# johncai117/Meta-Fine-Tuning

Hardware: AMD Instinct MI355X
Metric: episodes/sec at 5-way N-shot (ResNet10+GNN) per GPU and 1/2/4/8-GPU node (higher is better)
Workload: dtype f32

## Files before the change

include/mft_hip.h:

```cpp
#ifndef MFT_HIP_H
#define MFT_HIP_H

#ifdef __cplusplus
extern "C" {
#endif

#define MFT_EINVAL (-22)

enum { MFT_ACT_NONE = 0, MFT_ACT_RELU = 1, MFT_ACT_LRELU = 2 };
enum { MFT_BN_AFFINE_FMA = 0x100 };

int mft_version(void);
int mft_device_info(int* cu_count, int* gcn_arch_is_gfx950);

int mft_stream_create_cumask(const unsigned* mask_words, int n_words, void** stream_out);
int mft_stream_create_priority(int priority, void** stream_out, int* range_out);
int mft_stream_destroy(void* stream);
int mft_stream_probe(float* w, float* m, float* v, long long n, void* stream);
int mft_event_create(void** event_out);
int mft_event_record(void* event, void* stream);
int mft_event_elapsed_ms(void* start, void* stop, float* ms_out);
int mft_event_destroy(void* event);
int mft_probe_placement(unsigned* out, int n_blocks, int spin_cycles, void* stream);

int mft_augment_views(const unsigned char* src, int n_img, int Hs, int Ws, const float* params, int n_views, float* out,
                      long long view_stride, long long img_stride, int size, const float* mean3, const float* std3,
                      void* stream);

int mft_nchw_to_nhwc(const float* src, float* dst, int n_img, int C, int H, int W, void* stream);

long long mft_conv2d_wgrad_adam_dgrad_ws_floats(int n_img, int H, int W, int Cin);
int mft_conv2d_wgrad_adam_dgrad_nhwc(const float* x, int ldx, const float* dy, int ldy, float* w, float* m, float* v,
                                     float* dx_partials, int n_img, int H, int W, int Cin, int Cout, int imgs_per_group,
                                     long long group_stride, int step, float lr, float beta1, float beta2, float eps, void* stream);
int mft_conv2d_wgrad_adam_dgrad_nhwc_dev(const float* x, int ldx, const float* dy, int ldy, float* w, float* m, float* v,
                                         float* dx_partials, int n_img, int H, int W, int Cin, int Cout, int imgs_per_group,
                                         long long group_stride, const float* hyper, float beta1, float beta2, float eps,
                                         void* stream);
int mft_col2im_bn_backward_small(const float* dx_partials, const float* x_raw, const float* relu_out, float* dx, int n_img, int H,
                                 int W, int C, int imgs_per_group, const float* mean, const float* rstd, const float* gamma,
                                 long long gb_group_stride, float* dgamma, float* dbeta, void* stream);

int mft_ce_pool_bn_backward2(const float* feat, const int* labels, int imgs_per_group, int n_groups, int C, int hw,
                             const float* out, const float* xa, const float* xb, float* dxa, float* dxb, const float* mean_a,
                             const float* rstd_a, const float* gamma_a, const float* mean_b, const float* rstd_b,
                             const float* gamma_b, long long gb_group_stride, float* dgamma_a, float* dbeta_a, float* dgamma_b,
                             float* dbeta_b, float* loss, void* stream);

int mft_stem_cache_fill(const float* in, const float* w, int w_ld, int n_img, int H, int W, float* pmax, float* pmin,
                        float* mean_img, float* m2_img, void* stream);
int mft_pool_window_minmax(const float* x, float* ymax, float* ymin, long long n_img, int H, int W, int C, void* stream);
int mft_bn_relu_pooled_gather(const float* pmax, const float* pmin, const int* src_idx, float* y, int n_img, int OH, int OW, int C,
                              int imgs_per_group, const float* mean, const float* rstd, const float* gamma, const float* beta,
                              void* stream);

int mft_bn_apply_planes(const float* x, int ldx, float* y, int ldy, unsigned short* planes, long long plane_stride, int C,
                        int rows_per_group, int n_groups, const float* mean, const float* rstd, const float* gamma,
                        const float* beta, long long gb_group_stride, const float* res, int ldr, const float* res_mean,
                        const float* res_rstd, const float* res_gamma, const float* res_beta, int act, float slope,
                        void* stream);
int mft_bn_relu_maxpool_gather_planes(const float* x, const int* src_idx, float* y, unsigned short* planes,
                                      long long plane_stride, int n_img, int H, int W, int C, int imgs_per_group,
                                      const float* mean, const float* rstd, const float* gamma, const float* beta, void* stream);
int mft_conv2d_nhwc_x3p_bnstats(const unsigned short* in_planes, long long in_plane_elems, int ldi, const unsigned short* w3,
                                long long plane_elems, float* out, int ldo, int n_img, int H, int W, int Cin, int Cout, int KH,
                                int KW, int stride, int pad, int imgs_per_group, float eps, float* stats_ws, float* mean,
                                float* rstd, void* stream);

int mft_ingest_episode_views(const float* const* views, int n_views, int double_first, int n_way, int per_class, int n_support,
                             int C, int H, int W, float* support_store, float* all_store, void* stream);
int mft_pack_oihw(const float* w_oihw, float* w_pk, int Cout, int Cin, int KH, int KW, int k_pad, void* stream);
int mft_pack_oihw_multi(const void* jobs, int n_jobs, long long total_elements, void* stream);
int mft_unpack_oihw(const float* w_pk, float* w_oihw, int Cout, int Cin, int KH, int KW, int k_pad, void* stream);
int mft_pack_dgrad(const float* w_pk, float* wt_pk, int Cout, int Cin, int KH, int KW,
                   int groups, long long w_stride, long long wt_stride, void* stream);

int mft_conv2d_nhwc(const float* in, int ldi, const float* w, const float* bias, float* out, int ldo,
                    int n_img, int H, int W, int Cin, int Cout, int KH, int KW, int stride, int pad,
                    int imgs_per_group, long long w_group_stride, void* stream);

int mft_split_bf16x3(const float* w, unsigned short* planes, long long n, void* stream);
int mft_split_bf16x3_multi(const void* jobs, int n_jobs, long long total_elements, void* stream);
int mft_conv2d_nhwc_x3(const float* in, int ldi, const unsigned short* w3, long long plane_elems, float* out, int ldo,
                       int n_img, int H, int W, int Cin, int Cout, int KH, int KW, int stride, int pad, void* stream);
long long mft_conv2d_x3_stats_ws_floats(int n_img, int H, int W, int Cout, int KH, int KW, int stride, int pad);
int mft_conv2d_nhwc_x3_bnstats(const float* in, int ldi, const unsigned short* w3, long long plane_elems, float* out, int ldo,
                               int n_img, int H, int W, int Cin, int Cout, int KH, int KW, int stride, int pad,
                               int imgs_per_group, float eps, float* stats_ws, float* mean, float* rstd, void* stream);
int mft_conv2d_nhwc_x3_bnin_bnstats(const float* in, int ldi, const float* in_ws, const float* in_gamma, const float* in_beta,
                                    const unsigned short* w3, long long plane_elems, float* out, int ldo, int n_img, int H, int W,
                                    int Cin, int Cout, int imgs_per_group, float eps, float* stats_ws, float* mean, float* rstd,
                                    void* stream);
int mft_split_f16x2(const float* w, unsigned short* planes, long long n, void* stream);
int mft_conv2d_nhwc_h2(const float* in, int ldi, const unsigned short* w2, long long plane_elems, float* out, int ldo,
                       int n_img, int H, int W, int Cin, int Cout, int KH, int KW, int stride, int pad, void* stream);
int mft_conv2d_nhwc_h2_bnstats(const float* in, int ldi, const unsigned short* w2, long long plane_elems, float* out, int ldo,
                               int n_img, int H, int W, int Cin, int Cout, int KH, int KW, int stride, int pad,
                               int imgs_per_group, float eps, float* stats_ws, float* mean, float* rstd, void* stream);
int mft_conv2d_nhwc_h2_bnin_bnstats(const float* in, int ldi, const float* in_ws, const float* in_gamma, const float* in_beta,
                                    const unsigned short* w2, long long plane_elems, float* out, int ldo, int n_img, int H, int W,
                                    int Cin, int Cout, int imgs_per_group, float eps, float* stats_ws, float* mean, float* rstd,
                                    void* stream);
int mft_bn_apply_x3ws(const float* x, int ldx, float* y, int ldy, int C, int rows_per_group, int n_groups, const float* ws,
                      const float* gamma, const float* beta, const float* res, int ldr, const float* res_ws,
                      const float* res_gamma, const float* res_beta, int act, float slope, float eps, float* mean, float* rstd,
                      float* res_mean, float* res_rstd, void* stream);
int mft_bn_running_ema(const float* mean_a, const float* rstd_a, int rows_a, const float* mean_b, const float* rstd_b, int rows_b,
                       const int* order, int n_steps, int C, float eps, float momentum, float* running_mean, float* running_var,
                       void* stream);
int mft_bn_apply_x3ws_fits(int C, int rows_per_group, int with_res_bn);
int mft_bn_relu_pooled_gather_moments(const float* pmax, const float* pmin, const int* src_idx, float* y, int n_img, int OH, int OW,
                                      int C, int imgs_per_group, const float* mean_img, const float* m2_img, int rows_per_img,
                                      float eps, const float* gamma, const float* beta, float* mean, float* rstd, void* stream);

int mft_has_experiments(void);

int mft_conv2d_dgrad_nhwc(const float* dy, int ldy, const float* w, float* dx, int ldx,
                          int n_img, int H, int W, int Cin, int Cout, int KH, int KW, int stride, int pad,
                          int imgs_per_group, long long w_group_stride, void* stream);

long long mft_conv_ksplit_ws_floats(long long rows, int cols, int K);
long long mft_conv_ksplit_grouped_ws_floats(long long rows_per_group, int cols, int K, int groups);
int mft_conv2d_nhwc_ksplit_grouped(const float* in, int ldi, const float* w, float* out, int ldo, int n_img, int H, int W, int Cin,
                                   int Cout, int KH, int KW, int stride, int pad, int imgs_per_group, long long w_group_stride,
                                   float* ws, void* stream);
int mft_conv2d_dgrad_nhwc_ksplit_grouped(const float* dy, int ldy, const float* w, float* dx, int ldx, int n_img, int H, int W, int Cin,
                                         int Cout, int KH, int KW, int stride, int pad, int imgs_per_group, long long w_group_stride,
                                         float* ws, void* stream);
int mft_conv2d_nhwc_ksplit(const float* in, int ldi, const float* w, const float* bias, float* out, int ldo, int n_img, int H, int W,
                           int Cin, int Cout, int KH, int KW, int stride, int pad, float* ws, void* stream);
int mft_conv2d_dgrad_nhwc_ksplit(const float* dy, int ldy, const float* w, float* dx, int ldx, int n_img, int H, int W, int Cin,
                                 int Cout, int KH, int KW, int stride, int pad, float* ws, void* stream);
long long mft_conv2d_wgrad_ws_floats(int n_img, int H, int W, int Cin, int Cout, int KH, int KW, int stride, int pad,
                                     int imgs_per_group);
int mft_conv2d_wgrad_nhwc(const float* in, int ldi, const float* dy, int ldy, float* dw,
                          int n_img, int H, int W, int Cin, int Cout, int KH, int KW, int stride, int pad,
                          int imgs_per_group, long long dw_group_stride, float* ws, void* stream);

long long mft_conv2d_wgrad_oihw_ws_floats(int n_img, int H, int W, int Cin, int Cout, int KH, int KW, int stride, int pad);
int mft_conv2d_wgrad_oihw(const float* in, int ldi, const float* dy, int ldy, float* dw_oihw, int n_img, int H, int W, int Cin,
                          int Cout, int KH, int KW, int stride, int pad, int cin_valid, int cout_valid, float* ws, void* stream);

typedef struct MftWgradJob {
    const float* in; const float* dy; float* dw_oihw; float* ws;
    int ldi, ldy, n_img, H, W, Cin, Cout, KH, KW, stride, pad, cin_valid, cout_valid, reserved;
} MftWgradJob;
int mft_conv2d_wgrad_oihw_multi(const MftWgradJob* jobs, int n_jobs, void* stream);

int mft_conv2d_wgrad_adam_nhwc(const float* in, int ldi, const float* dy, int ldy, float* w, float* m, float* v,
                               float* dw_or_null, int n_img, int H, int W, int Cin, int Cout, int KH, int KW,
                               int stride, int pad, int imgs_per_group, long long group_stride,
                               int step, float lr, float beta1, float beta2, float eps, void* stream);

int mft_wgrad_adam_next_forward(const float* x, int ldx, const float* dy, int ldy, float* w, float* m, float* v,
                                float* dw_or_null, int n_img, int H, int W, int Cin, int Cout, int KH, int KW, int stride,
                                int pad, int imgs_per_group, long long group_stride, int step, const float* hyper, float lr,
                                float beta1, float beta2, float eps, const float* x_next, int mode, float* raw, float* act,
                                const float* gamma, const float* beta, long long gb_group_stride, float* mean, float* rstd,
                                const float* sc_raw, const float* gamma_s, const float* beta_s, float* mean_s, float* rstd_s,
                                float* pooled, float bn_eps, void* stream);


long long mft_bn_stats_ws_floats(int C, int rows_per_group, int n_groups);
int mft_bn_stats(const float* x, int ldx, int C, int rows_per_group, int n_groups, float eps,
                 float* mean, float* rstd, float* ws,
                 float* running_mean, float* running_var, float momentum, long long* num_batches_tracked, void* stream);
typedef struct MftBnStatsJob {
    const float* x; float* mean; float* rstd; float* ws; float* running_mean; float* running_var; long long* num_batches_tracked;
    int ldx, C, rows_per_group, n_groups; float eps, momentum;
} MftBnStatsJob;
int mft_bn_stats_multi(const MftBnStatsJob* jobs, int n_jobs, void* stream);
typedef struct MftBnFwdJob {
    const float* x; float* y; const float* gamma; const float* beta; float* mean; float* rstd;
    float* running_mean; float* running_var; long long* num_batches_tracked;
    const float* res; const float* res_gamma; const float* res_beta; float* res_mean; float* res_rstd;
    float* res_running_mean; float* res_running_var; long long* res_num_batches_tracked;
    int ldx, ldy, ldr, C, rows_per_group, n_groups, act; float eps, momentum, slope;
} MftBnFwdJob;
int mft_bn_forward_small(const MftBnFwdJob* job, void* stream);
int mft_bn_forward_small_max_rows(void);
typedef struct MftBnApplyJob {
    const float* x; float* y; const float* mean; const float* rstd; const float* gamma; const float* beta;
    int ldx, ldy, C, rows_per_group, n_groups, act; float slope; int reserved;
} MftBnApplyJob;
int mft_bn_apply_multi(const MftBnApplyJob* jobs, int n_jobs, void* stream);
int mft_bn_apply(const float* x, int ldx, float* y, int ldy, int C, int rows_per_group, int n_groups,
                 const float* mean, const float* rstd, const float* gamma, const float* beta,
                 long long gb_group_stride,
                 const float* res, int ldr, const float* res_mean, const float* res_rstd,
                 const float* res_gamma, const float* res_beta,
                 int act, float slope, void* stream);
int mft_var_to_rstd(const float* var, float* rstd, int n, float eps, void* stream);
int mft_bn_relu_maxpool(const float* x, float* y, int n_img, int H, int W, int C, int imgs_per_group,
                        const float* mean, const float* rstd, const float* gamma, const float* beta,
                        void* stream);

int mft_bn_image_moments(const float* x, int ldx, int C, int rows_per_img, long long n_img, float* mean_img, float* m2_img,
                         void* stream);
int mft_bn_combine_moments(const float* mean_img, const float* m2_img, const int* idx, int C, int rows_per_img,
                           int imgs_per_group, int n_groups, float eps, float* mean, float* rstd, void* stream);
int mft_bn_relu_maxpool_gather(const float* x, const int* src_idx, float* y, int n_img, int H, int W, int C,
                               int imgs_per_group, const float* mean, const float* rstd, const float* gamma,
                               const float* beta, void* stream);
int mft_global_avgpool(const float* x, float* y, int n_img, int HW, int C, void* stream);

int mft_bn_backward(const float* x, int ldx, const float* dy, int lddy, const float* relu_out, int ldro,
                    float* dx, int lddx, int C, int rows_per_group, int n_groups,
                    const float* mean, const float* rstd, const float* gamma, long long gb_group_stride,
                    float* dgamma, float* dbeta, void* stream);
int mft_bn_small_forward(const float* x1, int ld1, const float* x2, int ld2, const float* res, int ldr, float* y, int ldy, int C,
                         int rows_per_group, int n_groups, const float* gamma1, const float* beta1, const float* gamma2,
                         const float* beta2, long long gb_group_stride, float* mean1, float* rstd1, float* mean2, float* rstd2,
                         int act, float slope, float eps, float* pooled, int hw, void* stream);
int mft_bn_backward2(const float* xa, const float* xb, int ldx, const float* dy, int lddy, float* dxa, float* dxb, int lddx, int C,
                     int rows_per_group, int n_groups, const float* mean_a, const float* rstd_a, const float* gamma_a,
                     const float* mean_b, const float* rstd_b, const float* gamma_b, long long gb_group_stride, float* dgamma_a,
                     float* dbeta_a, float* dgamma_b, float* dbeta_b, void* stream);
int mft_ce_pool_backward(const float* feat, const int* labels, int rows_per_group, int n_groups, int C, int hw, const float* out,
                         float* d_out, float* loss, void* stream);

int mft_avgpool_relu_backward(const float* dfeat, const float* out, float* dout, int n_img, int HW, int C, void* stream);

int mft_cross_entropy(const float* logits, int ld, const int* labels, int C, int rows_per_group, int n_groups,
                      float* loss, float* dlogits, void* stream);
int mft_cross_entropy_mean(const float* logits, int ld, const void* labels, int labels_i64, int C, int rows, float* loss,
                           double* loss_sum, void* stream);
int mft_cross_entropy_mean_backward(const float* logits, int ld, const void* labels, int labels_i64, int C, int rows,
                                    const float* grad_loss, float* dlogits, int ldd, void* stream);
int mft_softmax_rows(const float* x, int ldx, float* y, int ldy, int C, int rows, void* stream);

int mft_proto_scores(const float* feats, int ld, int episodes, int n_way, int n_support, int n_query, int D, float* scores,
                     int softmax, void* stream);
int mft_proto_backward(const float* feats, int ld, int episodes, int n_way, int n_support, int n_query, int D,
                       const float* dscores, int ldg, float* dfeats, int ldd, void* stream);

int mft_adam_step(float* p, const float* g, float* m, float* v, long long n, int step,
                  float lr, float beta1, float beta2, float eps, float weight_decay, void* stream);
int mft_sgd_step(float* p, const float* g, float* buf, long long n, int first_step,
                 float lr, float momentum, float dampening, float weight_decay, void* stream);
int mft_block_entry_small_forward(const float* x, int ldx, const float* w_c1, long long w1_group_stride, const float* w_sc,
                                  long long wsc_group_stride, float* c1, float* r1, float* sc, int n_img, int H, int W, int Cin,
                                  int Cout, int stride, int imgs_per_group, const float* gamma1, const float* beta1,
                                  long long gb_group_stride, float* mean1, float* rstd1, float eps, void* stream);

int mft_block_exit_small_forward(const float* r1, const float* w_c2, long long w_group_stride, const float* sc, float* c2,
                                 float* out, float* pooled, int n_img, int H, int W, int C, int imgs_per_group,
                                 const float* gamma2, const float* beta2, const float* gamma_sc, const float* beta_sc,
                                 long long gb_group_stride, float* mean2, float* rstd2, float* mean_sc, float* rstd_sc, float eps,
                                 void* stream);

int mft_conv2d_dgrad_bn_backward_small(const float* dy, int ldy, const float* w, float* dx, int ldx, int n_img, int H, int W,
                                       int Cin, int Cout, int KH, int KW, int pad, int imgs_per_group, long long w_group_stride,
                                       const float* x_raw, const float* relu_out, const float* mean, const float* rstd,
                                       const float* gamma, long long gb_group_stride, float* dgamma, float* dbeta, void* stream);

int mft_linear_head_sgd_run(const float* z_support, const int* y_support, const int* idx_table, int n_groups, int n_support_rows,
                            int D, int n_way, int n_steps, int batch_size, float* W, float* b, float lr, float momentum,
                            float dampening, float weight_decay, void* stream);

int mft_linear_head_adam_run(const float* z_support, const int* y_support, const int* idx_table, int n_groups, int n_support_rows,
                             int D, int n_way, int n_steps, int batch_size, float* W, float* b, float lr, float beta1, float beta2,
                             float eps, float weight_decay, void* stream);

int mft_adam_multi(const void* chunk_table, int n_chunks, int step, float lr, float beta1, float beta2, float eps,
                   float weight_decay, float grad_scale, void* stream);

int mft_adam_hyper_advance(int* step, float* hyper, float lr, float beta1, float beta2, void* stream);
int mft_adam_step_dev(float* p, const float* g, float* m, float* v, long long n, const float* hyper, float beta1, float beta2,
                      float eps, float weight_decay, void* stream);
int mft_conv2d_wgrad_adam_nhwc_dev(const float* in, int ldi, const float* dy, int ldy, float* w, float* m, float* v,
                                   float* dw_or_null, int n_img, int H, int W, int Cin, int Cout, int KH, int KW, int stride,
                                   int pad, int imgs_per_group, long long group_stride, const float* hyper, float beta1,
                                   float beta2, float eps, void* stream);
int mft_maml_delta(float* p, const float* p2, const float* p3, long long n, void* stream);

int mft_linear_head_step(const float* feat, int ldf, const int* labels, int rows_per_group, int n_groups, int n_way, int D,
                         float* W, float* b, float* mW, float* vW, float* mb, float* vb, float* dfeat, int lddf, float* loss,
                         int step, float lr, float beta1, float beta2, float eps, float weight_decay, void* stream);
int mft_linear_head_scores(const float* feat, int ldf, int rows_per_group, int n_groups, int n_way, int D, const float* W,
                           const float* b, float* out, void* stream);

int mft_pair_absdiff(const float* x, int ldx, float* d, int ldd, int n_graphs, int N, int F, void* stream);
int mft_masked_softmax(const float* s, int lds_, float* A, int n_graphs, int N, void* stream);
int mft_gemm_rk(const float* a, int lda, const float* w, int w_rows, int K, const float* bias, float* out, int ldo, int M, int N,
                void* stream);
int mft_pair_mlp_tiles_m(int graphs_per_group, int N);
int mft_pair_mlp_tiles_m_rk(int graphs_per_group, int N);
int mft_pair_mlp_layer_rk(const float* in, int ld_in, int mode, const int* ij, const float* scale_in, const float* shift_in,
                          const float* w, int K, int Kpad, const float* bias, float* out, int Cout, int n_groups,
                          int graphs_per_group, int N, float slope, float* ws_mean, float* ws_m2, float* ws_n, void* stream);
int mft_pair_mlp_stats_finalize_rk(const float* ws_mean, const float* ws_m2, const float* ws_n, int n_groups, int tiles_m, int C,
                                   const float* gamma, const float* beta, float eps, float* scale, float* shift,
                                   float* mean_out, float* rstd_out, void* stream);
int mft_pair_mlp_layer(const float* in, int ld_in, int mode, const int* ij, const float* scale_in, const float* shift_in,
                       const float* w, int K, int Kpad, const float* bias, float* out, int Cout, int n_groups,
                       int graphs_per_group, int N, float slope, float* ws_mean, float* ws_m2, float* ws_n, int f16x2, void* stream);
int mft_pair_mlp_stats_finalize(const float* ws_mean, const float* ws_m2, const float* ws_n, int n_groups, int tiles_m, int C,
                                const float* gamma, const float* beta, float eps, float* scale, float* shift,
                                float* mean_out, float* rstd_out, void* stream);
int mft_pair_mlp_score(const float* h, int C, const float* scale, const float* shift, const float* w5, const float* b5,
                       float slope, float* s_ut, int n_groups, int graphs_per_group, int N, void* stream);
int mft_masked_softmax_ut(const float* s_ut, float* A, int n_graphs, int N, void* stream);

int mft_pair_softmax_ut_backward(const float* A, const float* dA, const int* ij, float* rowdot_ws, float* ds, int ldds,
                                 int n_graphs, int N, float* dbias_zero, void* stream);
long long mft_pair_bwd_stats_ws_floats(long long rows_per_group, int C);
int mft_pair_bn_act_backward(const float* g, int ldg, const float* z, int C, const float* scale, const float* shift,
                             const float* mean, const float* rstd, const float* gamma, const int* ij, int N, long long rows_per_group,
                             int n_groups, long long n_tot, float slope, float* ws, float* sums, float* dparams, float* dbias_zero,
                             float* dz, void* stream);
int mft_pair_absdiff_ut(const float* x, int ldx, const int* ij, float* d, int Kp, int F, int N, long long row0, long long nrows,
                        void* stream);
int mft_pair_dx_gather(const float* x, int ldx, const float* dd, int lddd, float* dX, int lddx, int n_graphs, int N, int F,
                       long long row0, long long nrows, void* stream);
int mft_graph_aggregate(const float* A, const float* x, int ldx, float* y, int ldy,
                        int n_graphs, int N, int F, void* stream);
int mft_copy_cols(const float* x, int ldx, float* y, int ldy, int col_off, int C, int rows,
                  int act, float slope, void* stream);

int mft_build_graph_nodes(const float* z, int zf, float* nodes, int ld, int n_episodes, int n_way,
                          int n_support, int n_query, int fold, void* stream);
int mft_gather_query_scores(const float* out, int ldo, float* scores, int n_episodes, int n_way,
                            int n_support, int n_query, void* stream);
int mft_gather_rows(const float* src, const int* idx, float* dst, int n_rows, long long row_floats, void* stream);

long long mft_bn_backward_ws_floats(int C, int rows_per_group, int n_groups);
int mft_bn_backward_act(const float* x, int ldx, const float* dy, int lddy, const float* y_act, int ldya,
                        float* dx, int lddx, int C, int rows_per_group, int n_groups,
                        const float* mean, const float* rstd, const float* gamma, long long gb_group_stride,
                        float* dgamma, float* dbeta, int act, float slope, float* ws, float* dgamma_sum, float* dbeta_sum,
                        float* dbias_zero, void* stream);
typedef struct MftBnBwdJob {
    const float* x; const float* dy; const float* y_act; float* dx; const float* mean; const float* rstd; const float* gamma;
    float* dgamma; float* dbeta; float* ws; float* dgamma_sum; float* dbeta_sum; float* dbias_zero;
    int ldx, lddy, ldya, lddx, C, rows_per_group, n_groups, act; float slope; int reserved;
} MftBnBwdJob;
int mft_bn_backward_act_multi(const MftBnBwdJob* jobs, int n_jobs, void* stream);
int mft_act_backward(const float* dy, int lddy, const float* y, int ldy, float* dx, int lddx, int C, long long rows,
                     int act, float slope, int accumulate, void* stream);
int mft_colsum(const float* x, int ldx, int C, long long rows, float* out, float* ws, void* stream);
int mft_bn_relu_maxpool_arg(const float* x, float* y, unsigned char* argmax, int n_img, int H, int W, int C,
                            int imgs_per_group, const float* mean, const float* rstd, const float* gamma,
                            const float* beta, void* stream);
int mft_maxpool_relu_backward(const float* dy, const unsigned char* argmax, const float* y, float* dx,
                              int n_img, int H, int W, int C, void* stream);
int mft_masked_softmax_backward(const float* A, const float* dA, float* ds, int ldds, int n_graphs, int N, void* stream);
int mft_pair_absdiff_backward(const float* x, int ldx, const float* dd, int ldd, float* dx, int lddx,
                              int n_graphs, int N, int F, void* stream);
int mft_graph_aggregate_backward(const float* A, const float* x, int ldx, const float* dy, int lddy, float* dx, int lddx,
                                 float* dA, int n_graphs, int N, int F, int accumulate, void* stream);
int mft_build_graph_nodes_backward(const float* dnodes, int ld, float* dz, int zf, int n_episodes, int n_way,
                                   int n_support, int n_query, int fold, void* stream);
int mft_gather_query_scores_backward(const float* dscores, float* dout, int ldo, int n_episodes, int n_way,
                                     int n_support, int n_query, float* dbias, void* stream);

#ifdef __cplusplus
}
#endif
#endif
```

include/mft_hip_testing.h:

```cpp
#ifndef MFT_HIP_TESTING_H
#define MFT_HIP_TESTING_H
#ifdef __cplusplus
extern "C" {
#endif

int mft_debug_set_conv_tile(int tile);
int mft_debug_set_x3_tile(int tile);
int mft_debug_reset(void);
void mft_wgrad_fwd_set_exact(int on);
void mft_wgrad_fwd_set_xcd(int on);

#ifdef __cplusplus
}
#endif
#endif
```

meta-fine-tuning_amd/_lib.py:

```python
import ctypes
import os

PKG = os.path.dirname(os.path.abspath(__file__))
LIB_PATH = os.path.join(PKG, "libmft_hip.so")

_P = ctypes.c_void_p
_I = ctypes.c_int
_L = ctypes.c_longlong
_F = ctypes.c_float

SIGNATURES = {
    "mft_version": [],
    "mft_device_info": [_P, _P],
    "mft_stream_create_cumask": [_P, _I, _P],
    "mft_stream_destroy": [_P],
    "mft_stream_probe": [_P, _P, _P, _L, _P],
    "mft_probe_placement": [_P, _I, _I, _P],
    "mft_event_create": [_P],
    "mft_event_record": [_P, _P],
    "mft_event_elapsed_ms": [_P, _P, _P],
    "mft_event_destroy": [_P],
    "mft_augment_views": [_P, _I, _I, _I, _P, _I, _P, _L, _L, _I, _P, _P, _P],
    "mft_nchw_to_nhwc": [_P, _P, _I, _I, _I, _I, _P],
    "mft_pack_oihw": [_P, _P, _I, _I, _I, _I, _I, _P],
    "mft_unpack_oihw": [_P, _P, _I, _I, _I, _I, _I, _P],
    "mft_pack_dgrad": [_P, _P, _I, _I, _I, _I, _I, _L, _L, _P],
    "mft_conv2d_nhwc": [_P, _I, _P, _P, _P, _I, _I, _I, _I, _I, _I, _I, _I, _I, _I, _I, _L, _P],
    "mft_has_experiments": [],
    "mft_split_bf16x3": [_P, _P, _L, _P],
    "mft_split_bf16x3_multi": [_P, _I, _L, _P],
    "mft_conv2d_nhwc_x3": [_P, _I, _P, _L, _P, _I, _I, _I, _I, _I, _I, _I, _I, _I, _I, _P],
    "mft_conv2d_x3_stats_ws_floats": [_I, _I, _I, _I, _I, _I, _I, _I],
    "mft_conv2d_nhwc_x3_bnstats": [_P, _I, _P, _L, _P, _I, _I, _I, _I, _I, _I, _I, _I, _I, _I, _I, _F, _P, _P, _P, _P],
    "mft_conv2d_dgrad_nhwc": [_P, _I, _P, _P, _I, _I, _I, _I, _I, _I, _I, _I, _I, _I, _I, _L, _P],
    "mft_conv_ksplit_ws_floats": [_L, _I, _I],
    "mft_conv_ksplit_grouped_ws_floats": [_L, _I, _I, _I],
    "mft_conv2d_nhwc_ksplit_grouped": [_P, _I, _P, _P, _I, _I, _I, _I, _I, _I, _I, _I, _I, _I, _I, _L, _P, _P],
    "mft_conv2d_dgrad_nhwc_ksplit_grouped": [_P, _I, _P, _P, _I, _I, _I, _I, _I, _I, _I, _I, _I, _I, _I, _L, _P, _P],
    "mft_conv2d_nhwc_ksplit": [_P, _I, _P, _P, _P, _I, _I, _I, _I, _I, _I, _I, _I, _I, _I, _P, _P],
    "mft_conv2d_dgrad_nhwc_ksplit": [_P, _I, _P, _P, _I, _I, _I, _I, _I, _I, _I, _I, _I, _I, _P, _P],
    "mft_conv2d_wgrad_oihw_ws_floats": [_I, _I, _I, _I, _I, _I, _I, _I, _I],
    "mft_conv2d_wgrad_oihw": [_P, _I, _P, _I, _P, _I, _I, _I, _I, _I, _I, _I, _I, _I, _I, _I, _P, _P],
    "mft_conv2d_wgrad_oihw_multi": [_P, _I, _P],
    "mft_conv2d_wgrad_ws_floats": [_I, _I, _I, _I, _I, _I, _I, _I, _I, _I],
    "mft_conv2d_wgrad_nhwc": [_P, _I, _P, _I, _P, _I, _I, _I, _I, _I, _I, _I, _I, _I, _I, _L, _P, _P],
    "mft_conv2d_wgrad_adam_nhwc": [_P, _I, _P, _I, _P, _P, _P, _P, _I, _I, _I, _I, _I, _I, _I, _I, _I, _I, _L, _I, _F, _F, _F,
                                   _F, _P],
    "mft_pair_softmax_ut_backward": [_P, _P, _P, _P, _P, _I, _I, _I, _P, _P],
    "mft_pair_bwd_stats_ws_floats": [_L, _I],
    "mft_pair_bn_act_backward": [_P, _I, _P, _I, _P, _P, _P, _P, _P, _P, _I, _L, _I, _L, _F, _P, _P, _P, _P, _P, _P],
    "mft_pair_absdiff_ut": [_P, _I, _P, _P, _I, _I, _I, _L, _L, _P],
    "mft_pair_dx_gather": [_P, _I, _P, _I, _P, _I, _I, _I, _I, _L, _L, _P],
    "mft_pack_oihw_multi": [_P, _I, _L, _P],
    "mft_wgrad_adam_next_forward": [_P, _I, _P, _I, _P, _P, _P, _P, _I, _I, _I, _I, _I, _I, _I, _I, _I, _I, _L, _I, _P, _F, _F, _F,
                                    _F, _P, _I, _P, _P, _P, _P, _L, _P, _P, _P, _P, _P, _P, _P, _P, _F, _P],
    "mft_bn_stats_ws_floats": [_I, _I, _I],
    "mft_bn_stats": [_P, _I, _I, _I, _I, _F, _P, _P, _P, _P, _P, _F, _P, _P],
    "mft_bn_apply": [_P, _I, _P, _I, _I, _I, _I, _P, _P, _P, _P, _L, _P, _I, _P, _P, _P, _P, _I, _F, _P],
    "mft_bn_apply_multi": [_P, _I, _P],
    "mft_bn_stats_multi": [_P, _I, _P],
    "mft_bn_relu_maxpool": [_P, _P, _I, _I, _I, _I, _I, _P, _P, _P, _P, _P],
    "mft_bn_relu_maxpool_gather": [_P, _P, _P, _I, _I, _I, _I, _I, _P, _P, _P, _P, _P],
    "mft_bn_image_moments": [_P, _I, _I, _I, _L, _P, _P, _P],
    "mft_bn_combine_moments": [_P, _P, _P, _I, _I, _I, _I, _F, _P, _P, _P],
    "mft_global_avgpool": [_P, _P, _I, _I, _I, _P],
    "mft_bn_small_forward": [_P, _I, _P, _I, _P, _I, _P, _I, _I, _I, _I, _P, _P, _P, _P, _L, _P, _P, _P, _P, _I, _F, _F, _P, _I, _P],
    "mft_bn_backward2": [_P, _P, _I, _P, _I, _P, _P, _I, _I, _I, _I, _P, _P, _P, _P, _P, _P, _L, _P, _P, _P, _P, _P],
    "mft_ce_pool_backward": [_P, _P, _I, _I, _I, _I, _P, _P, _P, _P],
    "mft_bn_backward": [_P, _I, _P, _I, _P, _I, _P, _I, _I, _I, _I, _P, _P, _P, _L, _P, _P, _P],
    "mft_avgpool_relu_backward": [_P, _P, _P, _I, _I, _I, _P],
    "mft_cross_entropy": [_P, _I, _P, _I, _I, _I, _P, _P, _P],
    "mft_softmax_rows": [_P, _I, _P, _I, _I, _I, _P],
    "mft_proto_scores": [_P, _I, _I, _I, _I, _I, _I, _P, _I, _P],
    "mft_proto_backward": [_P, _I, _I, _I, _I, _I, _I, _P, _I, _P, _I, _P],
    "mft_cross_entropy_mean": [_P, _I, _P, _I, _I, _I, _P, _P, _P],
    "mft_cross_entropy_mean_backward": [_P, _I, _P, _I, _I, _I, _P, _P, _I, _P],
    "mft_adam_step": [_P, _P, _P, _P, _L, _I, _F, _F, _F, _F, _F, _P],
    "mft_sgd_step": [_P, _P, _P, _L, _I, _F, _F, _F, _F, _P],
    "mft_maml_delta": [_P, _P, _P, _L, _P],
    "mft_conv2d_wgrad_adam_dgrad_ws_floats": [_I, _I, _I, _I],
    "mft_conv2d_wgrad_adam_dgrad_nhwc": [_P, _I, _P, _I, _P, _P, _P, _P, _I, _I, _I, _I, _I, _I, _L, _I, _F, _F, _F, _F, _P],
    "mft_conv2d_wgrad_adam_dgrad_nhwc_dev": [_P, _I, _P, _I, _P, _P, _P, _P, _I, _I, _I, _I, _I, _I, _L, _P, _F, _F, _F, _P],
    "mft_col2im_bn_backward_small": [_P, _P, _P, _P, _I, _I, _I, _I, _I, _P, _P, _P, _L, _P, _P, _P],
    "mft_stream_create_priority": [_I, _P, _P],
    "mft_ce_pool_bn_backward2": [_P, _P, _I, _I, _I, _I, _P, _P, _P, _P, _P, _P, _P, _P, _P, _P, _P, _L, _P, _P, _P, _P, _P, _P],
    "mft_pool_window_minmax": [_P, _P, _P, _L, _I, _I, _I, _P],
    "mft_stem_cache_fill": [_P, _P, _I, _I, _I, _I, _P, _P, _P, _P, _P],
    "mft_conv2d_nhwc_x3_bnin_bnstats": [_P, _I, _P, _P, _P, _P, _L, _P, _I, _I, _I, _I, _I, _I, _I, _F, _P, _P, _P, _P],
    "mft_split_f16x2": [_P, _P, _L, _P],
    "mft_conv2d_nhwc_h2": [_P, _I, _P, _L, _P, _I, _I, _I, _I, _I, _I, _I, _I, _I, _I, _P],
    "mft_conv2d_nhwc_h2_bnstats": [_P, _I, _P, _L, _P, _I, _I, _I, _I, _I, _I, _I, _I, _I, _I, _I, _F, _P, _P, _P, _P],
    "mft_conv2d_nhwc_h2_bnin_bnstats": [_P, _I, _P, _P, _P, _P, _L, _P, _I, _I, _I, _I, _I, _I, _I, _F, _P, _P, _P, _P],
    "mft_bn_apply_x3ws": [_P, _I, _P, _I, _I, _I, _I, _P, _P, _P, _P, _I, _P, _P, _P, _I, _F, _F, _P, _P, _P, _P, _P],
    "mft_bn_apply_x3ws_fits": [_I, _I, _I],
    "mft_bn_running_ema": [_P, _P, _I, _P, _P, _I, _P, _I, _I, _F, _F, _P, _P, _P],
    "mft_bn_relu_pooled_gather_moments": [_P, _P, _P, _P, _I, _I, _I, _I, _I, _P, _P, _I, _F, _P, _P, _P, _P, _P],
    "mft_bn_relu_pooled_gather": [_P, _P, _P, _P, _I, _I, _I, _I, _I, _P, _P, _P, _P, _P],
    "mft_bn_apply_planes": [_P, _I, _P, _I, _P, _L, _I, _I, _I, _P, _P, _P, _P, _L, _P, _I, _P, _P, _P, _P, _I, _F, _P],
    "mft_bn_relu_maxpool_gather_planes": [_P, _P, _P, _P, _L, _I, _I, _I, _I, _I, _P, _P, _P, _P, _P],
    "mft_conv2d_nhwc_x3p_bnstats": [_P, _L, _I, _P, _L, _P, _I, _I, _I, _I, _I, _I, _I, _I, _I, _I, _I, _F, _P, _P, _P, _P],
    "mft_ingest_episode_views": [_P, _I, _I, _I, _I, _I, _I, _I, _I, _P, _P, _P],
    "mft_block_entry_small_forward": [_P, _I, _P, _L, _P, _L, _P, _P, _P, _I, _I, _I, _I, _I, _I, _I, _P, _P, _L, _P, _P, _F, _P],
    "mft_block_exit_small_forward": [_P, _P, _L, _P, _P, _P, _P, _I, _I, _I, _I, _I, _P, _P, _P, _P, _L, _P, _P, _P, _P, _F, _P],
    "mft_conv2d_dgrad_bn_backward_small": [_P, _I, _P, _P, _I, _I, _I, _I, _I, _I, _I, _I, _I, _I, _L, _P, _P, _P, _P, _P, _L,
                                           _P, _P, _P],
    "mft_linear_head_sgd_run": [_P, _P, _P, _I, _I, _I, _I, _I, _I, _P, _P, _F, _F, _F, _F, _P],
    "mft_linear_head_adam_run": [_P, _P, _P, _I, _I, _I, _I, _I, _I, _P, _P, _F, _F, _F, _F, _F, _P],
    "mft_adam_multi": [_P, _I, _I, _F, _F, _F, _F, _F, _F, _P],
    "mft_adam_hyper_advance": [_P, _P, _F, _F, _F, _P],
    "mft_adam_step_dev": [_P, _P, _P, _P, _L, _P, _F, _F, _F, _F, _P],
    "mft_conv2d_wgrad_adam_nhwc_dev": [_P, _I, _P, _I, _P, _P, _P, _P, _I, _I, _I, _I, _I, _I, _I, _I, _I, _I, _L, _P, _F, _F,
                                       _F, _P],
    "mft_linear_head_step": [_P, _I, _P, _I, _I, _I, _I, _P, _P, _P, _P, _P, _P, _P, _I, _P, _I, _F, _F, _F, _F, _F, _P],
    "mft_linear_head_scores": [_P, _I, _I, _I, _I, _I, _P, _P, _P, _P],
    "mft_pair_absdiff": [_P, _I, _P, _I, _I, _I, _I, _P],
    "mft_masked_softmax": [_P, _I, _P, _I, _I, _P],
    "mft_pair_mlp_tiles_m": [_I, _I],
    "mft_pair_mlp_layer": [_P, _I, _I, _P, _P, _P, _P, _I, _I, _P, _P, _I, _I, _I, _I, _F, _P, _P, _P, _I, _P],
    "mft_bn_forward_small": [_P, _P],
    "mft_bn_forward_small_max_rows": [],
    "mft_gemm_rk": [_P, _I, _P, _I, _I, _P, _P, _I, _I, _I, _P],
    "mft_pair_mlp_tiles_m_rk": [_I, _I],
    "mft_pair_mlp_layer_rk": [_P, _I, _I, _P, _P, _P, _P, _I, _I, _P, _P, _I, _I, _I, _I, _F, _P, _P, _P, _P],
    "mft_pair_mlp_stats_finalize_rk": [_P, _P, _P, _I, _I, _I, _P, _P, _F, _P, _P, _P, _P, _P],
    "mft_pair_mlp_stats_finalize": [_P, _P, _P, _I, _I, _I, _P, _P, _F, _P, _P, _P, _P, _P],
    "mft_pair_mlp_score": [_P, _I, _P, _P, _P, _P, _F, _P, _I, _I, _I, _P],
    "mft_masked_softmax_ut": [_P, _P, _I, _I, _P],
    "mft_graph_aggregate": [_P, _P, _I, _P, _I, _I, _I, _I, _P],
    "mft_copy_cols": [_P, _I, _P, _I, _I, _I, _I, _I, _F, _P],
    "mft_build_graph_nodes": [_P, _I, _P, _I, _I, _I, _I, _I, _I, _P],
    "mft_gather_query_scores": [_P, _I, _P, _I, _I, _I, _I, _P],
    "mft_gather_rows": [_P, _P, _P, _I, _L, _P],
    "mft_var_to_rstd": [_P, _P, _I, _F, _P],
    "mft_bn_backward_ws_floats": [_I, _I, _I],
    "mft_bn_backward_act": [_P, _I, _P, _I, _P, _I, _P, _I, _I, _I, _I, _P, _P, _P, _L, _P, _P, _I, _F, _P, _P, _P, _P, _P],
    "mft_bn_backward_act_multi": [_P, _I, _P],
    "mft_act_backward": [_P, _I, _P, _I, _P, _I, _I, _L, _I, _F, _I, _P],
    "mft_colsum": [_P, _I, _I, _L, _P, _P, _P],
    "mft_bn_relu_maxpool_arg": [_P, _P, _P, _I, _I, _I, _I, _I, _P, _P, _P, _P, _P],
    "mft_maxpool_relu_backward": [_P, _P, _P, _P, _I, _I, _I, _I, _P],
    "mft_masked_softmax_backward": [_P, _P, _P, _I, _I, _I, _P],
    "mft_pair_absdiff_backward": [_P, _I, _P, _I, _P, _I, _I, _I, _I, _P],
    "mft_graph_aggregate_backward": [_P, _P, _I, _P, _I, _P, _I, _P, _I, _I, _I, _I, _P],
    "mft_build_graph_nodes_backward": [_P, _I, _P, _I, _I, _I, _I, _I, _I, _P],
    "mft_gather_query_scores_backward": [_P, _P, _I, _I, _I, _I, _I, _P, _P],
}
TESTING_SIGNATURES = {
    "mft_debug_set_conv_tile": [_I],
    "mft_debug_set_x3_tile": [_I],
    "mft_debug_reset": [],
    "mft_wgrad_fwd_set_exact": [_I],
    "mft_wgrad_fwd_set_xcd": [_I],
}
_RESTYPE = {"mft_conv2d_x3_stats_ws_floats": _L, "mft_bn_stats_ws_floats": _L, "mft_conv2d_wgrad_ws_floats": _L, "mft_bn_backward_ws_floats": _L,
            "mft_conv2d_wgrad_adam_dgrad_ws_floats": _L, "mft_pair_bwd_stats_ws_floats": _L, "mft_conv_ksplit_ws_floats": _L, "mft_conv2d_wgrad_oihw_ws_floats": _L, "mft_conv_ksplit_grouped_ws_floats": _L}

_lib = None


def lib():
    global _lib
    if _lib is None:
        if not os.path.exists(LIB_PATH):
            raise RuntimeError(
                "libmft_hip.so not found at %s -- build it with `python -c 'import __graft_entry__ as g; g.build()'`; "
                "this package has no CPU or PyTorch fallback" % LIB_PATH)
        import torch
        if torch.cuda.is_available():
            torch.cuda.init()
            torch.empty(1, device="cuda")
        h = ctypes.CDLL(LIB_PATH)
        for name, argtypes in list(SIGNATURES.items()) + list(TESTING_SIGNATURES.items()):
            fn = getattr(h, name)
            fn.argtypes = argtypes
            fn.restype = _RESTYPE.get(name, _I)
        _lib = h
    return _lib


MFT_EINVAL = -22


def check(rc, what):
    if rc != 0:
        raise RuntimeError("%s failed with code %d (hipError_t / MFT_EINVAL=-22)" % (what, rc))


class LaunchTimer:

    _SKIP = ("mft_event_", "mft_stream_", "mft_debug_", "mft_version", "mft_device_info", "mft_has_experiments",
             "mft_wgrad_fwd_set_", "mft_probe_placement")

    def __init__(self, only=None, keep_args=False):
        self.only = only
        self.keep_args = keep_args
        self._pairs = []
        self._free = []
        self._real = None

    def _event(self):
        if self._free:
            return self._free.pop()
        e = ctypes.c_void_p()
        check(self._real.mft_event_create(ctypes.byref(e)), "mft_event_create")
        return e

    def __getattr__(self, name):
        real = self.__dict__["_real"]
        fn = getattr(real, name)
        sig = SIGNATURES.get(name)
        if (sig is None or not sig or sig[-1] is not _P or name.endswith("_ws_floats") or name.startswith(self._SKIP)
                or (self.only is not None and not self.only(name))):
            return fn

        def timed(*args):
            stream = args[-1]
            a, b = self._event(), self._event()
            real.mft_event_record(a, stream)
            rc = fn(*args)
            if rc != 0:
                self._free += [a, b]
                return rc
            real.mft_event_record(b, stream)
            self._pairs.append((name, a, b, args if self.keep_args else None))
            return rc
        return timed

    def __enter__(self):
        global _lib
        self._real = lib()
        assert not isinstance(self._real, LaunchTimer), "LaunchTimer blocks do not nest"
        _lib = self
        return self

    def __exit__(self, *exc):
        global _lib
        _lib = self._real
        if exc and exc[0] is not None:
            for _, a, b, _ in self._pairs:
                self._free += [a, b]
            self._pairs = []
            self.close()
        return False

    def collect(self, calls=False):
        out, flat = {}, []
        ms = ctypes.c_float()
        for name, a, b, args in self._pairs:
            check(self._real.mft_event_elapsed_ms(a, b, ctypes.byref(ms)), "mft_event_elapsed_ms")
            out.setdefault(name, []).append(float(ms.value))
            flat.append((name, float(ms.value), args))
            self._free += [a, b]
        self._pairs = []
        return flat if calls else out

    def close(self):
        for e in self._free:
            self._real.mft_event_destroy(e)
        self._free = []
```

meta-fine-tuning_amd/csrc/conv_igemm.hip:

```cpp
#include "mft_common.h"
#include "mft_hip_testing.h"

int mft_stem_conv_dispatch(const float* in, const float* w, float* out, int n_img, int H, int W, int w_ld,
                           hipStream_t s);
int mft_skinny_fwd_dispatch(const float* in, int ldi, const float* w, float* out, int ldo, int n_img, int H, int W,
                            int Cin, int Cout, int KH, int KW, int stride, int pad, int imgs_per_group,
                            long long w_group_stride, hipStream_t s);
void mft_skinny_set_dgrad_slices(int n);
void mft_skinny_set_tap(int v);
void mft_skinny_set_x3(int v);
void mft_skinny_set_nw(int v);
void mft_bn_small_set_rows(int rows);
void mft_bn_fwd_small_set_rows(int rows);
void mft_skinny_set_lines(int v);
int mft_skinny_dgrad_dispatch(const float* dy, int ldy, const float* w, float* dx, int ldx, int n_img, int H, int W,
                              int Cin, int Cout, int KH, int KW, int stride, int pad, int imgs_per_group,
                              long long w_group_stride, hipStream_t s);

namespace {

struct ConvArgs {
    const float* in;
    const float* w;
    const float* bias;
// ... 915 lines not shown
            rdy[u] = v;
        }
        const long long ibase = (long long)img * p.H * p.W;
#pragma unroll
        for (int u = 0; u < NPR; ++u) {
            const int ih = 2 * oh - 3 + e_kh[u], iw = 2 * ow0 - 3 + e_q3[u];
            float v = 0.f;
            if (e_lds[u] >= 0 && ih >= 0 && ih < p.H && iw >= 0 && iw < p.W) v = p.in[(ibase + (long long)ih * p.W + iw) * p.ldi + e_ci[u]];
            rpr[u] = v;
        }
    };
    auto store_strip = [&]() {
#pragma unroll
        for (int u = 0; u < NDY; ++u) {
            const int i = tid + NT * u;
            *(f32x4*)(dy_s + (i >> 4) * 64 + (i & 15) * 4) = rdy[u];
        }
#pragma unroll
        for (int u = 0; u < NPR; ++u)
            if (e_lds[u] >= 0) prow[e_lds[u]] = rpr[u];
    };

    int kh_q[NQ];
#pragma unroll
    for (int q = 0; q < NQ; ++q) kh_q[q] = wave + NWAVE * q < 14 ? (wave + NWAVE * q) >> 1 : 0;
    int s = blockIdx.x;
    if (s < n_strips) load_strip(s);
    for (; s < n_strips; s += gridDim.x) {
        __syncthreads();
        store_strip();
        __syncthreads();
        if (s + (int)gridDim.x < n_strips) load_strip(s + gridDim.x);
        const float* ap = dy_s + h * 64 + cb * 32 + r;
        const float* bp = prow + 6 * h + r;
        const int np = S2 >> 1;
        int tp = 0;
        for (; tp + 4 <= np; tp += 4) {
            float a[4], b[4][NQ];
#pragma unroll
            for (int u = 0; u < 4; ++u) {
                a[u] = ap[(tp + u) * 128];
#pragma unroll
                for (int q = 0; q < NQ; ++q) b[u][q] = bp[kh_q[q] * PR + 12 * (tp + u)];
            }
#pragma unroll
            for (int u = 0; u < 4; ++u)
#pragma unroll
                for (int q = 0; q < NQ; ++q) acc[q] = __builtin_amdgcn_mfma_f32_32x32x2f32(a[u], b[u][q], acc[q], 0, 0, 0);
        }
        for (; tp < np; ++tp) {
            const float a = ap[tp * 128];
#pragma unroll
            for (int q = 0; q < NQ; ++q) acc[q] = __builtin_amdgcn_mfma_f32_32x32x2f32(a, bp[kh_q[q] * PR + 12 * tp], acc[q], 0, 0, 0);
        }
    }
    float* out = p.ws + (long long)blockIdx.x * p.dwgs;
#pragma unroll
    for (int q = 0; q < NQ; ++q) {
        const int c = wave + NWAVE * q;
        if (c >= 14 || r >= 21) continue;
        const int kh = c >> 1;
#pragma unroll
        for (int e = 0; e < 16; ++e) {
            const int co = cb * 32 + (e & 3) + 8 * (e >> 2) + 4 * h;
            out[(long long)co * p.Kpad + kh * 21 + r] = acc[q][e];
        }
    }
}

int g_stem_wgrad_strips = 1;

template <int BM, int BN, bool ADAM, bool STEMW = false, bool EARLYT = false, int POL = 3>
int launch_wgrad(const WgradArgs& a, int taps, int groups, hipStream_t s) {
    constexpr int lds_mm = 32 * (BM + BN) * 4;
    constexpr int lds_ad = BM * (BN + 4) * 4;
    constexpr int lds0 = ADAM ? (lds_ad > lds_mm ? lds_ad : lds_mm) : lds_mm;
    int lds = lds0;
    if (ADAM && g_wgrad_min_lds_kb * 1024 > lds) lds = g_wgrad_min_lds_kb * 1024;
    auto kern = conv_wgrad_kernel<BM, BN, ADAM, STEMW, EARLYT, POL>;
    if (lds > 64 * 1024) {
        static MftPerDeviceOnce attr_once;
        if (attr_once.need()) {
            hipError_t e = hipFuncSetAttribute((const void*)kern, hipFuncAttributeMaxDynamicSharedMemorySize, lds);
            if (e != hipSuccess) return (int)e;
            attr_once.mark();
        }
    }
    WgradArgs p = a;
    p.tiles_ci = ((STEMW ? a.Kpad : a.Cin) + BN - 1) / BN;
    p.tiles_co = (a.Cout + BM - 1) / BM;
    dim3 grid(p.tiles_ci * p.tiles_co * taps, groups, p.chunks);
    hipLaunchKernelGGL(kern, grid, dim3(256), lds, s, p);
    if (p.oihw || p.chunks > 1) {
        const long long n = (long long)a.Cout * a.Kpad;
        int blocks = (int)((n / 4 + 31) / 32);
        if (blocks > 4096) blocks = 4096;
        if (p.oihw)
            hipLaunchKernelGGL(reduce_chunks_kernel<true>, dim3(blocks, 1), dim3(256), 0, s, (const float*)p.ws, p.dw, n, p.chunks, p.dwgs,
                               a.Cin, a.KH * a.KW, a.Kpad, a.cin_out > 0 ? a.cin_out : a.Cin, a.cout_out > 0 ? a.cout_out : a.Cout);
        else
            hipLaunchKernelGGL(reduce_chunks_kernel<false>, dim3(blocks, groups), dim3(256), 0, s, (const float*)p.ws, p.dw, n, p.chunks,
                               p.dwgs, a.Cin, a.KH * a.KW, a.Kpad, a.Cin, a.Cout);
    }
    return mft_launch_status();
}

constexpr int WGRAD_CHUNK_ROWS = 1024;

inline void wgrad_chunking(long long rows, long long wgs_per_chunk, int* chunk_rows, int* chunks) {
    *chunk_rows = (int)rows;
    *chunks = 1;
    if (rows <= 256) return;
    const long long want = (768 + wgs_per_chunk - 1) / wgs_per_chunk;
    long long cr = ((rows + want - 1) / want + 31) / 32 * 32;
    if (cr < 128) cr = 128;
    if (cr > WGRAD_CHUNK_ROWS) cr = WGRAD_CHUNK_ROWS;
    const long long n = (rows + cr - 1) / cr;
    if (n <= 1) return;
    *chunk_rows = (int)cr;
    *chunks = (int)n;
}

inline long long wgrad_wgs_per_chunk(int Cin, int Cout, int KH, int KW, long long groups) {
    if (Cin == 3) return (long long)(((KH * KW * Cin + 31) / 32 * 32 + 63) / 64) * ((Cout + 63) / 64) * groups;
    return (long long)((Cin + 63) / 64) * ((Cout + 63) / 64) * KH * KW * groups;
}

int wgrad_dispatch(WgradArgs a, int n_img, int imgs_per_group, bool adam, float* ws, hipStream_t s) {
    if (imgs_per_group <= 0) imgs_per_group = n_img;
    if (n_img % imgs_per_group != 0) return MFT_EINVAL;
    const bool stem = (a.Cin == 3);
    if ((!stem && a.Cin % 4 != 0) || a.Cout % 4 != 0 || (!stem && a.ldi % 4 != 0) || a.ldy % 4 != 0) return MFT_EINVAL;
    const int groups = n_img / imgs_per_group;
    a.OH = (a.H + 2 * a.pad - a.KH) / a.stride + 1;
    a.OW = (a.W + 2 * a.pad - a.KW) / a.stride + 1;
    a.Kpad = (a.KH * a.KW * a.Cin + 31) / 32 * 32;
    a.imgs_per_group = imgs_per_group;
    a.rows_per_group = imgs_per_group * a.OH * a.OW;
    a.chunk_rows = a.rows_per_group;
    a.chunks = 1;
    a.ws = ws;
    if (a.oihw && (adam || ws == nullptr || groups != 1)) return MFT_EINVAL;
    if (!adam && ws != nullptr) wgrad_chunking(a.rows_per_group, wgrad_wgs_per_chunk(a.Cin, a.Cout, a.KH, a.KW, groups), &a.chunk_rows, &a.chunks);
    const int taps = a.KH * a.KW;
    if (stem && !adam && g_stem_wgrad_strips && a.oihw && a.KH == 7 && a.KW == 7 && a.stride == 2 && a.pad == 3 && a.Cout == 64 && groups == 1 &&
        a.chunks > 1 && a.Kpad == 160 && (((unsigned long long)a.dy) & 15) == 0 && (a.cin_out <= 0 || a.cin_out == a.Cin) &&
        (a.cout_out <= 0 || a.cout_out == a.Cout)) {
        StemWgArgs q;
        q.in = a.in; q.dy = a.dy; q.ws = a.ws; q.n_img = n_img; q.H = a.H; q.W = a.W; q.ldi = a.ldi; q.ldy = a.ldy; q.OH = a.OH; q.OW = a.OW;
        q.nseg = (a.OW + 63) / 64;
        q.S = (a.OW + q.nseg - 1) / q.nseg;
        q.Kpad = a.Kpad; q.dwgs = a.dwgs;
        int wgs = a.chunks;
        const long long strips = (long long)n_img * a.OH * q.nseg;
        if (strips < wgs) return launch_wgrad<64, 64, false, true>(a, 1, groups, s);
        hipLaunchKernelGGL(stem_wgrad_strip_kernel, dim3(wgs), dim3(512), 0, s, q);
        const long long n = (long long)a.Cout * a.Kpad;
        int blocks = (int)((n / 4 + 31) / 32);
        hipLaunchKernelGGL(reduce_chunks_kernel<true>, dim3(blocks, 1), dim3(256), 0, s, (const float*)a.ws, a.dw, n, a.chunks, a.dwgs, a.Cin,
                           a.KH * a.KW, a.Kpad, a.Cin, a.Cout);
        return mft_launch_status();
    }
    if (stem) return adam ? MFT_EINVAL : launch_wgrad<64, 64, false, true>(a, 1, groups, s);
    if (adam) {
        if (a.Cin % 64 != 0 || a.Cout % 64 != 0) return MFT_EINVAL;
        if (g_wgrad_rows && a.rows_per_group <= 64 && a.Cin % 128 == 0 && a.Cout % 32 == 0)
            return launch_wgrad_adam_rows(a, taps, groups, s);
        if (a.Cin % 128 == 0 && a.Cout % 128 == 0 && g_wgrad_tile != 64) return launch_wgrad<128, 128, true>(a, taps, groups, s);
        if (g_wgrad_early && (g_wgrad_pol & 3) == 0) return launch_wgrad<64, 64, true, false, true, 0>(a, taps, groups, s);
        if (g_wgrad_early && (g_wgrad_pol & 3) == 1) return launch_wgrad<64, 64, true, false, true, 1>(a, taps, groups, s);
        if (g_wgrad_early && (g_wgrad_pol & 3) == 2) return launch_wgrad<64, 64, true, false, true, 2>(a, taps, groups, s);
        if (g_wgrad_early) return launch_wgrad<64, 64, true, false, true>(a, taps, groups, s);
        return launch_wgrad<64, 64, true>(a, taps, groups, s);
    }
    return launch_wgrad<64, 64, false>(a, taps, groups, s);
}

}

static int conv2d_impl(const float* in, int ldi, const float* w, const float* bias, float* out, int ldo,
                       int n_img, int H, int W, int Cin, int Cout, int KH, int KW, int stride, int pad,
                       int imgs_per_group, long long w_group_stride, float* ws, void* stream) {
    if (n_img <= 0 || Cout <= 0) return MFT_EINVAL;
    const bool stem = (Cin == 3);
    if (!stem && (Cin % 32 != 0 || ldi % 4 != 0)) return MFT_EINVAL;
    if (imgs_per_group <= 0) imgs_per_group = n_img;
    if (n_img % imgs_per_group != 0) return MFT_EINVAL;
    const int groups = n_img / imgs_per_group;
    ConvArgs a;
    a.in = in; a.w = w; a.bias = bias; a.out = out;
    a.ldi = ldi; a.ldo = ldo;
    a.H = H; a.W = W; a.Cin = Cin; a.KH = KH; a.KW = KW; a.stride = stride; a.pad = pad;
    a.OH = (H + 2 * pad - KH) / stride + 1;
    a.OW = (W + 2 * pad - KW) / stride + 1;
    a.Cout = Cout;
    a.Ktot = KH * KW * Cin;
    a.Kpad = (a.Ktot + 31) / 32 * 32;
    a.imgs_per_group = imgs_per_group;
    a.rows_per_group = imgs_per_group * a.OH * a.OW;
    a.wgs = (groups > 1) ? w_group_stride : 0;
    a.tiles_n = 0;
    a.bt_stride = 1;
    a.ksplit = 1; a.ws = nullptr; a.parity = 0;
    if (ws != nullptr && !stem && ldo % 4 == 0) {
        a.ksplit = conv_ksplit(a.rows_per_group, Cout, a.Kpad, groups);
        a.ws = ws;
    }
    hipStream_t s = (hipStream_t)stream;
    if (stem) {
        if (g_stem_fast && KH == 7 && KW == 7 && stride == 2 && pad == 3 && Cout == 64 && ldi == 3 && ldo == 64 &&
            bias == nullptr && (W == 84 || W == 224)) {
            const int rc = mft_stem_conv_dispatch(in, w, out, n_img, H, W, a.Kpad, s);
            if (rc != MFT_EINVAL) return rc;
        }
        return launch_conv<128, 64, 2, 2, true>(a, groups, s);
    }
    if (g_skinny && groups > 1 && w_group_stride != 0 && bias == nullptr && ws == nullptr) {
        const int rc = mft_skinny_fwd_dispatch(in, ldi, w, out, ldo, n_img, H, W, Cin, Cout, KH, KW, stride, pad,
                                               imgs_per_group, w_group_stride, s);
        if (rc != MFT_EINVAL) return rc;
    }
    int tile = g_conv_tile;
    if (tile == 0) tile = (Cout >= 64) ? 4 : 5;
    switch (tile) {
        case 1: return launch_conv<128, 128, 2, 2, false>(a, groups, s);
        case 2: return launch_conv<128, 64, 2, 2, false>(a, groups, s);
        case 3: return launch_conv<64, 128, 2, 2, false>(a, groups, s);
        case 4: return launch_conv<64, 64, 2, 2, false>(a, groups, s);
        default: return launch_conv<128, 32, 4, 1, false>(a, groups, s);
    }
}

extern "C" int mft_conv2d_nhwc(const float* in, int ldi, const float* w, const float* bias, float* out, int ldo,
                               int n_img, int H, int W, int Cin, int Cout, int KH, int KW, int stride, int pad,
                               int imgs_per_group, long long w_group_stride, void* stream) {
    return conv2d_impl(in, ldi, w, bias, out, ldo, n_img, H, W, Cin, Cout, KH, KW, stride, pad, imgs_per_group, w_group_stride,
                       nullptr, stream);
}

extern "C" long long mft_conv_ksplit_ws_floats(long long rows, int cols, int K) {
    const int s = conv_ksplit(rows, cols, K);
    return s > 1 ? (long long)s * rows * cols : 0;
}

extern "C" long long mft_conv_ksplit_grouped_ws_floats(long long rows_per_group, int cols, int K, int groups) {
    const int s = conv_ksplit(rows_per_group, cols, K, groups);
    return s > 1 ? (long long)s * groups * rows_per_group * cols : 0;
}

extern "C" int mft_conv2d_nhwc_ksplit_grouped(const float* in, int ldi, const float* w, float* out, int ldo, int n_img, int H, int W,
                                              int Cin, int Cout, int KH, int KW, int stride, int pad, int imgs_per_group,
                                              long long w_group_stride, float* ws, void* stream) {
    if (ws == nullptr || imgs_per_group <= 0) return MFT_EINVAL;
    return conv2d_impl(in, ldi, w, nullptr, out, ldo, n_img, H, W, Cin, Cout, KH, KW, stride, pad, imgs_per_group, w_group_stride, ws,
                       stream);
}

extern "C" int mft_conv2d_nhwc_ksplit(const float* in, int ldi, const float* w, const float* bias, float* out, int ldo,
                                      int n_img, int H, int W, int Cin, int Cout, int KH, int KW, int stride, int pad, float* ws,
                                      void* stream) {
    return conv2d_impl(in, ldi, w, bias, out, ldo, n_img, H, W, Cin, Cout, KH, KW, stride, pad, 0, 0, ws, stream);
}

extern "C" int mft_has_experiments(void) {
#ifdef MFT_EXPERIMENTS
    return 1;
#else
    return 0;
#endif
}

extern "C" int mft_debug_set_conv_tile(int tile) {
#ifndef MFT_EXPERIMENTS
    if (tile == 9502 || tile == 9504 || tile == 9505) return MFT_EINVAL;
    if (tile >= 9000 && tile < 9100 && tile != 9003 && tile != 9007) return MFT_EINVAL;
    if (tile > 4000 && tile < 5000) return MFT_EINVAL;
#endif
    if (tile >= 11000) { mft_bn_small_set_rows(tile - 11000); mft_bn_fwd_small_set_rows(tile - 11000); }
    else if (tile >= 9800) g_dgrad_parity = tile - 9800;
    else if (tile >= 9700) mft_skinny_set_lines(tile - 9700);
    else if (tile >= 9600) g_wgrad_trim = tile - 9600;
    else if (tile >= 9500) g_wgrad_rows = tile - 9500;
    else if (tile >= 9100) mft_skinny_set_nw(tile - 9100);
    else if (tile >= 9000) g_wgrad_pol = tile - 9000;
    else if (tile >= 8000) mft_skinny_set_x3(tile - 8000);
    else if (tile >= 7000) mft_skinny_set_tap(tile - 7000);
    else if (tile >= 6000) mft_skinny_set_dgrad_slices(tile - 6000);
    else if (tile >= 5000) g_wgrad_early = tile - 5000;
    else if (tile >= 4000) g_wgrad_min_lds_kb = tile - 4000;
    else if (tile >= 3000) g_skinny = tile - 3000;
    else if (tile >= 2100) g_stem_wgrad_strips = tile - 2100;
    else if (tile >= 2000) g_stem_fast = tile - 2000;
    else if (tile >= 1000) g_wgrad_tile = tile - 1000;
    else g_conv_tile = tile;
    return 0;
}

extern "C" int mft_debug_set_x3_tile(int t);

extern "C" void mft_wgrad_fwd_set_exact(int on);
extern "C" int mft_debug_reset(void) {
    mft_wgrad_fwd_set_exact(0);
    mft_wgrad_fwd_set_xcd(1);
    g_dgrad_parity = 1; g_wgrad_trim = 1; g_wgrad_rows = 1; g_wgrad_tile = 64; g_conv_tile = 0; g_wgrad_pol = 7; g_wgrad_early = 1; g_wgrad_min_lds_kb = 0; g_skinny = 1; g_stem_fast = 1; g_stem_wgrad_strips = 1;
    mft_skinny_set_lines(1); mft_skinny_set_nw(0); mft_skinny_set_x3(1); mft_skinny_set_tap(1); mft_skinny_set_dgrad_slices(1);
    mft_debug_set_x3_tile(0); mft_debug_set_x3_tile(10); mft_debug_set_x3_tile(21); mft_debug_set_x3_tile(31); mft_debug_set_x3_tile(41);
    mft_bn_small_set_rows(512); mft_bn_fwd_small_set_rows(512);
    mft_debug_set_x3_tile(60); mft_debug_set_x3_tile(70); mft_debug_set_x3_tile(80); mft_debug_set_x3_tile(91); mft_debug_set_x3_tile(100); mft_debug_set_x3_tile(200);
    return 0;
}

static int dgrad_impl(const float* dy, int ldy, const float* w, float* dx, int ldx, int n_img, int H,
                      int W, int Cin, int Cout, int KH, int KW, int stride, int pad,
                      int imgs_per_group, long long w_group_stride, float* ws, void* stream) {
    if (Cout % 32 != 0 || Cin % 4 != 0 || ldy % 4 != 0 || stride < 1) return MFT_EINVAL;
    if (imgs_per_group <= 0) imgs_per_group = n_img;
    if (n_img % imgs_per_group != 0) return MFT_EINVAL;
    const int groups = n_img / imgs_per_group;
    if (g_skinny && groups > 1 && w_group_stride != 0 && ws == nullptr) {
        const int rc = mft_skinny_dgrad_dispatch(dy, ldy, w, dx, ldx, n_img, H, W, Cin, Cout, KH, KW, stride, pad,
                                                 imgs_per_group, w_group_stride, (hipStream_t)stream);
        if (rc != MFT_EINVAL) return rc;
    }
    ConvArgs a;
    a.in = dy; a.w = w; a.bias = nullptr; a.out = dx;
    a.ldi = ldy; a.ldo = ldx;
    a.H = (H + 2 * pad - KH) / stride + 1;
    a.W = (W + 2 * pad - KW) / stride + 1;
    a.Cin = Cout; a.KH = KH; a.KW = KW;
    a.stride = 1; a.pad = -pad;
    a.bt_stride = stride;
    a.OH = H; a.OW = W;
    a.Cout = Cin;
    a.Ktot = KH * KW * Cout;
    a.Kpad = a.Ktot;
    a.imgs_per_group = imgs_per_group;
    a.rows_per_group = imgs_per_group * H * W;
    a.wgs = (groups > 1) ? w_group_stride : 0;
    a.tiles_n = 0;
    a.ksplit = 1; a.ws = nullptr;
    a.parity = (groups == 1 && stride == 2 && g_dgrad_parity) ? 1 : 0;
    if (ws != nullptr && ldx % 4 == 0 && Cin % 64 == 0) {
        const int s_full = conv_ksplit(a.rows_per_group, Cin, a.Kpad, groups);
        if (!a.parity) {
            a.ksplit = s_full;
            a.ws = ws;
        } else if (s_full > 1) {
            int sp = conv_ksplit((long long)imgs_per_group * ((H + 1) / 2) * ((W + 1) / 2), Cin, ((KH + 1) / 2) * ((KW + 1) / 2) * Cout, 4);
            if (sp > s_full) sp = s_full;
            if (sp > 1) { a.ksplit = sp; a.ws = ws; }
        }
    }
    hipStream_t s = (hipStream_t)stream;
    if (Cin % 64 == 0) return launch_conv<64, 64, 2, 2, false, true>(a, groups, s);
    return launch_conv<128, 32, 4, 1, false, true>(a, groups, s);
}

extern "C" int mft_conv2d_dgrad_nhwc(const float* dy, int ldy, const float* w, float* dx, int ldx, int n_img, int H,
                                     int W, int Cin, int Cout, int KH, int KW, int stride, int pad,
                                     int imgs_per_group, long long w_group_stride, void* stream) {
    return dgrad_impl(dy, ldy, w, dx, ldx, n_img, H, W, Cin, Cout, KH, KW, stride, pad, imgs_per_group, w_group_stride, nullptr,
                      stream);
}

extern "C" int mft_conv2d_dgrad_nhwc_ksplit_grouped(const float* dy, int ldy, const float* w, float* dx, int ldx, int n_img, int H,
                                                    int W, int Cin, int Cout, int KH, int KW, int stride, int pad, int imgs_per_group,
                                                    long long w_group_stride, float* ws, void* stream) {
    if (ws == nullptr || imgs_per_group <= 0 || stride != 1) return MFT_EINVAL;
    return dgrad_impl(dy, ldy, w, dx, ldx, n_img, H, W, Cin, Cout, KH, KW, stride, pad, imgs_per_group, w_group_stride, ws, stream);
}

extern "C" int mft_conv2d_dgrad_nhwc_ksplit(const float* dy, int ldy, const float* w, float* dx, int ldx, int n_img, int H, int W,
                                            int Cin, int Cout, int KH, int KW, int stride, int pad, float* ws, void* stream) {
    return dgrad_impl(dy, ldy, w, dx, ldx, n_img, H, W, Cin, Cout, KH, KW, stride, pad, 0, 0, ws, stream);
}

extern "C" long long mft_conv2d_wgrad_ws_floats(int n_img, int H, int W, int Cin, int Cout, int KH, int KW, int stride,
                                                 int pad, int imgs_per_group) {
    if (imgs_per_group <= 0) imgs_per_group = n_img;
    const int OH = (H + 2 * pad - KH) / stride + 1, OW = (W + 2 * pad - KW) / stride + 1;
    const long long rows = (long long)imgs_per_group * OH * OW;
    int chunk_rows, chunks;
    wgrad_chunking(rows, wgrad_wgs_per_chunk(Cin, Cout, KH, KW, n_img / imgs_per_group), &chunk_rows, &chunks);
    if (chunks <= 1) return 0;
    const long long kpad = (KH * KW * Cin + 31) / 32 * 32;
    return (long long)(n_img / imgs_per_group) * chunks * Cout * kpad;
}

extern "C" int mft_conv2d_wgrad_nhwc(const float* in, int ldi, const float* dy, int ldy, float* dw,
                                     int n_img, int H, int W, int Cin, int Cout, int KH, int KW, int stride, int pad,
                                     int imgs_per_group, long long dw_group_stride, float* ws, void* stream) {
    WgradArgs a = {};
    a.in = in; a.dy = dy; a.dw = dw; a.ldi = ldi; a.ldy = ldy;
    a.H = H; a.W = W; a.Cin = Cin; a.Cout = Cout; a.KH = KH; a.KW = KW; a.stride = stride; a.pad = pad;
    a.dwgs = dw_group_stride;
    return wgrad_dispatch(a, n_img, imgs_per_group, false, ws, (hipStream_t)stream);
}

extern "C" long long mft_conv2d_wgrad_oihw_ws_floats(int n_img, int H, int W, int Cin, int Cout, int KH, int KW, int stride, int pad) {
    const int OH = (H + 2 * pad - KH) / stride + 1, OW = (W + 2 * pad - KW) / stride + 1;
    int chunk_rows, chunks;
    wgrad_chunking((long long)n_img * OH * OW, wgrad_wgs_per_chunk(Cin, Cout, KH, KW, 1), &chunk_rows, &chunks);
    return (long long)chunks * Cout * ((KH * KW * Cin + 31) / 32 * 32);
}

extern "C" int mft_conv2d_wgrad_oihw(const float* in, int ldi, const float* dy, int ldy, float* dw_oihw, int n_img, int H, int W,
                                     int Cin, int Cout, int KH, int KW, int stride, int pad, int cin_valid, int cout_valid, float* ws,
                                     void* stream) {
    if (ws == nullptr || cin_valid < 0 || cin_valid > Cin || cout_valid < 0 || cout_valid > Cout) return MFT_EINVAL;
    WgradArgs a = {};
    a.in = in; a.dy = dy; a.dw = dw_oihw; a.ldi = ldi; a.ldy = ldy;
    a.H = H; a.W = W; a.Cin = Cin; a.Cout = Cout; a.KH = KH; a.KW = KW; a.stride = stride; a.pad = pad;
    a.oihw = 1;
    a.cin_out = cin_valid; a.cout_out = cout_valid;
    a.dwgs = (long long)Cout * ((KH * KW * Cin + 31) / 32 * 32);
    return wgrad_dispatch(a, n_img, 0, false, ws, (hipStream_t)stream);
}

extern "C" int mft_conv2d_wgrad_oihw_multi(const MftWgradJob* jobs, int n_jobs, void* stream) {
    if (jobs == nullptr || n_jobs < 1) return MFT_EINVAL;
    hipStream_t s = (hipStream_t)stream;
    for (int j0 = 0; j0 < n_jobs;) {
        WgradMultiArgs wa = {};
        ReduceMultiArgs ra = {};
        int cnt = 0, wgs = 0, rblocks = 0;
        for (; j0 < n_jobs && cnt < WG_MULTI; ++j0) {
            const MftWgradJob& jb = jobs[j0];
            if (jb.ws == nullptr || jb.cin_valid < 0 || jb.cin_valid > jb.Cin || jb.cout_valid < 0 || jb.cout_valid > jb.Cout) return MFT_EINVAL;
            if (jb.Cin == 3) {
                int rc = mft_conv2d_wgrad_oihw(jb.in, jb.ldi, jb.dy, jb.ldy, jb.dw_oihw, jb.n_img, jb.H, jb.W, jb.Cin, jb.Cout, jb.KH, jb.KW,
                                               jb.stride, jb.pad, jb.cin_valid, jb.cout_valid, jb.ws, stream);
                if (rc != 0) return rc;
                continue;
            }
            if (jb.Cin % 4 != 0 || jb.Cout % 4 != 0 || jb.ldi % 4 != 0 || jb.ldy % 4 != 0 || jb.n_img < 1) return MFT_EINVAL;
            WgradArgs a = {};
            a.in = jb.in; a.dy = jb.dy; a.dw = jb.dw_oihw; a.ldi = jb.ldi; a.ldy = jb.ldy;
            a.H = jb.H; a.W = jb.W; a.Cin = jb.Cin; a.Cout = jb.Cout; a.KH = jb.KH; a.KW = jb.KW; a.stride = jb.stride; a.pad = jb.pad;
            a.oihw = 1; a.cin_out = jb.cin_valid; a.cout_out = jb.cout_valid;
            a.OH = (a.H + 2 * a.pad - a.KH) / a.stride + 1;
            a.OW = (a.W + 2 * a.pad - a.KW) / a.stride + 1;
            a.Kpad = (a.KH * a.KW * a.Cin + 31) / 32 * 32;
            a.dwgs = (long long)a.Cout * a.Kpad;
            a.imgs_per_group = jb.n_img;
            a.rows_per_group = jb.n_img * a.OH * a.OW;
            a.ws = jb.ws;
            wgrad_chunking(a.rows_per_group, wgrad_wgs_per_chunk(a.Cin, a.Cout, a.KH, a.KW, 1), &a.chunk_rows, &a.chunks);
            a.tiles_ci = (a.Cin + 63) / 64;
            a.tiles_co = (a.Cout + 63) / 64;
            const int nx = a.tiles_ci * a.tiles_co * a.KH * a.KW;
            wa.job[cnt] = a; wa.start[cnt] = wgs; wa.nx[cnt] = nx;
            wgs += nx * a.chunks;
            const long long n = (long long)a.Cout * a.Kpad;
            int blocks = (int)((n / 4 + 31) / 32);
            if (blocks > 4096) blocks = 4096;
            ra.ws[cnt] = a.ws; ra.dw[cnt] = a.dw; ra.n[cnt] = n; ra.dwgs[cnt] = a.dwgs; ra.chunks[cnt] = a.chunks; ra.Cin[cnt] = a.Cin;
            ra.taps[cnt] = a.KH * a.KW; ra.Kpad[cnt] = a.Kpad; ra.cin_out[cnt] = a.cin_out > 0 ? a.cin_out : a.Cin;
            ra.cout_out[cnt] = a.cout_out > 0 ? a.cout_out : a.Cout; ra.start[cnt] = rblocks;
            rblocks += blocks;
            ++cnt;
        }
        if (cnt == 0) continue;
        wa.start[cnt] = wgs; wa.n = cnt;
        ra.start[cnt] = rblocks; ra.cnt = cnt;
        constexpr int lds = 32 * (64 + 64) * 4;
        hipLaunchKernelGGL(conv_wgrad_multi_kernel, dim3(wgs), dim3(256), lds, s, wa);
        hipLaunchKernelGGL(reduce_chunks_multi_kernel, dim3(rblocks), dim3(256), 0, s, ra);
    }
    return mft_launch_status();
}

static int wgrad_adam_impl(const float* in, int ldi, const float* dy, int ldy, float* w, float* m, float* v,
                           float* dw_or_null, int n_img, int H, int W, int Cin, int Cout, int KH, int KW, int stride,
                           int pad, int imgs_per_group, long long group_stride, int step, const float* hyper, float lr,
                           float beta1, float beta2, float eps, void* stream) {
    if ((hyper == nullptr && step < 1) || (KH * KW * Cin) % 32 != 0) return MFT_EINVAL;
    if (hyper != nullptr) step = 1;
    WgradArgs a = {};
    a.in = in; a.dy = dy; a.dw = dw_or_null; a.ldi = ldi; a.ldy = ldy;
    a.H = H; a.W = W; a.Cin = Cin; a.Cout = Cout; a.KH = KH; a.KW = KW; a.stride = stride; a.pad = pad;
    a.dwgs = group_stride;
    a.w = w; a.m = m; a.v = v;
    const double bc1 = 1.0 - pow((double)beta1, (double)step);
    const double bc2 = 1.0 - pow((double)beta2, (double)step);
    a.step_size = (float)((double)lr / bc1);
    a.inv_sqrt_bc2 = (float)(1.0 / sqrt(bc2));
    a.b1 = beta1; a.b2 = beta2; a.eps = eps;
    a.hyper = hyper;
    return wgrad_dispatch(a, n_img, imgs_per_group, true, nullptr, (hipStream_t)stream);
}

extern "C" int mft_conv2d_wgrad_adam_nhwc(const float* in, int ldi, const float* dy, int ldy, float* w, float* m,
                                          float* v, float* dw_or_null, int n_img, int H, int W, int Cin, int Cout,
                                          int KH, int KW, int stride, int pad, int imgs_per_group,
                                          long long group_stride, int step, float lr, float beta1, float beta2,
                                          float eps, void* stream) {
    return wgrad_adam_impl(in, ldi, dy, ldy, w, m, v, dw_or_null, n_img, H, W, Cin, Cout, KH, KW, stride, pad,
                           imgs_per_group, group_stride, step, nullptr, lr, beta1, beta2, eps, stream);
}

extern "C" int mft_conv2d_wgrad_adam_nhwc_dev(const float* in, int ldi, const float* dy, int ldy, float* w, float* m,
                                              float* v, float* dw_or_null, int n_img, int H, int W, int Cin, int Cout,
                                              int KH, int KW, int stride, int pad, int imgs_per_group,
                                              long long group_stride, const float* hyper, float beta1, float beta2,
                                              float eps, void* stream) {
    if (hyper == nullptr) return MFT_EINVAL;
    return wgrad_adam_impl(in, ldi, dy, ldy, w, m, v, dw_or_null, n_img, H, W, Cin, Cout, KH, KW, stride, pad,
                           imgs_per_group, group_stride, 1, hyper, 0.f, beta1, beta2, eps, stream);
}
```

meta-fine-tuning_amd/csrc/wgrad_fwd.hip:

```cpp
#include "mft_common.h"
#include <math.h>

namespace {

struct WfArgs {
    const float* in; const float* dy; float* dw;
    float* w; float* m; float* v;
    int ldi, ldy;
    int H, W, Cin, OH, OW, Cout, KH, KW, stride, pad;
    int Kpad;
    int rows, ipg;
    int tiles_ci;
    int inv_ohw, inv_ow;
    int mma_rows;
    long long dwgs;
    float step_size, inv_sqrt_bc2, b1, b2, eps;
    const float* hyper;
    const float* xn;
    float* raw;
    float* act;
    const float* gamma; const float* beta; long long gbs;
    float* mean; float* rstd;
    const float* sc; const float* gs; const float* bs; float* means; float* rstds;
    float* pooled; int hw;
    float bn_eps;
    int co_blocks;
    int xcd_groups;
};

enum { WF_RAW = 0, WF_ENTRY = 1, WF_EXIT = 2 };

__device__ __forceinline__ float lane8_sum(float v) {
    v += __shfl_xor(v, 1, 64);
    v += __shfl_xor(v, 2, 64);
    v += __shfl_xor(v, 4, 64);
    return v;
}

template <int MODE, bool FAST, int NT>
__global__ __launch_bounds__(256) __attribute__((amdgpu_waves_per_eu(2, 2))) void wgrad_adam_fwd_kernel(WfArgs p) {
    constexpr int BM = 32, BN = 128, BLD = BN + 32, GLD = BN + 4, RLD = 36, TLD = 33;
    extern __shared__ __attribute__((aligned(16))) float smem[];
    float* As = smem;
    float* Bs = smem + 48 * BM;
    float* Gs = Bs + 48 * BLD;
    const int tid = threadIdx.x, lane = tid & 63, wave = tid >> 6;
    const int r = lane & 31, h = lane >> 5;
    const int fm = lane & 15, fq = lane >> 4;
    int g, co0;
    if (p.xcd_groups) {
        const int xcd = blockIdx.x & 7, slot = blockIdx.x >> 3;
        g = (slot / p.co_blocks) * 8 + xcd;
        co0 = (slot % p.co_blocks) * BM;
    } else {
        g = blockIdx.x / p.co_blocks;
        co0 = (blockIdx.x % p.co_blocks) * BM;
    }
    const int ohw = p.OH * p.OW;
    const int rows = p.rows;
    const long long row0 = (long long)g * rows;
    const long long img0 = (long long)g * p.ipg;
    const int n_kt = p.KH * p.KW * p.tiles_ci;
    const bool fwd = p.xn != nullptr;

    const int arow = tid >> 3, acol = (tid & 7) * 4;
    const int brow = tid >> 5, bcol = (tid & 31) * 4;
#pragma unroll
    for (int j = 0; j < 2; ++j) {
        const int m = arow + 32 * j;
        f32x4 v = {0.f, 0.f, 0.f, 0.f};
        if (m < rows) v = *(const f32x4*)(p.dy + (row0 + m) * p.ldy + co0 + acol);
        if (m < 48) *(f32x4*)(As + m * BM + acol) = v;
    }
    auto geom = [&](int m) {
        if (m >= rows) return -1;
        const int img = (m * p.inv_ohw) >> 16, rem = m - img * ohw;
        const int oh = (rem * p.inv_ow) >> 16, ow = rem - oh * p.OW;
        return (img << 16) | ((oh * p.stride - p.pad + 64) << 8) | (ow * p.stride - p.pad + 64);
    };
    int bgeo[6], xgeo[3];
#pragma unroll
    for (int j = 0; j < 6; ++j) bgeo[j] = geom(brow + 8 * j);
#pragma unroll
    for (int nb = 0; nb < 3; ++nb) xgeo[nb] = geom(nb * 16 + fm);
    auto pix_off = [&](int geo, int kh, int kw, bool& ok) -> int {
        const int img = (geo >> 16) & 255, ih = ((geo >> 8) & 255) - 64 + kh, iw = (geo & 255) - 64 + kw;
        ok = geo >= 0 && ih >= 0 && ih < p.H && iw >= 0 && iw < p.W;
        return ok ? ((img * p.H + ih) * p.W + iw) * p.ldi : 0;
    };
    const f32x4 zero4 = {0.f, 0.f, 0.f, 0.f};

    int nkh = 0, nkw = 0, nci0 = 0;
    auto advance = [&]() {
        nci0 += BN;
        if (nci0 == p.Cin) {
            nci0 = 0;
            if (++nkw == p.KW) { nkw = 0; ++nkh; }
        }
    };
    f32x4 vb[6];
    const float* const in_e = p.in + (img0 * p.H * p.W) * p.ldi;
    auto load_b = [&](int kh, int kw, int ci0) {
#pragma unroll
        for (int j = 0; j < 6; ++j) {
            bool ok;
            const int o = pix_off(bgeo[j], kh, kw, ok);
            const f32x4 v = *(const f32x4*)(in_e + (o + ci0 + bcol));
            vb[j] = ok ? v : zero4;
        }
    };
    f32x4 xb[3][2];
    const float* const xn_e = p.xn + (img0 * p.H * p.W) * p.ldi;
    auto load_x = [&](int kh, int kw, int ci0) {
        const int xo = ci0 + 32 * wave + 4 * fq;
#pragma unroll
        for (int nb = 0; nb < 3; ++nb) {
            bool ok;
            const int o = pix_off(xgeo[nb], kh, kw, ok);
#pragma unroll
            for (int j = 0; j < 2; ++j) {
                const f32x4 v = *(const f32x4*)(xn_e + (o + xo + 16 * j));
                xb[nb][j] = ok ? v : zero4;
            }
        }
    };
    const int q = tid & 31, rr = tid >> 5;
    const long long tile_base = (long long)g * p.dwgs + (long long)co0 * p.Kpad;
    float* const wg_ = p.w + tile_base;
    float* const mg_ = p.m + tile_base;
    float* const vg_ = p.v + tile_base;
    const int lo0 = rr * p.Kpad + 4 * q;
    f32x4 am[4], av[4], aw[4], bm[4], bv[4], bw[4];
    auto load_wmv = [&](int kt, f32x4 (&M)[4], f32x4 (&V)[4], f32x4 (&W)[4]) {
#pragma unroll
        for (int u = 0; u < 4; ++u) {
            const int gi = lo0 + 8 * u * p.Kpad + kt * BN;
            M[u] = __builtin_nontemporal_load((const f32x4*)(mg_ + gi));
            V[u] = __builtin_nontemporal_load((const f32x4*)(vg_ + gi));
            W[u] = __builtin_nontemporal_load((const f32x4*)(wg_ + gi));
        }
    };
    load_b(0, 0, 0);
    if (fwd) load_x(0, 0, 0);
    load_wmv(0, am, av, aw);
    if (n_kt > 1) load_wmv(1, bm, bv, bw);
    advance();
    f32x4 accf[3][2];
#pragma unroll
    for (int nb = 0; nb < 3; ++nb)
#pragma unroll
        for (int cb = 0; cb < 2; ++cb) accf[nb][cb] = zero4;
    const float step_size = p.hyper ? p.hyper[0] : p.step_size;
    const float inv_sqrt_bc2 = p.hyper ? p.hyper[1] : p.inv_sqrt_bc2;

    auto tile = [&](int kt, f32x4 (&cm)[4], f32x4 (&cv)[4], f32x4 (&cw)[4]) {
        const bool more = kt + 1 < n_kt;
#pragma unroll
        for (int j = 0; j < 6; ++j) *(f32x4*)(Bs + (brow + 8 * j) * BLD + bcol) = vb[j];
        __syncthreads();
        f32x16 acc;
#pragma unroll
        for (int e = 0; e < 16; ++e) acc[e] = 0.f;
#pragma unroll 1
        for (int t0 = 0; t0 < NT; t0 += 8) {
            const float* ap = As + (2 * t0 + h) * BM + r;
            const float* bp = Bs + (2 * t0 + h) * BLD + wave * 32 + r;
#pragma unroll
            for (int t = 0; t < 8; ++t) acc = __builtin_amdgcn_mfma_f32_32x32x2f32(ap[2 * t * BM], bp[2 * t * BLD], acc, 0, 0, 0);
        }
        if (more) load_b(nkh, nkw, nci0);
#pragma unroll
        for (int e = 0; e < 16; ++e) Gs[((e & 3) + 8 * (e >> 2) + 4 * h) * GLD + wave * 32 + r] = acc[e];
        __syncthreads();
#pragma unroll
        for (int u = 0; u < 4; ++u) {
            const int gi = lo0 + 8 * u * p.Kpad + kt * BN;
            float* gcell = Gs + (rr + 8 * u) * GLD + 4 * q;
            const f32x4 ge = *(const f32x4*)gcell;
            if (FAST) mft_adam4_fast(cm[u], cv[u], cw[u], ge, p.b1, p.b2, p.eps, step_size, inv_sqrt_bc2);
            else mft_adam4_exact(cm[u], cv[u], cw[u], ge, p.b1, p.b2, p.eps, step_size, inv_sqrt_bc2);
            __builtin_nontemporal_store(cm[u], (f32x4*)(mg_ + gi));
            __builtin_nontemporal_store(cv[u], (f32x4*)(vg_ + gi));
            __builtin_nontemporal_store(cw[u], (f32x4*)(wg_ + gi));
            if (p.dw) *(f32x4*)(p.dw + tile_base + gi) = ge;
            if (fwd) *(f32x4*)gcell = cw[u];
        }
        if (fwd) {
            __syncthreads();
#pragma unroll
            for (int j = 0; j < 2; ++j) {
                const f32x4 a0 = *(const f32x4*)(Gs + fm * GLD + 32 * wave + 16 * j + 4 * fq);
                const f32x4 a1 = *(const f32x4*)(Gs + (16 + fm) * GLD + 32 * wave + 16 * j + 4 * fq);
#pragma unroll
                for (int i = 0; i < 4; ++i)
#pragma unroll
                    for (int nb = 0; nb < 3; ++nb) {
                        accf[nb][0] = __builtin_amdgcn_mfma_f32_16x16x4f32(a0[i], xb[nb][j][i], accf[nb][0], 0, 0, 0);
                        accf[nb][1] = __builtin_amdgcn_mfma_f32_16x16x4f32(a1[i], xb[nb][j][i], accf[nb][1], 0, 0, 0);
                    }
            }
            if (more) load_x(nkh, nkw, nci0);
        }
        if (kt + 2 < n_kt) load_wmv(kt + 2, cm, cv, cw);
        advance();
    };
    for (int kt = 0; kt < n_kt; kt += 2) {
        tile(kt, am, av, aw);
        if (kt + 1 < n_kt) tile(kt + 1, bm, bv, bw);
    }
    if (!fwd) return;

    __syncthreads();
    float* Red = smem;
#pragma unroll
    for (int nb = 0; nb < 3; ++nb)
#pragma unroll
        for (int cb = 0; cb < 2; ++cb)
            *(f32x4*)(Red + ((wave * 48 + nb * 16 + fm) * RLD + cb * 16 + 4 * fq)) = accf[nb][cb];
    __syncthreads();
    const int c = tid >> 3, pl = tid & 7;
    float val[6];
#pragma unroll
    for (int i = 0; i < 6; ++i) {
        const int px = pl + 8 * i;
        val[i] = ((Red[(px)*RLD + c] + Red[(48 + px) * RLD + c]) + Red[(96 + px) * RLD + c]) + Red[(144 + px) * RLD + c];
    }
    float* T0 = Gs;
    float* T1 = Gs + 48 * TLD;
    const float inv_rows = 1.f / (float)rows;
    if (MODE == WF_RAW) {
#pragma unroll
        for (int i = 0; i < 6; ++i) T0[(pl + 8 * i) * TLD + c] = val[i];
    } else {
        auto stats = [&](const float* x, float& mu, float& rs) {
            float s = 0.f;
#pragma unroll
            for (int i = 0; i < 6; ++i)
                if (pl + 8 * i < rows) s += x[i];
            mu = lane8_sum(s) * inv_rows;
            s = 0.f;
#pragma unroll
            for (int i = 0; i < 6; ++i)
                if (pl + 8 * i < rows) {
                    const float d = x[i] - mu;
                    s += d * d;
                }
            rs = 1.0f / sqrtf(lane8_sum(s) * inv_rows + p.bn_eps);
        };
        const int co = co0 + c;
        float mu, rs;
        stats(val, mu, rs);
        const float ga = p.gamma[g * p.gbs + co], be = p.beta[g * p.gbs + co];
        if (pl == 0) {
            p.mean[(long long)g * p.Cout + co] = mu;
            p.rstd[(long long)g * p.Cout + co] = rs;
        }
        if (MODE == WF_ENTRY) {
#pragma unroll
            for (int i = 0; i < 6; ++i) {
                T0[(pl + 8 * i) * TLD + c] = val[i];
                T1[(pl + 8 * i) * TLD + c] = fmaxf((val[i] - mu) * rs * ga + be, 0.f);
            }
        } else {
            float sv[6];
#pragma unroll
            for (int i = 0; i < 6; ++i) {
                const int px = pl + 8 * i;
                sv[i] = px < rows ? p.sc[(row0 + px) * p.Cout + co] : 0.f;
            }
            float mus, rss;
            stats(sv, mus, rss);
            const float gas = p.gs[g * p.gbs + co], bes = p.bs[g * p.gbs + co];
            if (pl == 0) {
                p.means[(long long)g * p.Cout + co] = mus;
                p.rstds[(long long)g * p.Cout + co] = rss;
            }
#pragma unroll
            for (int i = 0; i < 6; ++i) {
                float o = (val[i] - mu) * rs * ga + be;
                o += (sv[i] - mus) * rss * gas + bes;
                T0[(pl + 8 * i) * TLD + c] = val[i];
                T1[(pl + 8 * i) * TLD + c] = fmaxf(o, 0.f);
            }
        }
    }
    __syncthreads();
    const int c2 = tid & 31, p2 = tid >> 5;
#pragma unroll
    for (int i = 0; i < 6; ++i) {
        const int px = p2 + 8 * i;
        if (px < rows) {
            p.raw[(row0 + px) * p.Cout + co0 + c2] = T0[px * TLD + c2];
            if (MODE != WF_RAW) p.act[(row0 + px) * p.Cout + co0 + c2] = T1[px * TLD + c2];
        }
    }
    if (MODE == WF_EXIT) {
        const int n_img = rows / p.hw;
        if (p2 < n_img) {
            float sum = 0.f;
            for (int k2 = 0; k2 < p.hw; ++k2) sum += T1[(p2 * p.hw + k2) * TLD + c2];
            p.pooled[((long long)g * n_img + p2) * p.Cout + co0 + c2] = sum * (1.f / (float)p.hw);
        }
    }
}

int g_wf_exact = 0;
int g_wf_xcd = 1;

}

extern "C" void mft_wgrad_fwd_set_exact(int on) { g_wf_exact = on ? 1 : 0; }
extern "C" void mft_wgrad_fwd_set_xcd(int on) { g_wf_xcd = on ? 1 : 0; }

extern "C" int mft_wgrad_adam_next_forward(const float* x, int ldx, const float* dy, int ldy, float* w, float* m, float* v,
                                           float* dw_or_null, int n_img, int H, int W, int Cin, int Cout, int KH, int KW,
                                           int stride, int pad, int imgs_per_group, long long group_stride, int step,
                                           const float* hyper, float lr, float beta1, float beta2, float eps,
                                           const float* x_next, int mode, float* raw, float* act, const float* gamma,
                                           const float* beta, long long gb_group_stride, float* mean, float* rstd,
                                           const float* sc_raw, const float* gamma_s, const float* beta_s, float* mean_s,
                                           float* rstd_s, float* pooled, float bn_eps, void* stream) {
    if (n_img <= 0 || imgs_per_group <= 0 || n_img % imgs_per_group != 0) return MFT_EINVAL;
    if (Cin % 128 != 0 || Cout % 32 != 0 || ldx % 4 != 0 || ldy % 4 != 0) return MFT_EINVAL;
    if (hyper == nullptr && step < 1) return MFT_EINVAL;
    const int OH = (H + 2 * pad - KH) / stride + 1, OW = (W + 2 * pad - KW) / stride + 1;
    const int rows = imgs_per_group * OH * OW;
    if (rows > 48 || OH < 1 || OW < 1 || H > 100 || W > 100 || imgs_per_group > 8) return MFT_EINVAL;
    if (mode < WF_RAW || mode > WF_EXIT) return MFT_EINVAL;
    if (x_next != nullptr) {
        if (raw == nullptr) return MFT_EINVAL;
        if (mode != WF_RAW && (act == nullptr || gamma == nullptr || beta == nullptr || mean == nullptr || rstd == nullptr)) return MFT_EINVAL;
        if (mode == WF_EXIT && (sc_raw == nullptr || gamma_s == nullptr || beta_s == nullptr || mean_s == nullptr || rstd_s == nullptr ||
                                pooled == nullptr)) return MFT_EINVAL;
    }
    WfArgs p = {};
    p.in = x; p.dy = dy; p.dw = dw_or_null; p.w = w; p.m = m; p.v = v;
    p.ldi = ldx; p.ldy = ldy;
    p.H = H; p.W = W; p.Cin = Cin; p.OH = OH; p.OW = OW; p.Cout = Cout; p.KH = KH; p.KW = KW; p.stride = stride; p.pad = pad;
    p.Kpad = KH * KW * Cin;
    p.rows = rows; p.ipg = imgs_per_group;
    p.tiles_ci = Cin / 128;
    p.inv_ohw = (65536 + OH * OW - 1) / (OH * OW);
    p.inv_ow = (65536 + OW - 1) / OW;
    p.mma_rows = rows;
    p.dwgs = group_stride;
    if (hyper != nullptr) step = 1;
    const double bc1 = 1.0 - pow((double)beta1, (double)step);
    const double bc2 = 1.0 - pow((double)beta2, (double)step);
    p.step_size = (float)((double)lr / bc1);
    p.inv_sqrt_bc2 = (float)(1.0 / sqrt(bc2));
    p.b1 = beta1; p.b2 = beta2; p.eps = eps;
    p.hyper = hyper;
    p.xn = x_next; p.raw = raw; p.act = act; p.gamma = gamma; p.beta = beta; p.gbs = gb_group_stride;
    p.mean = mean; p.rstd = rstd; p.sc = sc_raw; p.gs = gamma_s; p.bs = beta_s; p.means = mean_s; p.rstds = rstd_s;
    p.pooled = pooled; p.hw = OH * OW; p.bn_eps = bn_eps;
    const int groups = n_img / imgs_per_group;
    constexpr int lds = (48 * 32 + 48 * (128 + 32) + 32 * (128 + 4)) * 4;
    p.co_blocks = Cout / 32;
    p.xcd_groups = (g_wf_xcd && groups % 8 == 0) ? 1 : 0;
    const dim3 grid((unsigned)(p.co_blocks * groups), 1, 1), block(256);
    hipStream_t s = (hipStream_t)stream;
    const int nt = rows <= 32 ? 16 : 24;
#define WF_LAUNCH2(MODE_, NT_)                                                                            \
    if (g_wf_exact) hipLaunchKernelGGL((wgrad_adam_fwd_kernel<MODE_, false, NT_>), grid, block, lds, s, p);  \
    else hipLaunchKernelGGL((wgrad_adam_fwd_kernel<MODE_, true, NT_>), grid, block, lds, s, p);
#define WF_LAUNCH(MODE_)                                  \
    if (nt == 16) { WF_LAUNCH2(MODE_, 16) }               \
    else { WF_LAUNCH2(MODE_, 24) }
    if (mode == WF_RAW) { WF_LAUNCH(WF_RAW) }
    else if (mode == WF_ENTRY) { WF_LAUNCH(WF_ENTRY) }
    else { WF_LAUNCH(WF_EXIT) }
#undef WF_LAUNCH
#undef WF_LAUNCH2
    return mft_launch_status();
}
```

meta-fine-tuning_amd/functional.py:

```python
import os

import numpy as np

import torch

from . import ops
from . import settings

FUSED_DGRAD = settings.current().fused_dgrad
FUSED_LAST_BLOCK = settings.current().fused_last_block
X3_PLANES = settings.current().x3_planes
X3_FUSED_STATS = settings.current().x3_fused_stats
X3_FOLD_BN = settings.current().x3_fold_bn
TRUNK_F16X2 = settings.current().trunk_f16x2
TRAIN_X3 = settings.current().train_x3
TRAIN_X3_MIN_ROWS = settings.current().train_x3_min_rows
FUSE_NEXT_C2_ONLY = settings.current().fuse_next_c2_only
F16X2_BOUND = 3.0e4
F16X2_FLOOR = 2.0 ** -10
F16X2_MAX_ROWS = 1 << 20


def stem_rows_bound(ipg, image_size):
    oh = (image_size + 6 - 7) // 2 + 1
# ... 417 lines not shown
        c2 = arena.get(tag + ".c2", (n, OH, OH, cout))
        out = arena.get(tag + ".out", (n * OH * OH, cout))
        rc = ops._lib.MFT_EINVAL
        if FUSED_LAST_BLOCK and pooled is not None and c2w.dim() == 3 and groups > ops.SMALL_GROUPS and not so:
            m2, s2, ms, ss = (arena.get(tag + ".bn2." + k, (groups, cout)) for k in ("mean", "rstd", "mean2", "rstd2"))
            rc = ops._lib.lib().mft_block_exit_small_forward(
                ops._p(r1), ops._p(c2w), c2w.shape[1] * c2w.shape[2], ops._p(sc), ops._p(c2), ops._p(out), ops._p(pooled), n, OH,
                OH, cout, ipg, ops._p(g2), ops._p(b2), ops._p(gs), ops._p(bs), gbs, ops._p(m2), ops._p(s2), ops._p(ms),
                ops._p(ss), ops.BN_EPS, ops._stream())
            if rc != ops._lib.MFT_EINVAL:
                ops._lib.check(rc, "mft_block_exit_small_forward")
        if rc == ops._lib.MFT_EINVAL:
            conv(".C2", r1, c2w, 3, 1, 1, c2)
            m2, s2, ms, ss = _bn_small(arena, tag + ".bn2", c2, g2, b2, rows, groups, cout, gbs, out, x2=sc, g2=gs, b2=bs,
                                       pooled=pooled, hw=OH * OH, stats=so.get("bn2"), stats2=so.get("bns"))
        out = out.view(n, OH, OH, cout)
        if tape is not None:
            tape.update(x=x, c1=c1, m1=m1, s1=s1, r1=r1, c2=c2, m2=m2, s2=s2, sc=sc, ms=ms, ss=ss, out=out,
                        pooled=pooled is not None)
        return out
    fuse_stats = (slab is None and running is None and fixed is None and rows >= 128 and X3_FUSED_STATS)

    def conv_bn(name, bnname, inp, wpk, k, s, pd, obuf, stag):
        if fuse_stats and (p + name) in w3:
            H_in = inp.shape[1]
            nws = int(ops._lib.lib().mft_conv2d_x3_stats_ws_floats(n, H_in, H_in, cout, k, k, s, pd))
            ws = arena.get("x3.statws", (max(nws, 1 << 20),)) if nws <= (1 << 20) else arena.get(stag + ".statws", (nws,))
            mean = arena.get(stag + ".mean", (groups, cout))
            rstd = arena.get(stag + ".rstd", (groups, cout))
            r = ops.conv2d_x3_bnstats(inp, w3[p + name], cout, k, k, s, pd, ipg, obuf, ws, mean, rstd)
            if r is not None:
                return r
        o = conv(name, inp, wpk, k, s, pd, obuf)
        mm, ss_ = _bn_stats4(arena, stag, o, ipg, groups, run(p + bnname), fix(p + bnname))
        return o, mm, ss_

    if (X3_FOLD_BN and xp is None and fuse_stats and tape is None and out_mode == "f32"
            and all((p + nm) in w3 for nm in ((".C1", ".C2", ".shortcut") if cin != cout else (".C1", ".C2")))):
        r = _frozen_block_folded(W, p, x, arena, ipg, cin, cout, stride, tag)
        if r is not None:
            return r

    if xp is not None and fuse_stats and tape is None and all((p + nm) in w3 for nm in ((".C1", ".C2", ".shortcut") if cin != cout
                                                                                      else (".C1", ".C2"))):
        def conv_bn_p(name, inp_p, h_in, k, s, pd, obuf, stag):
            nws = int(ops._lib.lib().mft_conv2d_x3_stats_ws_floats(n, h_in, h_in, cout, k, k, s, pd))
            ws = arena.get("x3.statws", (max(nws, 1 << 20),)) if nws <= (1 << 20) else arena.get(stag + ".statws", (nws,))
            mean = arena.get(stag + ".mean", (groups, cout))
            rstd = arena.get(stag + ".rstd", (groups, cout))
            return ops.conv2d_x3p_bnstats(inp_p, n, h_in, h_in, w3[p + name], cout, k, k, s, pd, ipg, obuf, ws, mean, rstd)

        c1, m1, s1 = conv_bn_p(".C1", xp, H, 3, stride, 1, arena.get(tag + ".c1", (n, OH, OH, cout)), tag + ".bn1")
        r1p = arena.get(tag + ".r1p", (3, n * OH * OH, cout), torch.int16)
        ops.bn_apply(c1.view(-1, cout), cout, rows, groups, m1, s1, g1, b1, act=ops.ACT_RELU, fma_affine=True, gb_group_stride=gbs, planes=r1p,
                     write_y=False)
        c2, m2, s2 = conv_bn_p(".C2", r1p, OH, 3, 1, 1, arena.get(tag + ".c2", (n, OH, OH, cout)), tag + ".bn2")
        want_f32 = out_mode in ("f32", "both")
        out = arena.get(tag + ".out", (n * OH * OH, cout)) if want_f32 else None
        outp = arena.get(tag + ".outp", (3, n * OH * OH, cout), torch.int16) if out_mode in ("planes", "both") else None
        if cin != cout:
            sc, ms, ss = conv_bn_p(".shortcut", xp, H, 1, stride, 0, arena.get(tag + ".sc", (n, OH, OH, cout)), tag + ".bns")
            res, res_bn = sc.view(-1, cout), (ms, ss, gs, bs)
        else:
            res, res_bn = x.view(-1, cin), None
        if outp is not None:
            ops.bn_apply(c2.view(-1, cout), cout, rows, groups, m2, s2, g2, b2, act=ops.ACT_RELU, fma_affine=True, res=res, res_bn=res_bn, out=out,
                         gb_group_stride=gbs, planes=outp, write_y=want_f32)
        else:
            ops.bn_apply(c2.view(-1, cout), cout, rows, groups, m2, s2, g2, b2, act=ops.ACT_RELU, fma_affine=True, res=res, res_bn=res_bn, out=out,
                         gb_group_stride=gbs)
        out = out.view(n, OH, OH, cout) if out is not None else None
        return out if out_mode == "f32" else (out, outp)
    assert out_mode == "f32" or xp is None or not fuse_stats, "planes output requested outside the pre-split chain"

    c1, m1, s1 = conv_bn(".C1", ".BN1", x, c1w, 3, stride, 1, arena.get(tag + ".c1", (n, OH, OH, cout)), tag + ".bn1")
    r1 = ops.bn_apply(c1.view(-1, cout), cout, rows, groups, m1, s1, g1, b1, act=ops.ACT_RELU, fma_affine=fuse_stats,
                      out=arena.get(tag + ".r1", (n * OH * OH, cout)), gb_group_stride=gbs).view(n, OH, OH, cout)
    c2, m2, s2 = conv_bn(".C2", ".BN2", r1, c2w, 3, 1, 1, arena.get(tag + ".c2", (n, OH, OH, cout)), tag + ".bn2")
    out = arena.get(tag + ".out", (n * OH * OH, cout))
    sc = ms = ss = None
    if cin != cout:
        sc, ms, ss = conv_bn(".shortcut", ".BNshortcut", x, scw, 1, stride, 0, arena.get(tag + ".sc", (n, OH, OH, cout)),
                             tag + ".bns")
        ops.bn_apply(c2.view(-1, cout), cout, rows, groups, m2, s2, g2, b2, act=ops.ACT_RELU, fma_affine=fuse_stats, res=sc.view(-1, cout),
                     res_bn=(ms, ss, gs, bs), out=out, gb_group_stride=gbs)
    else:
        ops.bn_apply(c2.view(-1, cout), cout, rows, groups, m2, s2, g2, b2, act=ops.ACT_RELU, fma_affine=fuse_stats, res=x.view(-1, cin),
                     out=out, gb_group_stride=gbs)
    out = out.view(n, OH, OH, cout)
    if tape is not None:
        tape.update(x=x, c1=c1, m1=m1, s1=s1, r1=r1, c2=c2, m2=m2, s2=s2, sc=sc, ms=ms, ss=ss, out=out)
    return out


_X3WS_FITS = {}


def _frozen_block_folded(W, p, x, arena, ipg, cin, cout, stride, tag):
    n, H, _, _ = x.shape
    groups = n // ipg
    OH = (H + 2 - 3) // stride + 1
    rows = ipg * OH * OH
    lib = ops._lib.lib()
    fits = _X3WS_FITS.get((cout, rows))
    if fits is None:
        fits = _X3WS_FITS[(cout, rows)] = bool(lib.mft_bn_apply_x3ws_fits(cout, rows, 1))
    if not fits:
        return None
    (g1, b1), (g2, b2) = W.bn[p + ".BN1"], W.bn[p + ".BN2"]
    w3 = W.conv3

    def partials(name, inp, k, s, pd, obuf, stag):
        ws = arena.get(stag + ".statws", (int(lib.mft_conv2d_x3_stats_ws_floats(n, inp.shape[1], inp.shape[1], cout, k, k, s, pd)),))
        r = ops.conv2d_x3_bnstats(inp, w3[p + name], cout, k, k, s, pd, ipg, obuf, ws, None, None)
        return None if r is None else ws

    c1 = arena.get(tag + ".c1", (n, OH, OH, cout))
    ws1 = partials(".C1", x, 3, stride, 1, c1, tag + ".bn1")
    if ws1 is None:
        return None
    c2 = arena.get(tag + ".c2", (n, OH, OH, cout))
    ws2 = arena.get(tag + ".bn2.statws", (int(lib.mft_conv2d_x3_stats_ws_floats(n, OH, OH, cout, 3, 3, 1, 1)),))
    if ops.conv2d_x3_bnin_bnstats(c1, ws1, g1, b1, w3[p + ".C2"], cout, ipg, c2, ws2) is None:
        r1 = ops.bn_apply_x3ws(c1.view(-1, cout), cout, rows, groups, ws1, g1, b1, arena.get(tag + ".r1", (n * OH * OH, cout)),
                               act=ops.ACT_RELU).view(n, OH, OH, cout)
        if ops.conv2d_x3_bnstats(r1, w3[p + ".C2"], cout, 3, 3, 1, 1, ipg, c2, ws2, None, None) is None:
            raise RuntimeError("frozen block %s: C2 outside the bf16x3 domain after C1 was inside it" % p)
    out = arena.get(tag + ".out", (n * OH * OH, cout))
    if cin != cout:
        gs, bs = W.bn[p + ".BNshortcut"]
        sc = arena.get(tag + ".sc", (n, OH, OH, cout))
        wss = partials(".shortcut", x, 1, stride, 0, sc, tag + ".bns")
        if wss is None:
            raise RuntimeError("frozen block %s: shortcut outside the bf16x3 domain after C1 was inside it" % p)
        ops.bn_apply_x3ws(c2.view(-1, cout), cout, rows, groups, ws2, g2, b2, out, act=ops.ACT_RELU, res=sc.view(-1, cout),
                          res_ws=wss, res_gamma=gs, res_beta=bs)
    else:
        ops.bn_apply_x3ws(c2.view(-1, cout), cout, rows, groups, ws2, g2, b2, out, act=ops.ACT_RELU, res=x.view(-1, cin))
    return out.view(n, OH, OH, cout)


def last_block_forward(W, a, arena, ipg, slab=None, tape=None, running=None, tag="f", fixed=None, stats_out=None):
    n = a.shape[0]
    feat = arena.get(tag + ".feat", (n, 512))
    info = tape if tape is not None else {}
    out = simple_block(W, "trunk.7", a, arena, ipg, 256, 512, 2, running, tag + ".trunk.7", slab=slab, tape=info, pooled=feat,
                       fixed=fixed, stats_out=stats_out)
    if not info.get("pooled", False):
        ops._lib.check(ops._lib.lib().mft_global_avgpool(ops._p(out), ops._p(feat), n, out.shape[1] * out.shape[2], 512,
                                                         ops._stream()), "mft_global_avgpool")
    return feat


def resnet10_forward(W, x, arena, ipg=0, slab=None, tape=None, running=None, tag="f", fixed=None):
    n = x.shape[0]
    if ipg <= 0 or fixed is not None:
        ipg = n
    a = resnet10_trunk(W, x, arena, ipg, upto=7, running=running, tag=tag, fixed=fixed)
    return last_block_forward(W, a, arena, ipg, slab=slab, tape=tape, running=running, tag=tag, fixed=fixed)


def _dgrad_c2_bn1(lib, tape, params, grads, arena, tag, dc2, c1, r1, n, oh, ow, C, ipg, bn_bwd):
    rc = ops._lib.MFT_EINVAL
    if FUSED_LAST_BLOCK and n // ipg > ops.SMALL_GROUPS:
        dc1 = arena.get(tag + ".dc1", tuple(c1.shape))
        w2 = params.c2w
        rc = lib.mft_conv2d_dgrad_bn_backward_small(ops._p(dc2), C, ops._p(w2), ops._p(dc1), C, n, oh, ow, C, C, 3, 3, 1, ipg,
                                                    w2.shape[1] * w2.shape[2], ops._p(c1), ops._p(r1), ops._p(tape["m1"]),
                                                    ops._p(tape["s1"]), ops._p(params.bn1g), C, ops._p(grads.bn1g),
                                                    ops._p(grads.bn1b), ops._stream())
        if rc != ops._lib.MFT_EINVAL:
            ops._lib.check(rc, "mft_conv2d_dgrad_bn_backward_small")
    if rc == ops._lib.MFT_EINVAL:
        dr1 = ops.conv2d_dgrad(dc2, params.c2w, 512, 3, 3, 1, imgs_per_group=ipg, out=arena.get(tag + ".dr1", (n, oh, ow, C)))
        dc1 = bn_bwd(c1, dr1, tape["m1"], tape["s1"], params.bn1g, grads.bn1g, grads.bn1b, r1, "dc1")
    return dc1


def next_step_tape(arena, tag, n, oh, ow, C, groups):
    rows = n * oh * ow
    t = {k: arena.get(tag + "." + k, (n, oh, ow, C)) for k in ("c1", "r1", "c2", "sc", "out")}
    for k in ("m1", "s1", "m2", "s2", "ms", "ss"):
        t[k] = arena.get(tag + "." + k, (groups, C))
    t["feat"] = arena.get(tag + ".feat", (n, C))
    t["pooled"] = True
    assert t["c1"].numel() == rows * C
    return t


def last_block_backward(tape, dfeat, params, grads, arena, ipg, tag="bw", adam=None, ce=None, nxt=None, before_next_read=None):
    x, c1, r1, c2, sc, out = tape["x"], tape["c1"], tape["r1"], tape["c2"], tape["sc"], tape["out"]
    n, oh, ow, C = out.shape
    groups = n // ipg
    rows = ipg * oh * ow
    lib = ops._lib.lib()
    fused_ce = FUSED_LAST_BLOCK and ce is not None and C % 64 == 0 and ipg <= 16
    d_out = None
    if fused_ce:
        pass
    elif ce is not None:
        d_out = arena.get(tag + ".dout", (n, oh, ow, C))
        feat, labels, loss = ce
        ops._lib.check(lib.mft_ce_pool_backward(ops._p(feat), ops._p(labels), ipg, groups, C, oh * ow, ops._p(out), ops._p(d_out),
                                                ops._p(loss), ops._stream()), "mft_ce_pool_backward")
    else:
        d_out = arena.get(tag + ".dout", (n, oh, ow, C))
        ops._lib.check(lib.mft_avgpool_relu_backward(ops._p(dfeat), ops._p(out), ops._p(d_out), n, oh * ow, C,
                                                     ops._stream()), "mft_avgpool_relu_backward")

    def bn_bwd(xraw, dy, mean, rstd, gamma, dgamma, dbeta, relu_out, name, need_dx=True):
        dx = arena.get(tag + "." + name, tuple(xraw.shape)) if need_dx else None
        rc = lib.mft_bn_backward(ops._p(xraw), C, ops._p(dy), C, ops._p(relu_out), C, ops._p(dx), C, C, rows, groups,
                                 ops._p(mean), ops._p(rstd), ops._p(gamma), C, ops._p(dgamma), ops._p(dbeta),
                                 ops._stream())
        ops._lib.check(rc, "mft_bn_backward")
        return dx

    def wgrad(xin, dy, name, k, stride, pad):
        if adam is None:
            ops.conv2d_wgrad(xin, dy, 512, k, k, stride, pad, imgs_per_group=ipg, out=getattr(grads, name))
        else:
            m, v, step, lr = adam
            hyper = step if torch.is_tensor(step) else None
            ops.conv2d_wgrad_adam(xin, dy, getattr(params, name), getattr(m, name), getattr(v, name), 512, k, k,
                                  stride, pad, 1 if hyper is not None else step, imgs_per_group=ipg, lr=lr, hyper=hyper)

    if fused_ce:
        feat, labels, loss = ce
        dc2 = arena.get(tag + ".dc2", tuple(c2.shape))
        dsc = arena.get(tag + ".dsc", tuple(sc.shape))
        rc = lib.mft_ce_pool_bn_backward2(ops._p(feat), ops._p(labels), ipg, groups, C, oh * ow, ops._p(out), ops._p(c2), ops._p(sc),
                                          ops._p(dc2), ops._p(dsc), ops._p(tape["m2"]), ops._p(tape["s2"]), ops._p(params.bn2g),
                                          ops._p(tape["ms"]), ops._p(tape["ss"]), ops._p(params.bnsg), C, ops._p(grads.bn2g),
                                          ops._p(grads.bn2b), ops._p(grads.bnsg), ops._p(grads.bnsb), ops._p(loss), ops._stream())
        ops._lib.check(rc, "mft_ce_pool_bn_backward2")
    elif C % 64 == 0:
        dc2 = arena.get(tag + ".dc2", tuple(c2.shape))
        dsc = arena.get(tag + ".dsc", tuple(sc.shape))
        rc = lib.mft_bn_backward2(ops._p(c2), ops._p(sc), C, ops._p(d_out), C, ops._p(dc2), ops._p(dsc), C, C, rows, groups,
                                  ops._p(tape["m2"]), ops._p(tape["s2"]), ops._p(params.bn2g), ops._p(tape["ms"]),
                                  ops._p(tape["ss"]), ops._p(params.bnsg), C, ops._p(grads.bn2g), ops._p(grads.bn2b),
                                  ops._p(grads.bnsg), ops._p(grads.bnsb), ops._stream())
        ops._lib.check(rc, "mft_bn_backward2")
    else:
        dc2 = bn_bwd(c2, d_out, tape["m2"], tape["s2"], params.bn2g, grads.bn2g, grads.bn2b, None, "dc2")
        dsc = bn_bwd(sc, d_out, tape["ms"], tape["ss"], params.bnsg, grads.bnsg, grads.bnsb, None, "dsc")
    done_c2 = False
    if FUSED_DGRAD and FUSED_LAST_BLOCK and adam is not None and rows <= 64 and C % 64 == 0:
        m_, v_, step, lr = adam
        hyper = step if torch.is_tensor(step) else None
        w2 = params.c2w
        dxp = arena.get(tag + ".dxp", (groups, 9, rows, C))
        dc1 = arena.get(tag + ".dc1", tuple(c1.shape))
        if ops.conv2d_wgrad_adam_dgrad(r1, dc2, w2, m_.c2w, v_.c2w, dxp, 1 if hyper is not None else step, ipg, lr=lr,
                                       hyper=hyper):
            ops._lib.check(lib.mft_col2im_bn_backward_small(ops._p(dxp), ops._p(c1), ops._p(r1), ops._p(dc1), n, oh, ow, C, ipg,
                                                            ops._p(tape["m1"]), ops._p(tape["s1"]), ops._p(params.bn1g), C,
                                                            ops._p(grads.bn1g), ops._p(grads.bn1b), ops._stream()),
                           "mft_col2im_bn_backward_small")
            done_c2 = True
    def adam_tail():
        m, v, step, lr = adam
        nb = params.E * 6 * 512
        hyper = step if torch.is_tensor(step) else None
        ops.adam_step(params.flat[-nb:], grads.flat[-nb:], m.flat[-nb:], v.flat[-nb:], 1 if hyper is not None else step,
                      lr=lr, hyper=hyper)

    if before_next_read is not None and (nxt is None or nxt[0] is None):
        raise RuntimeError("before_next_read given, but this call never reads x_next")
    if nxt is not None:
        assert adam is not None and not done_c2
        x_next, tn = nxt[0], nxt[1]
        waited = [before_next_read is None]

        def wait_next_once():
            if not waited[0]:
                before_next_read()
                waited[0] = True
        m_, v_, step, lr = adam
        hyper = step if torch.is_tensor(step) else None
        st = 1 if hyper is not None else step
        dc1 = _dgrad_c2_bn1(lib, tape, params, grads, arena, tag, dc2, c1, r1, n, oh, ow, C, ipg, bn_bwd)
        adam_tail()
        kw = dict(lr=lr, hyper=hyper)
        fw = x_next is not None
        ok = hybrid = False
        if FUSE_NEXT_C2_ONLY and FUSED_LAST_BLOCK and groups > ops.SMALL_GROUPS:
            wgrad(x, dsc, "scw", 1, 2, 0)
            wgrad(x, dc1, "c1w", 3, 2, 1)
            hybrid = ok = True
            if fw:
                wait_next_once()
                rc = lib.mft_block_entry_small_forward(
                    ops._p(x_next), x_next.shape[-1], ops._p(params.c1w), params.c1w.shape[1] * params.c1w.shape[2], ops._p(params.scw),
                    params.scw.shape[1] * params.scw.shape[2], ops._p(tn["c1"]), ops._p(tn["r1"]), ops._p(tn["sc"]), n, x_next.shape[1],
                    x_next.shape[2], x_next.shape[-1], C, 2, ipg, ops._p(params.bn1g), ops._p(params.bn1b), C, ops._p(tn["m1"]),
                    ops._p(tn["s1"]), ops.BN_EPS, ops._stream())
                if rc == ops._lib.MFT_EINVAL:
                    raise RuntimeError("block entry launch outside its domain after next_forward_ok accepted the shape")
                ops._lib.check(rc, "mft_block_entry_small_forward")
        if not hybrid:
            if fw:
                wait_next_once()
            ok = ops.wgrad_adam_next_forward(x, dsc, params.scw, m_.scw, v_.scw, 1, 1, 2, 0, st, ipg, x_next=x_next, mode=ops.WF_RAW,
                                             raw=tn["sc"] if fw else None, **kw)
            ok = ok and ops.wgrad_adam_next_forward(x, dc1, params.c1w, m_.c1w, v_.c1w, 3, 3, 2, 1, st, ipg, x_next=x_next,
                                                    mode=ops.WF_ENTRY, raw=tn["c1"] if fw else None, act=tn["r1"] if fw else None,
                                                    gamma=params.bn1g, beta=params.bn1b, gbs=C, mean=tn["m1"] if fw else None,
                                                    rstd=tn["s1"] if fw else None, **kw)
        ok = ok and ops.wgrad_adam_next_forward(r1, dc2, params.c2w, m_.c2w, v_.c2w, 3, 3, 1, 1, st, ipg,
                                                x_next=tn["r1"] if fw else None, mode=ops.WF_EXIT, raw=tn["c2"] if fw else None,
                                                act=tn["out"] if fw else None, gamma=params.bn2g, beta=params.bn2b, gbs=C,
                                                mean=tn["m2"] if fw else None, rstd=tn["s2"] if fw else None,
                                                sc_raw=tn["sc"] if fw else None, gamma_s=params.bnsg, beta_s=params.bnsb,
                                                mean_s=tn["ms"] if fw else None, rstd_s=tn["ss"] if fw else None,
                                                pooled=tn["feat"] if fw else None, **kw)
        if not ok:
            raise RuntimeError("wgrad_adam_next_forward: shape outside the fused kernel's domain (the caller checks next_forward_ok)")
        assert waited[0] or not fw, "x_next was read without the caller's stream wait"
        if fw:
            tn["x"] = x_next
        return
    if not done_c2:
        dc1 = _dgrad_c2_bn1(lib, tape, params, grads, arena, tag, dc2, c1, r1, n, oh, ow, C, ipg, bn_bwd)
        wgrad(r1, dc2, "c2w", 3, 1, 1)
    wgrad(x, dc1, "c1w", 3, 2, 1)
    wgrad(x, dsc, "scw", 1, 2, 0)
    if adam is not None:
        adam_tail()


def next_forward_ok(ipg, H6):
    oh = (H6 + 2 - 3) // 2 + 1
    return FUSED_LAST_BLOCK and not FUSED_DGRAD and 0 < ipg <= 8 and ipg * oh * oh <= 48



MAX_N_WAY = 32


def check_n_way(n_way):
    if not 1 <= int(n_way) <= MAX_N_WAY:
        raise ValueError("GnnNet head: n_way = %d is not supported (1 <= n_way <= %d: the graph-node rows hold 128 + 96 + n_way "
                         "<= 256 features)" % (int(n_way), MAX_N_WAY))


class GnnHeadWeights:

    def __init__(self, sd, device, n_way):
        check_n_way(n_way)
        self.n_way = n_way
        self.plan = ops.PackPlan()
        n_packed = [0]

        def dev(t):
            return t.detach().to(device=device, dtype=torch.float32).contiguous()

        def packed(src):
            w = dev(src)
            pk = ops.pack_conv_weight(w, rows32=True)
            n_packed[0] += 1
            if w.data_ptr() == src.data_ptr():
                self.plan.add(w, pk)
                pk.wT = torch.zeros((pk.shape[1], ops.round_up(w.shape[0], 32)), device=device, dtype=torch.float32)
                self.plan.add_transposed(w, pk.wT)
                self.has_wT = True
            return pk

        self.fc_w = packed(sd["fc.0.weight"])
        self.fc_b = dev(sd["fc.0.bias"])
        self.fc_g, self.fc_beta = dev(sd["fc.1.weight"]), dev(sd["fc.1.bias"])
        self.wc = {}
        self.gc = {}
        for name in ("layer_w0", "layer_w1", "w_comp_last"):
            layers = []
            for li in range(1, 5):
                w = sd["gnn.%s.conv2d_%d.weight" % (name, li)]
                layers.append((packed(w), dev(sd["gnn.%s.conv2d_%d.bias" % (name, li)]),
                               dev(sd["gnn.%s.bn_%d.weight" % (name, li)]), dev(sd["gnn.%s.bn_%d.bias" % (name, li)]),
                               w.shape[0]))
            last = (packed(sd["gnn.%s.conv2d_last.weight" % name]),
                    dev(sd["gnn.%s.conv2d_last.bias" % name]))
            self.wc[name] = (layers, last)
        for name, bn in (("layer_l0", True), ("layer_l1", True), ("layer_last", False)):
            w = sd["gnn.%s.fc.weight" % name]
            g = b = None
            if bn:
                g, b = dev(sd["gnn.%s.bn.weight" % name]), dev(sd["gnn.%s.bn.bias" % name])
            self.gc[name] = (packed(w), dev(sd["gnn.%s.fc.bias" % name]), g, b, w.shape[0])
        self._n_packed = n_packed[0]
        if getattr(self, "has_wT", False):
            self.plan.run()

    def can_repack(self):
        return len(self.plan.jobs) == self._n_packed * (2 if getattr(self, "has_wT", False) else 1)

    def repack(self):
        assert self.can_repack()
        self.plan.run()


_PAIR_IJ = {}
FUSED_PAIR_MLP = settings.current().fused_pair_mlp
PAIR_F16X2 = settings.current().pair_f16x2
PAIR_MLP_BYTES = int(settings.current().pair_mlp_gb * (1 << 30))


def pair_index_table(N, device):
    key = (N, str(device))
    t = _PAIR_IJ.get(key)
    if t is None:
        import numpy as np
        i, j = np.triu_indices(N)
        t = torch.from_numpy(((i.astype(np.int64) << 16) | j).astype(np.int32)).to(device)
        _PAIR_IJ[key] = t
    return t


def wcompute(G, name, x, F, n_graphs, N, n_groups, arena, tag="wc"):
    if not FUSED_PAIR_MLP:
        return wcompute_unfused(G, name, x, F, n_graphs, N, n_groups, arena, tag)
    layers, (w5, b5) = G.wc[name]
    lib = ops._lib.lib()
    gpg = n_graphs // n_groups
    P = N * (N + 1) // 2
    ij = pair_index_table(N, x.device)
    A = arena.get(tag + ".A", (n_graphs, N, N))
    widths = [l[4] for l in layers]
    per_group = gpg * P * 4 * (widths[0] + widths[1] + widths[3])
    chunk = max(1, min(n_groups, PAIR_MLP_BYTES // max(per_group, 1)))
    tiles_m = int(lib.mft_pair_mlp_tiles_m(gpg, N))
    rows_c = chunk * gpg * P
    hbuf = [arena.get("pm.h%d" % i, (rows_c * w,)) for i, w in ((0, widths[0]), (1, widths[1]), (3, widths[3]))]
    ws_mean = arena.get("pm.wsm", (chunk * tiles_m * 192,))
    ws_m2 = arena.get("pm.wsq", (chunk * tiles_m * 192,))
    ws_n = arena.get("pm.wsn", (chunk * tiles_m,))
    scale = [arena.get("pm.sc%d" % i, (chunk, w)) for i, w in enumerate(widths)]
    shift = [arena.get("pm.sh%d" % i, (chunk, w)) for i, w in enumerate(widths)]
    s_ut = arena.get("pm.s", (rows_c,))
    Kp = ops.round_up(F, 32)
    ld = x.shape[1]
    st = ops._stream
    for g0 in range(0, n_groups, chunk):
        ng = min(chunk, n_groups - g0)
        xin = x[g0 * gpg * N:]
        outs = [hbuf[0], hbuf[1], hbuf[0], hbuf[2]]
        h_in, ld_in, K, Kpad = xin, ld, F, Kp
        for li, (w, b, gam, beta, cout) in enumerate(layers):
            ops._lib.check(lib.mft_pair_mlp_layer(ops._p(h_in), ld_in, 0 if li == 0 else 1, ops._p(ij),
                                                  ops._p(scale[li - 1]) if li else None, ops._p(shift[li - 1]) if li else None,
                                                  ops._p(w), K, Kpad, ops._p(b), ops._p(outs[li]), cout, ng, gpg, N,
                                                  ops.LRELU_SLOPE, ops._p(ws_mean), ops._p(ws_m2), ops._p(ws_n), 1 if PAIR_F16X2 else 0, st()),
                           "mft_pair_mlp_layer")
            ops._lib.check(lib.mft_pair_mlp_stats_finalize(ops._p(ws_mean), ops._p(ws_m2), ops._p(ws_n), ng, tiles_m, cout,
                                                           ops._p(gam), ops._p(beta), ops.BN_EPS, ops._p(scale[li]),
                                                           ops._p(shift[li]), None, None, st()), "mft_pair_mlp_stats_finalize")
            h_in, ld_in, K, Kpad = outs[li], cout, cout, cout
        ops._lib.check(lib.mft_pair_mlp_score(ops._p(h_in), widths[3], ops._p(scale[3]), ops._p(shift[3]), ops._p(w5), ops._p(b5),
                                              ops.LRELU_SLOPE, ops._p(s_ut), ng, gpg, N, st()), "mft_pair_mlp_score")
        ops._lib.check(lib.mft_masked_softmax_ut(ops._p(s_ut), ops._p(A[g0 * gpg:]), ng * gpg, N, st()), "mft_masked_softmax_ut")
    return A


def wcompute_unfused(G, name, x, F, n_graphs, N, n_groups, arena, tag="wc"):
    layers, (w5, b5) = G.wc[name]
    Kp = ops.round_up(F, 32)
    rows = n_graphs * N * N
    rpg = rows // n_groups
    lib = ops._lib.lib()
    d = arena.get(tag + ".d", (rows, Kp))
    ops._lib.check(lib.mft_pair_absdiff(ops._p(x), x.shape[1], ops._p(d), Kp, n_graphs, N, F, ops._stream()),
                   "mft_pair_absdiff")
    h, K = d, Kp
    for li, (w, b, g, beta, cout) in enumerate(layers):
        o = ops.gemm(h, K, w, cout, bias=b, out=arena.get(tag + ".h%d" % li, (rows, cout)))
        m, s = _bn_stats4(arena, tag + ".bn%d" % li, o.view(rows, 1, 1, cout), rpg, n_groups)
        ops.bn_apply(o, cout, rpg, n_groups, m, s, g, beta, act=ops.ACT_LRELU, out=o)
        h, K = o, cout
    sc = ops.gemm(h, K, w5, 1, bias=b5, out=arena.get(tag + ".s", (rows, 1)))
    A = arena.get(tag + ".A", (n_graphs, N, N))
    ops._lib.check(lib.mft_masked_softmax(ops._p(sc), 1, ops._p(A), n_graphs, N, ops._stream()), "mft_masked_softmax")
    return A


def gconv(G, name, A, x, F, n_graphs, N, n_groups, arena, tag="gc"):
    w, b, g, beta, cout = G.gc[name]
    rows = n_graphs * N
    ldy = ops.round_up(2 * F, 32)
    y = arena.get(tag + ".y", (rows, ldy))
    ops._lib.check(ops._lib.lib().mft_graph_aggregate(ops._p(A), ops._p(x), x.shape[1], ops._p(y), ldy, n_graphs, N, F,
                                                      ops._stream()), "mft_graph_aggregate")
    o = ops.gemm(y, ldy, w, cout, bias=b, out=arena.get(tag + ".o", (rows, cout)))
    if g is not None:
        rpg = rows // n_groups
        m, s = _bn_stats4(arena, tag + ".bn", o.view(rows, 1, 1, cout), rpg, n_groups)
        ops.bn_apply(o, cout, rpg, n_groups, m, s, g, beta, act=ops.ACT_NONE, out=o)
    return o


def gnn_forward(G, nodes, n_graphs, N, n_groups, arena, tag="gnn"):
    F = 128 + G.n_way
    x = nodes
    for i in range(2):
        A = wcompute(G, "layer_w%d" % i, x, F, n_graphs, N, n_groups, arena, tag + ".w%d" % i)
        o = gconv(G, "layer_l%d" % i, A, x, F, n_graphs, N, n_groups, arena, tag + ".l%d" % i)
        ops.copy_cols(o, x, F, o.shape[1], act=ops.ACT_LRELU)
        F += o.shape[1]
    A = wcompute(G, "w_comp_last", x, F, n_graphs, N, n_groups, arena, tag + ".wl")
    return gconv(G, "layer_last", A, x, F, n_graphs, N, n_groups, arena, tag + ".ll")


def gnnnet_scores(G, feats, n_episodes, n_way, n_support, n_query, arena, fold=False, tag="head"):
    rows = feats.shape[0]
    rpg = rows // n_episodes
    z = ops.gemm(feats, 512, G.fc_w, 128, bias=G.fc_b, out=arena.get(tag + ".z", (rows, 128)))
    m, s = _bn_stats4(arena, tag + ".fcbn", z.view(rows, 1, 1, 128), rpg, n_episodes)
    ops.bn_apply(z, 128, rpg, n_episodes, m, s, G.fc_g, G.fc_beta, act=ops.ACT_NONE, out=z)
    N = n_way * (n_support + 1)
    n_graphs = n_episodes * n_query
    nodes = arena.get(tag + ".nodes", (n_graphs * N, 256))
    ops._lib.check(ops._lib.lib().mft_build_graph_nodes(ops._p(z), 128, ops._p(nodes), 256, n_episodes, n_way,
                                                        n_support, n_query, 1 if fold else 0, ops._stream()),
                   "mft_build_graph_nodes")
    out = gnn_forward(G, nodes, n_graphs, N, n_episodes, arena, tag + ".gnn")
    return ops.gather_query_scores(out, n_episodes, n_way, n_support, n_query)
```

meta-fine-tuning_amd/ops.py:

```python
import ctypes
import os

import torch

from . import _lib
from . import settings

ACT_NONE, ACT_RELU, ACT_LRELU = 0, 1, 2
BN_EPS = 1e-5
LRELU_SLOPE = 0.01


import threading

_tls = threading.local()


def _stream(t=None):
    dev = getattr(_tls, "dev", None)
    _tls.dev = None
    if t is not None:
        dev = t.device.index if torch.is_tensor(t) else (t.index if isinstance(t, torch.device) else int(t))
    return ctypes.c_void_p(torch.cuda.current_stream(dev).cuda_stream)

# ... 115 lines not shown
            self.table = torch.from_numpy(np.asarray(self.jobs, dtype=np.int64)).to(self.keep[0][0].device)
        _lib.check(_lib.lib().mft_split_bf16x3_multi(_p(self.table), len(self.jobs), self.total, _stream()), "mft_split_bf16x3_multi")

    def run(self):
        if self.jobs:
            self._launch()


def unpack_conv_weight(pk, shape):
    Cout, Cin, KH, KW = shape
    w = torch.empty(shape, device=pk.device, dtype=torch.float32)
    _lib.check(_lib.lib().mft_unpack_oihw(_p(pk), _p(w), Cout, Cin, KH, KW, pk.shape[-1], _stream()), "mft_unpack_oihw")
    return w


def pack_dgrad_weight(w_pk, Cout, Cin, KH, KW, groups=1):
    w_pk = _f32c(w_pk)
    K = KH * KW * Cin
    wt = torch.empty((groups, Cin, KH * KW * Cout), device=w_pk.device, dtype=torch.float32)
    _lib.check(_lib.lib().mft_pack_dgrad(_p(w_pk), _p(wt), Cout, Cin, KH, KW, groups, Cout * K, Cin * KH * KW * Cout,
                                         _stream()), "mft_pack_dgrad")
    return wt



def conv2d(x, w_pk, Cout, KH, KW, stride, pad, imgs_per_group=0, bias=None, out=None):
    _f32c(x)
    n, H, W, Cin = x.shape
    OH = (H + 2 * pad - KH) // stride + 1
    OW = (W + 2 * pad - KW) // stride + 1
    if out is None:
        out = torch.empty((n, OH, OW, Cout), device=x.device, dtype=torch.float32)
    wgs = 0
    if w_pk.dim() == 3:
        wgs = w_pk.shape[1] * w_pk.shape[2]
        if imgs_per_group <= 0 or n // imgs_per_group != w_pk.shape[0]:
            raise RuntimeError("per-group weights need imgs_per_group with n/imgs_per_group == groups")
    if ((wgs == 0 and imgs_per_group <= 0) or (w_pk.dim() == 3 and w_pk.shape[0] == 1)) and Cin != 3:
        nws = _ksplit_ws(n * OH * OW, Cout, w_pk.shape[-1])
        if nws:
            ws = torch.empty((nws,), device=x.device, dtype=torch.float32)
            rc = _lib.lib().mft_conv2d_nhwc_ksplit(_p(x), Cin, _p(w_pk), _p(bias), _p(out), Cout, n, H, W, Cin, Cout, KH, KW,
                                                   stride, pad, _p(ws), _stream())
            _lib.check(rc, "mft_conv2d_nhwc_ksplit")
            return out
    if w_pk.dim() == 3 and 1 < w_pk.shape[0] <= SMALL_GROUPS and bias is None and Cin != 3:
        G = w_pk.shape[0]
        nws = _ksplit_ws(imgs_per_group * OH * OW, Cout, w_pk.shape[-1], G)
        if nws:
            ws = torch.empty((nws,), device=x.device, dtype=torch.float32)
            rc = _lib.lib().mft_conv2d_nhwc_ksplit_grouped(_p(x), Cin, _p(w_pk), _p(out), Cout, n, H, W, Cin, Cout, KH, KW, stride, pad,
                                                           imgs_per_group, wgs, _p(ws), _stream())
            _lib.check(rc, "mft_conv2d_nhwc_ksplit_grouped")
            return out
    rc = _lib.lib().mft_conv2d_nhwc(_p(x), Cin, _p(w_pk), _p(bias), _p(out), Cout, n, H, W, Cin, Cout, KH, KW,
                                    stride, pad, imgs_per_group, wgs, _stream())
    _lib.check(rc, "mft_conv2d_nhwc")
    return out


SMALL_GROUPS = settings.current().small_groups
_KSPLIT_WS = {}


def _ksplit_ws(rows, cols, K, groups=1):
    key = (rows, cols, K, groups)
    v = _KSPLIT_WS.get(key)
    if v is None:
        v = _KSPLIT_WS[key] = int(_lib.lib().mft_conv_ksplit_ws_floats(rows, cols, K) if groups == 1 else
                                  _lib.lib().mft_conv_ksplit_grouped_ws_floats(rows, cols, K, groups))
    return v


def split_weight_x3(w_pk):
    _f32c(w_pk)
    planes = torch.empty((3,) + tuple(w_pk.shape), device=w_pk.device, dtype=torch.int16)
    _lib.check(_lib.lib().mft_split_bf16x3(_p(w_pk), _p(planes), w_pk.numel(), _stream()), "mft_split_bf16x3")
    return planes


def split_weight_h2(w_pk):
    _f32c(w_pk)
    planes = torch.empty((2,) + tuple(w_pk.shape), device=w_pk.device, dtype=torch.int16)
    _lib.check(_lib.lib().mft_split_f16x2(_p(w_pk), _p(planes), w_pk.numel(), _stream()), "mft_split_f16x2")
    return planes


def _x3_fn(w3, stem):
    kind = {3: "x3", 2: "h2"}[int(w3.shape[0])]
    name = "mft_conv2d_nhwc_%s%s" % (kind, stem)
    return getattr(_lib.lib(), name), name


def conv2d_x3(x, w3, Cout, KH, KW, stride, pad, out=None):
    _f32c(x)
    n, H, W, Cin = x.shape
    OH = (H + 2 * pad - KH) // stride + 1
    OW = (W + 2 * pad - KW) // stride + 1
    if out is None:
        out = torch.empty((n, OH, OW, Cout), device=x.device, dtype=torch.float32)
    fn, name = _x3_fn(w3, "")
    rc = fn(_p(x), Cin, _p(w3), w3.shape[1] * w3.shape[2], _p(out), Cout, n, H, W, Cin, Cout, KH, KW, stride, pad, _stream())
    _lib.check(rc, name)
    return out


def conv2d_x3_bnstats(x, w3, Cout, KH, KW, stride, pad, imgs_per_group, out, ws, mean, rstd, eps=BN_EPS):
    _f32c(x)
    n, H, W, Cin = x.shape
    fn, name = _x3_fn(w3, "_bnstats")
    rc = fn(_p(x), Cin, _p(w3), w3.shape[1] * w3.shape[2], _p(out), Cout, n, H, W, Cin, Cout, KH, KW, stride, pad, imgs_per_group, eps,
            _p(ws), _p(mean), _p(rstd), _stream())
    if rc == _lib.MFT_EINVAL:
        return None
    _lib.check(rc, name)
    return out, mean, rstd


def conv2d_x3_bnin_bnstats(c_raw, in_ws, in_gamma, in_beta, w3, Cout, imgs_per_group, out, ws, mean=None, rstd=None, eps=BN_EPS):
    _f32c(c_raw)
    n, H, W, Cin = c_raw.shape
    fn, name = _x3_fn(w3, "_bnin_bnstats")
    rc = fn(_p(c_raw), Cin, _p(in_ws), _p(in_gamma), _p(in_beta), _p(w3), w3.shape[1] * w3.shape[2], _p(out), Cout, n, H, W, Cin, Cout,
            imgs_per_group, eps, _p(ws), _p(mean), _p(rstd), _stream())
    if rc == _lib.MFT_EINVAL:
        return None
    _lib.check(rc, name)
    return out


def bn_apply_x3ws(x2d, C, rows_per_group, n_groups, ws, gamma, beta, out, act=ACT_NONE, res=None, res_ws=None, res_gamma=None,
                  res_beta=None, slope=LRELU_SLOPE, eps=BN_EPS, stats=None, res_stats=None):
    _f32c(x2d)
    m, r = stats if stats is not None else (None, None)
    rm, rr = res_stats if res_stats is not None else (None, None)
    rc = _lib.lib().mft_bn_apply_x3ws(_p(x2d), x2d.shape[-1], _p(out), out.shape[-1], C, rows_per_group, n_groups, _p(ws), _p(gamma),
                                      _p(beta), _p(res), 0 if res is None else res.shape[-1], _p(res_ws), _p(res_gamma),
                                      _p(res_beta), act, slope, eps, _p(m), _p(r), _p(rm), _p(rr), _stream())
    _lib.check(rc, "mft_bn_apply_x3ws")
    return out


def conv2d_x3p_bnstats(xp, n, H, W, w3, Cout, KH, KW, stride, pad, imgs_per_group, out, ws, mean, rstd, eps=BN_EPS):
    Cin = xp.shape[2]
    if w3.shape[0] != 3:
        raise ValueError("pre-split activation planes exist for the bf16x3 kernels only")
    rc = _lib.lib().mft_conv2d_nhwc_x3p_bnstats(_p(xp), xp.shape[1] * Cin, Cin, _p(w3), w3.shape[1] * w3.shape[2], _p(out), Cout,
                                                n, H, W, Cin, Cout, KH, KW, stride, pad, imgs_per_group, eps, _p(ws), _p(mean),
                                                _p(rstd), _stream())
    _lib.check(rc, "mft_conv2d_nhwc_x3p_bnstats")
    return out, mean, rstd


def gemm(a, K, w_pk, N, bias=None, out=None, ldo=None, rows_per_group=0):
    _f32c(a)
    M, lda = a.shape
    if out is None:
        ldo = N if ldo is None else ldo
        out = torch.empty((M, ldo), device=a.device, dtype=torch.float32)
    else:
        ldo = out.shape[1]
    wgs = 0
    if w_pk.dim() == 3:
        wgs = w_pk.shape[1] * w_pk.shape[2]
    rc = _lib.lib().mft_conv2d_nhwc(_p(a), lda, _p(w_pk), _p(bias), _p(out), ldo, M, 1, 1, K, N, 1, 1, 1, 0,
                                    rows_per_group, wgs, _stream())
    _lib.check(rc, "mft_conv2d_nhwc(gemm)")
    return out


def gemm_rk(a, K, w_pk, N, bias=None, out=None, ldo=None):
    _f32c(a)
    M, lda = a.shape
    assert w_pk.dim() == 2 and w_pk.shape[1] == K and w_pk.shape[0] >= N and K % 16 == 0 and K <= 512, (tuple(w_pk.shape), K, N)
    if out is None:
        ldo = N if ldo is None else ldo
        out = torch.empty((M, ldo), device=a.device, dtype=torch.float32)
    else:
        ldo = out.shape[1]
    _lib.check(_lib.lib().mft_gemm_rk(_p(a), lda, _p(w_pk), w_pk.shape[0], K, _p(bias), _p(out), ldo, M, N, _stream()), "mft_gemm_rk")
    return out


def conv2d_dgrad(dy, w_pk, Cin, KH, KW, pad, imgs_per_group=0, out=None, stride=1, in_hw=None):
    _f32c(dy)
    n, OH, OW, Cout = dy.shape
    H, W = (OH, OW) if in_hw is None else in_hw
    if out is None:
        out = torch.empty((n, H, W, Cin), device=dy.device, dtype=torch.float32)
    wgs = w_pk.shape[1] * w_pk.shape[2] if w_pk.dim() == 3 else 0
    if ((wgs == 0 and imgs_per_group <= 0) or (w_pk.dim() == 3 and w_pk.shape[0] == 1)) and Cin % 64 == 0:
        nws = _ksplit_ws(n * H * W, Cin, KH * KW * Cout)
        if nws:
            ws = torch.empty((nws,), device=dy.device, dtype=torch.float32)
            rc = _lib.lib().mft_conv2d_dgrad_nhwc_ksplit(_p(dy), Cout, _p(w_pk), _p(out), Cin, n, H, W, Cin, Cout, KH, KW, stride, pad,
                                                         _p(ws), _stream())
            _lib.check(rc, "mft_conv2d_dgrad_nhwc_ksplit")
            return out
    if w_pk.dim() == 3 and 1 < w_pk.shape[0] <= SMALL_GROUPS and Cin % 64 == 0 and stride == 1 and imgs_per_group > 0:
        nws = _ksplit_ws(imgs_per_group * H * W, Cin, KH * KW * Cout, w_pk.shape[0])
        if nws:
            ws = torch.empty((nws,), device=dy.device, dtype=torch.float32)
            rc = _lib.lib().mft_conv2d_dgrad_nhwc_ksplit_grouped(_p(dy), Cout, _p(w_pk), _p(out), Cin, n, H, W, Cin, Cout, KH, KW, stride,
                                                                 pad, imgs_per_group, wgs, _p(ws), _stream())
            _lib.check(rc, "mft_conv2d_dgrad_nhwc_ksplit_grouped")
            return out
    rc = _lib.lib().mft_conv2d_dgrad_nhwc(_p(dy), Cout, _p(w_pk), _p(out), Cin, n, H, W, Cin, Cout, KH, KW, stride, pad,
                                          imgs_per_group, wgs, _stream())
    _lib.check(rc, "mft_conv2d_dgrad_nhwc")
    return out


def conv2d_wgrad(x, dy, Cout, KH, KW, stride, pad, imgs_per_group=0, out=None, ldy=None):
    _f32c(x)
    _f32c(dy)
    n, H, W, Cin = x.shape
    groups = 1 if imgs_per_group <= 0 else n // imgs_per_group
    K = round_up(KH * KW * Cin, 32)
    if out is None:
        out = torch.empty((groups, Cout, K), device=x.device, dtype=torch.float32)
    nws = int(_lib.lib().mft_conv2d_wgrad_ws_floats(n, H, W, Cin, Cout, KH, KW, stride, pad, imgs_per_group))
    ws = torch.empty((nws,), device=x.device, dtype=torch.float32) if nws > 0 else None
    rc = _lib.lib().mft_conv2d_wgrad_nhwc(_p(x), Cin, _p(dy), dy.shape[-1] if ldy is None else ldy, _p(out), n, H, W,
                                          Cin, Cout, KH, KW, stride, pad, imgs_per_group, Cout * K, _p(ws), _stream())
    _lib.check(rc, "mft_conv2d_wgrad_nhwc")
    return out


def conv2d_wgrad_oihw(x, dy, Cout, KH, KW, stride, pad, cin_valid=0, cout_valid=0, out=None):
    _f32c(x)
    _f32c(dy)
    n, H, W, Cin = x.shape
    if out is None:
        out = torch.empty((cout_valid or Cout, cin_valid or Cin, KH, KW), device=x.device, dtype=torch.float32)
    ws = torch.empty((int(_lib.lib().mft_conv2d_wgrad_oihw_ws_floats(n, H, W, Cin, Cout, KH, KW, stride, pad)),), device=x.device,
                     dtype=torch.float32)
    rc = _lib.lib().mft_conv2d_wgrad_oihw(_p(x), Cin, _p(dy), dy.shape[-1], _p(out), n, H, W, Cin, Cout, KH, KW, stride, pad,
                                          cin_valid, cout_valid, _p(ws), _stream())
    _lib.check(rc, "mft_conv2d_wgrad_oihw")
    return out


class _WgradJob(ctypes.Structure):
    _fields_ = [("inp", ctypes.c_void_p), ("dy", ctypes.c_void_p), ("dw", ctypes.c_void_p), ("ws", ctypes.c_void_p)] + \
               [(n, ctypes.c_int) for n in ("ldi", "ldy", "n_img", "H", "W", "Cin", "Cout", "KH", "KW", "stride", "pad", "cin_valid",
                                            "cout_valid", "reserved")]


class WgradBatch:

    def __init__(self, enabled=True):
        self.enabled = enabled
        self.jobs, self.keep, self.after = [], [], []

    def add(self, x, dy, Cout, KH, KW, stride, pad, cin_valid=0, cout_valid=0):
        if not self.enabled:
            return conv2d_wgrad_oihw(x, dy, Cout, KH, KW, stride, pad, cin_valid, cout_valid)
        _f32c(x)
        _f32c(dy)
        n, H, W, Cin = x.shape
        out = torch.empty((cout_valid or Cout, cin_valid or Cin, KH, KW), device=x.device, dtype=torch.float32)
        ws = torch.empty((int(_lib.lib().mft_conv2d_wgrad_oihw_ws_floats(n, H, W, Cin, Cout, KH, KW, stride, pad)),), device=x.device,
                         dtype=torch.float32)
        self.jobs.append((x.data_ptr(), dy.data_ptr(), out.data_ptr(), ws.data_ptr(), Cin, dy.shape[-1], n, H, W, Cin, Cout, KH, KW, stride,
                          pad, cin_valid, cout_valid, 0))
        self.keep.append((x, dy, out, ws))
        return out

    def then(self, fn):
        if not self.enabled:
            fn()
        else:
            self.after.append(fn)

    def flush(self):
        if self.jobs:
            arr = (_WgradJob * len(self.jobs))(*[_WgradJob(*j) for j in self.jobs])
            dev = self.keep[0][0].device
            _lib.check(_lib.lib().mft_conv2d_wgrad_oihw_multi(arr, len(self.jobs), _stream(dev)), "mft_conv2d_wgrad_oihw_multi")
        for fn in self.after:
            fn()
        self.jobs, self.keep, self.after = [], [], []


def conv2d_wgrad_adam(x, dy, w, m, v, Cout, KH, KW, stride, pad, step, imgs_per_group=0, lr=0.01, beta1=0.9,
                      beta2=0.999, eps=1e-8, dw=None, hyper=None):
    _f32c(x)
    _f32c(dy)
    n, H, W, Cin = x.shape
    K = KH * KW * Cin
    if hyper is not None:
        rc = _lib.lib().mft_conv2d_wgrad_adam_nhwc_dev(_p(x), Cin, _p(dy), Cout, _p(w), _p(m), _p(v), _p(dw), n, H, W, Cin,
                                                       Cout, KH, KW, stride, pad, imgs_per_group, Cout * K, _p(hyper), beta1,
                                                       beta2, eps, _stream())
        _lib.check(rc, "mft_conv2d_wgrad_adam_nhwc_dev")
        return
    rc = _lib.lib().mft_conv2d_wgrad_adam_nhwc(_p(x), Cin, _p(dy), Cout, _p(w), _p(m), _p(v), _p(dw), n, H, W, Cin,
                                               Cout, KH, KW, stride, pad, imgs_per_group, Cout * K, step, lr, beta1,
                                               beta2, eps, _stream())
    _lib.check(rc, "mft_conv2d_wgrad_adam_nhwc")


WF_RAW, WF_ENTRY, WF_EXIT = 0, 1, 2


def wgrad_adam_next_forward(x, dy, w, m, v, KH, KW, stride, pad, step, imgs_per_group, x_next=None, mode=WF_RAW, raw=None, act=None,
                            gamma=None, beta=None, gbs=0, mean=None, rstd=None, sc_raw=None, gamma_s=None, beta_s=None, mean_s=None,
                            rstd_s=None, pooled=None, lr=0.01, beta1=0.9, beta2=0.999, eps=1e-8, dw=None, hyper=None):
    _f32c(x)
    _f32c(dy)
    n, H, W, Cin = x.shape
    Cout = dy.shape[-1]
    rc = _lib.lib().mft_wgrad_adam_next_forward(
        _p(x), Cin, _p(dy), Cout, _p(w), _p(m), _p(v), _p(dw), n, H, W, Cin, Cout, KH, KW, stride, pad, imgs_per_group,
        Cout * KH * KW * Cin, 1 if hyper is not None else step, _p(hyper), lr, beta1, beta2, eps, _p(x_next), mode, _p(raw), _p(act),
        _p(gamma), _p(beta), gbs, _p(mean), _p(rstd), _p(sc_raw), _p(gamma_s), _p(beta_s), _p(mean_s), _p(rstd_s), _p(pooled),
        BN_EPS, _stream())
    if rc == _lib.MFT_EINVAL:
        return False
    _lib.check(rc, "mft_wgrad_adam_next_forward")
    return True


def conv2d_wgrad_adam_dgrad(x, dy, w, m, v, dxp, step, imgs_per_group, lr=0.01, beta1=0.9, beta2=0.999, eps=1e-8, hyper=None):
    n, H, W, Cin = x.shape
    Cout = dy.shape[-1]
    gs = w.shape[1] * w.shape[2]
    if hyper is not None:
        rc = _lib.lib().mft_conv2d_wgrad_adam_dgrad_nhwc_dev(_p(x), Cin, _p(dy), Cout, _p(w), _p(m), _p(v), _p(dxp), n, H, W, Cin,
                                                             Cout, imgs_per_group, gs, _p(hyper), beta1, beta2, eps, _stream())
    else:
        rc = _lib.lib().mft_conv2d_wgrad_adam_dgrad_nhwc(_p(x), Cin, _p(dy), Cout, _p(w), _p(m), _p(v), _p(dxp), n, H, W, Cin, Cout,
                                                         imgs_per_group, gs, step, lr, beta1, beta2, eps, _stream())
    if rc == _lib.MFT_EINVAL:
        return False
    _lib.check(rc, "mft_conv2d_wgrad_adam_dgrad_nhwc")
    return True



def bn_stats(x2d, C, rows_per_group, n_groups, running_mean=None, running_var=None, momentum=0.1, eps=BN_EPS,
             num_batches_tracked=None):
    _f32c(x2d)
    ld = x2d.shape[-1]
    mean = torch.empty((n_groups, C), device=x2d.device, dtype=torch.float32)
    rstd = torch.empty_like(mean)
    nws = _lib.lib().mft_bn_stats_ws_floats(C, rows_per_group, n_groups)
    ws = torch.empty((max(int(nws), 1),), device=x2d.device, dtype=torch.float32)
    rc = _lib.lib().mft_bn_stats(_p(x2d), ld, C, rows_per_group, n_groups, eps, _p(mean), _p(rstd), _p(ws),
                                 _p(running_mean), _p(running_var), momentum, _p(num_batches_tracked), _stream())
    _lib.check(rc, "mft_bn_stats")
    return mean, rstd


BN_AFFINE_FMA = 0x100


def bn_apply(x2d, C, rows_per_group, n_groups, mean, rstd, gamma, beta, act=ACT_NONE, res=None, res_bn=None,
             out=None, gb_group_stride=0, slope=LRELU_SLOPE, planes=None, write_y=True, fma_affine=False):
    _f32c(x2d)
    if fma_affine:
        act = act | BN_AFFINE_FMA
    if out is None and (planes is None or write_y):
        out = torch.empty_like(x2d)
    rm = rr = rg = rb = None
    if res_bn is not None:
        rm, rr, rg, rb = res_bn
    if planes is not None:
        y = out if write_y else None
        rc = _lib.lib().mft_bn_apply_planes(_p(x2d), x2d.shape[-1], _p(y), 0 if y is None else y.shape[-1], _p(planes),
                                            planes.shape[1] * planes.shape[2], C, rows_per_group, n_groups, _p(mean), _p(rstd),
                                            _p(gamma), _p(beta), gb_group_stride, _p(res), 0 if res is None else res.shape[-1],
                                            _p(rm), _p(rr), _p(rg), _p(rb), act, slope, _stream())
        _lib.check(rc, "mft_bn_apply_planes")
        return y
    rc = _lib.lib().mft_bn_apply(_p(x2d), x2d.shape[-1], _p(out), out.shape[-1], C, rows_per_group, n_groups,
                                 _p(mean), _p(rstd), _p(gamma), _p(beta), gb_group_stride,
                                 _p(res), 0 if res is None else res.shape[-1], _p(rm), _p(rr), _p(rg), _p(rb),
                                 act, slope, _stream())
    _lib.check(rc, "mft_bn_apply")
    return out


class _BnStatsJob(ctypes.Structure):
    _fields_ = [(n, ctypes.c_void_p) for n in ("x", "mean", "rstd", "ws", "running_mean", "running_var", "nbt")] + \
               [(n, ctypes.c_int) for n in ("ldx", "C", "rows_per_group", "n_groups")] + [("eps", ctypes.c_float), ("momentum", ctypes.c_float)]


def bn_stats_multi(jobs, momentum=0.1, eps=BN_EPS):
    arr = (_BnStatsJob * len(jobs))()
    out, keep = [], []
    for a, (x, C, rpg, ng, rm, rv, nbt) in zip(arr, jobs):
        _f32c(x)
        mean = torch.empty((ng, C), device=x.device, dtype=torch.float32)
        rstd = torch.empty_like(mean)
        ws = torch.empty((max(int(_lib.lib().mft_bn_stats_ws_floats(C, rpg, ng)), 1),), device=x.device, dtype=torch.float32)
        a.x, a.mean, a.rstd, a.ws = x.data_ptr(), mean.data_ptr(), rstd.data_ptr(), ws.data_ptr()
        a.running_mean = None if rm is None else rm.data_ptr()
        a.running_var = None if rv is None else rv.data_ptr()
        a.nbt = None if nbt is None else nbt.data_ptr()
        a.ldx, a.C, a.rows_per_group, a.n_groups, a.eps, a.momentum = x.shape[-1], C, rpg, ng, eps, momentum
        out.append((mean, rstd))
        keep.append(ws)
    _lib.check(_lib.lib().mft_bn_stats_multi(arr, len(jobs), _stream(jobs[0][0].device)), "mft_bn_stats_multi")
    return out


class _BnFwdJob(ctypes.Structure):
    _fields_ = [(n, ctypes.c_void_p) for n in ("x", "y", "gamma", "beta", "mean", "rstd", "running_mean", "running_var", "nbt", "res",
                                                "res_gamma", "res_beta", "res_mean", "res_rstd", "res_running_mean", "res_running_var",
                                                "res_nbt")] + \
               [(n, ctypes.c_int) for n in ("ldx", "ldy", "ldr", "C", "rows_per_group", "n_groups", "act")] + \
               [(n, ctypes.c_float) for n in ("eps", "momentum", "slope")]


def bn_forward_small_ok(C, rows_per_group):
    return C % 4 == 0 and 0 < rows_per_group <= int(_lib.lib().mft_bn_forward_small_max_rows())


def bn_forward_small(x2d, C, rows_per_group, n_groups, gamma, beta, act=ACT_NONE, running=None, res=None, res_bn=None, out=None,
                     momentum=0.1, eps=BN_EPS, slope=LRELU_SLOPE, out_col=0):
    _f32c(x2d)
    dev = x2d.device
    if out is None:
        out = torch.empty_like(x2d)
    assert out_col >= 0 and out_col + C <= out.shape[-1]
    mean = torch.empty((n_groups, C), device=dev, dtype=torch.float32)
    rstd = torch.empty_like(mean)
    j = _BnFwdJob()
    j.x, j.y, j.gamma, j.beta, j.mean, j.rstd = (t.data_ptr() for t in (x2d, out, gamma, beta, mean, rstd))
    j.y = out.data_ptr() + 4 * out_col
    rm, rv, nbt = running if running is not None else (None, None, None)
    j.running_mean, j.running_var, j.nbt = (None if t is None else t.data_ptr() for t in (rm, rv, nbt))
    rmean = rrstd = None
    if res is not None:
        _f32c(res)
        j.res, j.ldr = res.data_ptr(), res.shape[-1]
        if res_bn is not None:
            rg, rb, rrun = res_bn
            rmean = torch.empty((n_groups, C), device=dev, dtype=torch.float32)
            rrstd = torch.empty_like(rmean)
            j.res_gamma, j.res_beta, j.res_mean, j.res_rstd = rg.data_ptr(), rb.data_ptr(), rmean.data_ptr(), rrstd.data_ptr()
            rrm, rrv, rnbt = rrun if rrun is not None else (None, None, None)
            j.res_running_mean, j.res_running_var, j.res_nbt = (None if t is None else t.data_ptr() for t in (rrm, rrv, rnbt))
    j.ldx, j.ldy, j.C, j.rows_per_group, j.n_groups, j.act = x2d.shape[-1], out.shape[-1], C, rows_per_group, n_groups, act
    j.eps, j.momentum, j.slope = eps, momentum, slope
    _lib.check(_lib.lib().mft_bn_forward_small(ctypes.byref(j), _stream(dev)), "mft_bn_forward_small")
    if rmean is not None:
        return out, mean, rstd, rmean, rrstd
    return out, mean, rstd


class _BnBwdJob(ctypes.Structure):
    _fields_ = [(n, ctypes.c_void_p) for n in ("x", "dy", "y_act", "dx", "mean", "rstd", "gamma", "dgamma", "dbeta", "ws", "dgamma_sum",
                                                "dbeta_sum", "dbias_zero")] + \
               [(n, ctypes.c_int) for n in ("ldx", "lddy", "ldya", "lddx", "C", "rows_per_group", "n_groups", "act")] + \
               [("slope", ctypes.c_float), ("reserved", ctypes.c_int)]


def bn_backward_multi(jobs):
    arr = (_BnBwdJob * len(jobs))()
    out, keep = [], []
    for a, (x, dy, ya, C, rows, groups, mean, rstd, gamma, act) in zip(arr, jobs):
        _f32c(x)
        _f32c(dy)
        dev = x.device
        rpg = rows // groups
        dx = torch.empty_like(x)
        dg, db = torch.empty((C,), device=dev, dtype=torch.float32), torch.empty((C,), device=dev, dtype=torch.float32)
        ws = torch.empty((int(_lib.lib().mft_bn_backward_ws_floats(C, rpg, groups)),), device=dev, dtype=torch.float32)
        a.x, a.dy, a.dx, a.mean, a.rstd, a.gamma, a.ws = (t.data_ptr() for t in (x, dy, dx, mean, rstd, gamma, ws))
        a.y_act = None if ya is None else ya.data_ptr()
        one = groups == 1
        a.dgamma, a.dbeta = (dg.data_ptr(), db.data_ptr()) if one else (None, None)
        a.dgamma_sum, a.dbeta_sum = (None, None) if one else (dg.data_ptr(), db.data_ptr())
        a.dbias_zero = None
        a.ldx, a.lddy, a.ldya, a.lddx = x.shape[-1], dy.shape[-1], 0 if ya is None else ya.shape[-1], dx.shape[-1]
        a.C, a.rows_per_group, a.n_groups, a.act, a.slope = C, rpg, groups, act, LRELU_SLOPE
        out.append((dx, dg, db))
        keep.append(ws)
    _lib.check(_lib.lib().mft_bn_backward_act_multi(arr, len(jobs), _stream(jobs[0][0].device)), "mft_bn_backward_act_multi")
    return out


class _BnApplyJob(ctypes.Structure):
    _fields_ = [(n, ctypes.c_void_p) for n in ("x", "y", "mean", "rstd", "gamma", "beta")] + \
               [(n, ctypes.c_int) for n in ("ldx", "ldy", "C", "rows_per_group", "n_groups", "act")] + [("slope", ctypes.c_float), ("reserved", ctypes.c_int)]


def bn_apply_multi(jobs):
    if not jobs:
        return []
    arr = (_BnApplyJob * len(jobs))()
    for a, (x, C, rpg, ng, mean, rstd, gamma, beta, act, out) in zip(arr, jobs):
        _f32c(x)
        a.x, a.y, a.mean, a.rstd, a.gamma, a.beta = (t.data_ptr() for t in (x, out, mean, rstd, gamma, beta))
        a.ldx, a.ldy, a.C, a.rows_per_group, a.n_groups, a.act, a.slope = x.shape[-1], out.shape[-1], C, rpg, ng, act, LRELU_SLOPE
    _lib.check(_lib.lib().mft_bn_apply_multi(arr, len(jobs), _stream(jobs[0][0].device)), "mft_bn_apply_multi")
    return [j[-1] for j in jobs]


def bn_relu_maxpool(x, mean, rstd, gamma, beta, imgs_per_group=0):
    _f32c(x)
    n, H, W, C = x.shape
    OH, OW = (H + 2 - 3) // 2 + 1, (W + 2 - 3) // 2 + 1
    y = torch.empty((n, OH, OW, C), device=x.device, dtype=torch.float32)
    rc = _lib.lib().mft_bn_relu_maxpool(_p(x), _p(y), n, H, W, C, imgs_per_group, _p(mean), _p(rstd), _p(gamma),
                                        _p(beta), _stream())
    _lib.check(rc, "mft_bn_relu_maxpool")
    return y


def bn_relu_maxpool_gather(cache, src_idx, n_img, mean, rstd, gamma, beta, imgs_per_group, out=None, planes=None):
    _f32c(cache)
    _, H, W, C = cache.shape
    OH, OW = (H + 2 - 3) // 2 + 1, (W + 2 - 3) // 2 + 1
    if out is None:
        out = torch.empty((n_img, OH, OW, C), device=cache.device, dtype=torch.float32)
    if planes is not None:
        rc = _lib.lib().mft_bn_relu_maxpool_gather_planes(_p(cache), _p(src_idx), _p(out), _p(planes),
                                                          planes.shape[1] * planes.shape[2], n_img, H, W, C, imgs_per_group,
                                                          _p(mean), _p(rstd), _p(gamma), _p(beta), _stream())
        _lib.check(rc, "mft_bn_relu_maxpool_gather_planes")
        return out
    rc = _lib.lib().mft_bn_relu_maxpool_gather(_p(cache), _p(src_idx), _p(out), n_img, H, W, C, imgs_per_group, _p(mean),
                                               _p(rstd), _p(gamma), _p(beta), _stream())
    _lib.check(rc, "mft_bn_relu_maxpool_gather")
    return out


def bn_image_moments(x):
    _f32c(x)
    n, H, W, C = x.shape
    mean = torch.empty((n, C), device=x.device, dtype=torch.float32)
    m2 = torch.empty_like(mean)
    _lib.check(_lib.lib().mft_bn_image_moments(_p(x), C, C, H * W, n, _p(mean), _p(m2), _stream()), "mft_bn_image_moments")
    return mean, m2


def bn_combine_moments(mean_img, m2_img, idx_i32, rows_per_img, imgs_per_group, n_groups, mean=None, rstd=None, eps=BN_EPS):
    C = mean_img.shape[1]
    if mean is None:
        mean = torch.empty((n_groups, C), device=mean_img.device, dtype=torch.float32)
        rstd = torch.empty_like(mean)
    rc = _lib.lib().mft_bn_combine_moments(_p(mean_img), _p(m2_img), _p(idx_i32), C, rows_per_img, imgs_per_group,
                                           n_groups, eps, _p(mean), _p(rstd), _stream())
    _lib.check(rc, "mft_bn_combine_moments")
    return mean, rstd


def global_avgpool(x):
    _f32c(x)
    n, H, W, C = x.shape
    y = torch.empty((n, C), device=x.device, dtype=torch.float32)
    _lib.check(_lib.lib().mft_global_avgpool(_p(x), _p(y), n, H * W, C, _stream()), "mft_global_avgpool")
    return y


def avgpool_relu_backward(dfeat, out):
    _f32c(dfeat)
    _f32c(out)
    n, H, W, C = out.shape
    d = torch.empty_like(out)
    _lib.check(_lib.lib().mft_avgpool_relu_backward(_p(dfeat), _p(out), _p(d), n, H * W, C, _stream()),
               "mft_avgpool_relu_backward")
    return d


def bn_backward(x2d, dy2d, C, rows_per_group, n_groups, mean, rstd, gamma, relu_out=None, need_dx=True,
                gb_group_stride=0):
    _f32c(x2d)
    _f32c(dy2d)
    dx = torch.empty_like(x2d) if need_dx else None
    dg = torch.empty((n_groups, C), device=x2d.device, dtype=torch.float32)
    db = torch.empty_like(dg)
    rc = _lib.lib().mft_bn_backward(_p(x2d), x2d.shape[-1], _p(dy2d), dy2d.shape[-1], _p(relu_out),
                                    0 if relu_out is None else relu_out.shape[-1], _p(dx),
                                    0 if dx is None else dx.shape[-1], C, rows_per_group, n_groups, _p(mean), _p(rstd),
                                    _p(gamma), gb_group_stride, _p(dg), _p(db), _stream())
    _lib.check(rc, "mft_bn_backward")
    return dx, dg, db



def cross_entropy(logits, labels_i32, rows_per_group, n_groups, need_grad=True):
    _f32c(logits)
    rows, C = logits.shape
    buf = torch.empty((n_groups + rows,), device=logits.device, dtype=torch.float32)
    d = torch.empty_like(logits) if need_grad else None
    rc = _lib.lib().mft_cross_entropy(_p(logits), C, _p(labels_i32), C, rows_per_group, n_groups, _p(buf), _p(d),
                                      _stream())
    _lib.check(rc, "mft_cross_entropy")
    return buf[:n_groups], d


def softmax_rows(x):
    _f32c(x)
    rows, C = x.shape
    y = torch.empty_like(x)
    _lib.check(_lib.lib().mft_softmax_rows(_p(x), C, _p(y), C, C, rows, _stream()), "mft_softmax_rows")
    return y


def _proto_check(feats, episodes, n_way, n_support, n_query):
    _f32c(feats)
    if feats.dim() != 2 or feats.shape[0] != episodes * n_way * (n_support + n_query):
        raise ValueError("ProtoNet head: feats %s is not [episodes*n_way*(n_support+n_query) = %d, D]"
                         % (tuple(feats.shape), episodes * n_way * (n_support + n_query)))


def proto_scores(feats, episodes, n_way, n_support, n_query, softmax=False, out=None):
    _proto_check(feats, episodes, n_way, n_support, n_query)
    D = feats.shape[1]
    rows = episodes * n_way * n_query
    if out is not None and (tuple(out.shape) != (rows, n_way) or not out.is_contiguous()):
        raise ValueError("proto_scores: out must be a contiguous [%d, %d] tensor" % (rows, n_way))
    y = out if out is not None else torch.empty((rows, n_way), device=feats.device, dtype=torch.float32)
    _lib.check(_lib.lib().mft_proto_scores(_p(feats), feats.stride(0), episodes, n_way, n_support, n_query, D, _p(y),
                                           1 if softmax else 0, _stream()), "mft_proto_scores")
    return y


def proto_backward(feats, dscores, episodes, n_way, n_support, n_query, out=None):
# ... 100 lines not shown
```

meta-fine-tuning_amd/settings.py:

```python
import dataclasses
import os


def _flag(v):
    lv = v.strip().lower()
    if lv in ("1", "true", "yes", "on"):
        return True
    if lv in ("0", "false", "no", "off"):
        return False
    raise ValueError("expected 0 / 1 (or true / false), got %r" % (v,))


def _opt_int(v):
    return None if v in ("", "none", "None") else int(v)


def _fuse(v):
    if v not in ("auto", "0", "1"):
        raise ValueError("expected auto, 0 or 1, got %r" % (v,))
    return v


KNOBS = (
    ("fuse_next", "MFT_FUSE_NEXT", _fuse, "auto", "fused weight-gradient + Adam + next-step forward launches: auto = engine.fuse_next_policy | 1 | 0"),
    ("wf_xcd", "MFT_WF_XCD", _flag, True, "fused launch: all workgroups of an episode on one XCD (A/B hook; read once per process)"),
    ("slab_candidates", "MFT_SLAB_CANDIDATES", _opt_int, None, "candidate buffers of the w/m/v placement scan (None: engine default 12; 0: off)"),
    ("slab_ballast_gb", "MFT_SLAB_BALLAST_GB", float, 12.0, "throw-away allocation between groups of placement candidates, GB"),
    ("slab_hints", "MFT_SLAB_HINTS", _flag, True, "re-use an earlier scan's placement when one probe confirms it"),
    ("trunk_chunk", "MFT_TRUNK_CHUNK", _opt_int, None, "inner steps per frozen-trunk launch set (None: 32 at E = 1, else 1)"),
    ("trunk_priority", "MFT_TRUNK_PRIORITY", int, 1, "HIP priority of the frozen-trunk stream (1 = the device's least)"),
    ("last_priority", "MFT_LAST_PRIORITY", int, -1, "torch priority of the last-block stream"),
    ("trunk_cus_per_xcd", "MFT_TRUNK_CUS_PER_XCD", int, 0, "CU-masked streams: CUs per XCD for the trunk stream (0 = no partition; measured slower)"),
    ("trunk_cus_only", "MFT_TRUNK_CUS_ONLY", _flag, False, "with trunk_cus_per_xcd: confine only the trunk stream"),
    ("debug_skip_trunk", "MFT_DEBUG_SKIP_TRUNK", _flag, False, "measurement aid: reuse one cached trunk output (results are WRONG)"),
    ("adapt_graph", "MFT_ADAPT_GRAPH", _flag, True, "adapt_last_block: replay the meta-fine-tuning inner loop from one hipGraph"),
    ("adapt_batched_trunk", "MFT_ADAPT_BATCHED_TRUNK", _flag, True, "adapt_last_block: frozen trunk of all steps as two grouped passes"),
    ("fused_dgrad", "MFT_FUSED_DGRAD", _flag, False, "one-pass trunk.7.C2 weight gradient + Adam + data gradient (measured slower in the step)"),
    ("x3_planes", "MFT_X3_PLANES", _flag, False, "trunk activations pre-split into bf16x3 planes (measured slower)"),
    ("x3_fused_stats", "MFT_X3_FUSED_STATS", _flag, True, "BatchNorm statistics from the split-precision convolution epilogue"),
    ("x3_fold_bn", "MFT_X3_FOLD_BN", _flag, True, "frozen blocks without helper launches (per-tile partials merged by the consumers)"),
    ("trunk_f16x2", "MFT_TRUNK_F16X2", _flag, True, "frozen trunk.4-6 on two fp16 pieces per operand (0: three bf16 pieces)"),
    ("fuse_next_c2_only", "MFT_FUSE_NEXT_C2_ONLY", _flag, False, "only trunk.7.C2's launch fused (measured slower)"),
    ("stem_pooled", "MFT_STEM_POOLED", _flag, True, "stem cache keeps per-window (max, min) instead of the full-resolution output"),
    ("stem_fused_fill", "MFT_STEM_FUSED_FILL", _flag, True, "stem cache filled by ONE launch (convolution + moments + window min/max; 0: three launches through a full-resolution buffer)"),
    ("stem_chunk", "MFT_STEM_CHUNK", _opt_int, None, "images per stem-cache fill launch (None: StemCache's default)"),
    ("fused_last_block", "MFT_FUSED_LAST_BLOCK", _flag, True, "conv + BatchNorm fusions of the adapted block (csrc/skinny.hip)"),
    ("small_groups", "MFT_SMALL_GROUPS", int, 12, "up to this many per-episode weight sets take the K-sliced GEMM route"),
    ("fused_pair_mlp", "MFT_FUSED_PAIR_MLP", _flag, True, "Wcompute on the fused upper-triangle pair-MLP kernels"),
    ("pair_mlp_gb", "MFT_PAIR_MLP_GB", float, 6.0, "memory budget of the fused pair-MLP's hidden activations per chunk, GB"),
    ("train_graph", "MFT_TRAIN_GRAPH", _flag, True, "MetaTemplate episode loop: loss + backward replayed from one hipGraph"),
    ("train_x3", "MFT_TRAIN_X3", _flag, True, "meta-training: 3x3 layers with >= 8192 output rows on the bf16x3 kernels, forward and stride-1 data gradient (0: fp32 MFMA everywhere)"),
    ("train_x3_min_rows", "MFT_TRAIN_X3_MIN_ROWS", int, 6000, "meta-training: output rows from which a 3x3 layer takes the bf16x3 kernels (below: fp32 MFMA with K slices; measured at 3,780 / 945 rows in profiles/r06_q_train_x3_min_rows.txt)"),
    ("wgrad_batch", "MFT_WGRAD_BATCH", _flag, True, "meta-training backward: every layer's weight gradient deferred to the end of the pass and run in one multi-problem launch pair per 16 layers (0: one launch pair per layer, as round 5; bit-identical)"),
    ("pair_f16x2", "MFT_PAIR_F16X2", _flag, False, "GNN pair-MLP layers (Wcompute) as f16x2 products on the fp16 matrix cores (fp32-accurate; 0: fp32 MFMA)"),
    ("gemm_rk_rows", "MFT_GEMM_RK_ROWS", int, 4096, "meta-training: head linear layers (fc, Gconv.fc) of at most this many rows take the skinny register-K GEMM (0: the tile kernel always)"),
    ("pair_rk_rows", "MFT_PAIR_RK_ROWS", int, 16384, "meta-training: Wcompute layers over at most this many pair rows (all episodes of the step) take the register-K small-problem kernel, 32-row tiles, no LDS staging (0: the 128-row tile kernel always)"),
    ("train_source", "MFT_TRAIN_SOURCE", str, "pool", "train.main --dataset miniImageNet: 'pool' = resident uint8 class pool, 'synthetic' = host fp32 episodes"),
    ("standin_weights", "MFT_STANDIN_WEIGHTS", _flag, False, "allow synthetic stand-in weights when no checkpoint is found (explicit opt-in)"),
    ("image_size", "MFT_IMAGE_SIZE", int, 84, "image side the CLI evaluates at (84 = BASELINE; 224 = the reference's)"),
    ("episodes", "MFT_EPISODES", _opt_int, None, "override of the CLI's episode count (None: 600)"),
    ("episodes_per_batch", "MFT_EPISODES_PER_BATCH", _opt_int, None, "override of the CLI's lockstep batch (None: 128 / 96 / 64 by n_shot)"),
    ("timings", "MFT_TIMINGS", _flag, False, "print the drivers' phase timings to stderr"),
    ("pool_per_class", "MFT_POOL_PER_CLASS", _opt_int, None, "images per class of the dataset-shaped resident pool (None: the dataset's)"),
    ("synth_on_host", "MFT_SYNTH_ON_HOST", _flag, False, "generate synthetic test episodes with numpy on the host instead of on the device"),
    ("balance_batches", "MFT_BALANCE_BATCHES", _flag, True, "equalise the lockstep batch sizes of an evaluation"),
    ("force_collectives", "MFT_FORCE_COLLECTIVES", _flag, False, "run the N-rank collectives even with one rank (1-GPU RCCL tests)"),
    ("one_device", "MFT_ONE_DEVICE", _flag, False, "test hook: W ranks share device 0, gloo for the gathers"),
)


@dataclasses.dataclass(frozen=True)
class Settings:
    fuse_next: str = "auto"
    wf_xcd: bool = True
    slab_candidates: "int | None" = None
    slab_ballast_gb: float = 12.0
    slab_hints: bool = True
    trunk_chunk: "int | None" = None
    trunk_priority: int = 1
    last_priority: int = -1
    trunk_cus_per_xcd: int = 0
    trunk_cus_only: bool = False
    debug_skip_trunk: bool = False
    adapt_graph: bool = True
    adapt_batched_trunk: bool = True
    fused_dgrad: bool = False
    x3_planes: bool = False
    x3_fused_stats: bool = True
    x3_fold_bn: bool = True
    trunk_f16x2: bool = True
    fuse_next_c2_only: bool = False
    stem_pooled: bool = True
    stem_fused_fill: bool = True
    stem_chunk: "int | None" = None
    fused_last_block: bool = True
    small_groups: int = 12
    fused_pair_mlp: bool = True
    pair_mlp_gb: float = 6.0
    train_graph: bool = True
    train_x3: bool = True
    train_x3_min_rows: int = 6000
    wgrad_batch: bool = True
    pair_f16x2: bool = False
    gemm_rk_rows: int = 4096
    pair_rk_rows: int = 16384
    train_source: str = "pool"
    standin_weights: bool = False
    image_size: int = 84
    episodes: "int | None" = None
    episodes_per_batch: "int | None" = None
    timings: bool = False
    pool_per_class: "int | None" = None
    synth_on_host: bool = False
    balance_batches: bool = True
    force_collectives: bool = False
    one_device: bool = False

    @classmethod
    def from_env(cls, env=None):
        env = os.environ if env is None else env
        kw = {}
        for field, var, parse, default, _ in KNOBS:
            raw = env.get(var)
            if raw is None:
                kw[field] = default
                continue
            try:
                kw[field] = parse(raw)
            except (TypeError, ValueError) as e:
                raise ValueError("%s=%r: %s" % (var, raw, e)) from None
        s = cls(**kw)
        if s.train_source not in ("pool", "synthetic"):
            raise ValueError("MFT_TRAIN_SOURCE=%r: expected pool or synthetic" % (s.train_source,))
        if s.image_size < 32 or not 0 <= s.trunk_cus_per_xcd < 32:
            raise ValueError("MFT_IMAGE_SIZE / MFT_TRUNK_CUS_PER_XCD out of range")
        return s


assert tuple(f.name for f in dataclasses.fields(Settings)) == tuple(k[0] for k in KNOBS), "KNOBS and Settings fields must match"
_VARS = tuple(k[1] for k in KNOBS)
_cache = (None, None)


def current():
    global _cache
    key = tuple(os.environ.get(v) for v in _VARS)
    if _cache[0] != key:
        _cache = (key, Settings.from_env())
    return _cache[1]


IMPORT_TIME = frozenset((
    "debug_skip_trunk", "adapt_graph", "adapt_batched_trunk", "fused_dgrad", "fused_last_block", "x3_planes", "x3_fused_stats",
    "x3_fold_bn", "trunk_f16x2", "train_x3", "train_x3_min_rows", "fuse_next_c2_only", "fused_pair_mlp", "pair_f16x2", "pair_rk_rows", "gemm_rk_rows", "pair_mlp_gb", "wgrad_batch",
    "train_graph", "small_groups", "wf_xcd",
))
assert IMPORT_TIME <= set(k[0] for k in KNOBS), IMPORT_TIME - set(k[0] for k in KNOBS)


def describe():
    return "\n".join("%-26s %-22s %-7s default %-8r %s" % (var, field, "import" if field in IMPORT_TIME else "live", default, doc)
                     for field, var, _, default, doc in KNOBS)
```

Before: 88.91.

## Run fused wgrad+Adam+forward as persistent workgroups, pairing shortcut and C1

Adds a persistent-workgroup version of the fused weight-gradient + Adam + next-step forward kernel. Each workgroup walks several (episode, output-channel block) items and prefetches the next item's activations, dy and Adam state during the tail of the current one. The shortcut and C1 layers now share one pair launch, and C2 uses the persistent mode, which cuts launch count and pipeline fill/drain. This costs register pressure and more kernel complexity, and falls back to the old three launches when the shapes are outside the supported domain.

```diff
diff --git a/include/mft_hip.h b/include/mft_hip.h
--- a/include/mft_hip.h
+++ b/include/mft_hip.h
@@ -161,6 +161,18 @@
                                 float* pooled, float bn_eps, void* stream);
 
 
+typedef struct MftWfLayer {
+    const float* x; const float* dy; float* w; float* m; float* v; float* dw_or_null;
+    const float* x_next; float* raw; float* act; const float* gamma; const float* beta; float* mean; float* rstd;
+    const float* sc_raw; const float* gamma_s; const float* beta_s; float* mean_s; float* rstd_s; float* pooled;
+    long long group_stride, gb_group_stride;
+    int ldx, ldy, H, W, Cin, Cout, KH, KW, stride, pad, mode;
+} MftWfLayer;
+int mft_wgrad_adam_next_forward_pair(const MftWfLayer* raw_layer, const MftWfLayer* entry_layer, int n_img, int imgs_per_group,
+                                     int step, const float* hyper, float lr, float beta1, float beta2, float eps, float bn_eps,
+                                     void* stream);
+
+
 long long mft_bn_stats_ws_floats(int C, int rows_per_group, int n_groups);
 int mft_bn_stats(const float* x, int ldx, int C, int rows_per_group, int n_groups, float eps,
                  float* mean, float* rstd, float* ws,
diff --git a/include/mft_hip_testing.h b/include/mft_hip_testing.h
--- a/include/mft_hip_testing.h
+++ b/include/mft_hip_testing.h
@@ -9,6 +9,7 @@
 int mft_debug_reset(void);
 void mft_wgrad_fwd_set_exact(int on);
 void mft_wgrad_fwd_set_xcd(int on);
+void mft_wgrad_fwd_set_grid_cap(int workgroups);
 
 #ifdef __cplusplus
 }
diff --git a/meta-fine-tuning_amd/_lib.py b/meta-fine-tuning_amd/_lib.py
--- a/meta-fine-tuning_amd/_lib.py
+++ b/meta-fine-tuning_amd/_lib.py
@@ -54,6 +54,7 @@
     "mft_pack_oihw_multi": [_P, _I, _L, _P],
     "mft_wgrad_adam_next_forward": [_P, _I, _P, _I, _P, _P, _P, _P, _I, _I, _I, _I, _I, _I, _I, _I, _I, _I, _L, _I, _P, _F, _F, _F,
                                     _F, _P, _I, _P, _P, _P, _P, _L, _P, _P, _P, _P, _P, _P, _P, _P, _F, _P],
+    "mft_wgrad_adam_next_forward_pair": [_P, _P, _I, _I, _I, _P, _F, _F, _F, _F, _F, _P],
     "mft_bn_stats_ws_floats": [_I, _I, _I],
     "mft_bn_stats": [_P, _I, _I, _I, _I, _F, _P, _P, _P, _P, _P, _F, _P, _P],
     "mft_bn_apply": [_P, _I, _P, _I, _I, _I, _I, _P, _P, _P, _P, _L, _P, _I, _P, _P, _P, _P, _I, _F, _P],
@@ -151,6 +152,7 @@
     "mft_debug_reset": [],
     "mft_wgrad_fwd_set_exact": [_I],
     "mft_wgrad_fwd_set_xcd": [_I],
+    "mft_wgrad_fwd_set_grid_cap": [_I],
 }
 _RESTYPE = {"mft_conv2d_x3_stats_ws_floats": _L, "mft_bn_stats_ws_floats": _L, "mft_conv2d_wgrad_ws_floats": _L, "mft_bn_backward_ws_floats": _L,
             "mft_conv2d_wgrad_adam_dgrad_ws_floats": _L, "mft_pair_bwd_stats_ws_floats": _L, "mft_conv_ksplit_ws_floats": _L, "mft_conv2d_wgrad_oihw_ws_floats": _L, "mft_conv_ksplit_grouped_ws_floats": _L}
diff --git a/meta-fine-tuning_amd/csrc/conv_igemm.hip b/meta-fine-tuning_amd/csrc/conv_igemm.hip
--- a/meta-fine-tuning_amd/csrc/conv_igemm.hip
+++ b/meta-fine-tuning_amd/csrc/conv_igemm.hip
@@ -1241,6 +1241,7 @@
 extern "C" int mft_debug_reset(void) {
     mft_wgrad_fwd_set_exact(0);
     mft_wgrad_fwd_set_xcd(1);
+    mft_wgrad_fwd_set_grid_cap(0);
     g_dgrad_parity = 1; g_wgrad_trim = 1; g_wgrad_rows = 1; g_wgrad_tile = 64; g_conv_tile = 0; g_wgrad_pol = 7; g_wgrad_early = 1; g_wgrad_min_lds_kb = 0; g_skinny = 1; g_stem_fast = 1; g_stem_wgrad_strips = 1;
     mft_skinny_set_lines(1); mft_skinny_set_nw(0); mft_skinny_set_x3(1); mft_skinny_set_tap(1); mft_skinny_set_dgrad_slices(1);
     mft_debug_set_x3_tile(0); mft_debug_set_x3_tile(10); mft_debug_set_x3_tile(21); mft_debug_set_x3_tile(31); mft_debug_set_x3_tile(41);
diff --git a/meta-fine-tuning_amd/csrc/wgrad_fwd.hip b/meta-fine-tuning_amd/csrc/wgrad_fwd.hip
--- a/meta-fine-tuning_amd/csrc/wgrad_fwd.hip
+++ b/meta-fine-tuning_amd/csrc/wgrad_fwd.hip
@@ -1,5 +1,6 @@
 #include "mft_common.h"
 #include <math.h>
+#include <type_traits>
 
 namespace {
 
@@ -28,7 +29,7 @@
     int xcd_groups;
 };
 
-enum { WF_RAW = 0, WF_ENTRY = 1, WF_EXIT = 2 };
+enum { WF_RAW = 0, WF_ENTRY = 1, WF_EXIT = 2, WF_PERSISTENT = 4 };
 
 __device__ __forceinline__ float lane8_sum(float v) {
     v += __shfl_xor(v, 1, 64);
@@ -304,6 +305,371 @@
     }
 }
 
+struct WfRegs {
+    f32x4 am[4], av[4], aw[4], bm[4], bv[4], bw[4];
+    f32x4 vb[6];
+    f32x4 xb[3][2];
+    f32x4 dyr[2];
+    int nkh, nkw, nci0;
+};
+
+struct WfPersistArgs {
+    WfArgs a, b;
+    int n_items;
+    int per_xcd;
+};
+
+__device__ __forceinline__ int wf_tid() {
+    int t = threadIdx.x;
+    asm volatile("" : "+v"(t));
+    return t;
+}
+
+__device__ __forceinline__ int wf_geom(const WfArgs& p, int m) {
+    if (m >= p.rows) return -1;
+    const int ohw = p.OH * p.OW;
+    const int img = (m * p.inv_ohw) >> 16, rem = m - img * ohw;
+    const int oh = (rem * p.inv_ow) >> 16, ow = rem - oh * p.OW;
+    return (img << 16) | ((oh * p.stride - p.pad + 64) << 8) | (ow * p.stride - p.pad + 64);
+}
+
+__device__ __forceinline__ int wf_pix_off(const WfArgs& p, int geo, int kh, int kw, bool& ok) {
+    const int img = (geo >> 16) & 255, ih = ((geo >> 8) & 255) - 64 + kh, iw = (geo & 255) - 64 + kw;
+    ok = geo >= 0 && ih >= 0 && ih < p.H && iw >= 0 && iw < p.W;
+    return ok ? ((img * p.H + ih) * p.W + iw) * p.ldi : 0;
+}
+
+__device__ __forceinline__ void wf_load_b(const WfArgs& p, int g, int tid, WfRegs& R) {
+    const int bcol = (tid & 31) * 4;
+    const float* const in_e = p.in + ((long long)g * p.ipg * p.H * p.W) * p.ldi;
+    const f32x4 zero4 = {0.f, 0.f, 0.f, 0.f};
+#pragma unroll
+    for (int j = 0; j < 6; ++j) {
+        bool ok;
+        const int o = wf_pix_off(p, wf_geom(p, (tid >> 5) + 8 * j), R.nkh, R.nkw, ok);
+        const f32x4 v = *(const f32x4*)(in_e + (o + R.nci0 + bcol));
+        R.vb[j] = ok ? v : zero4;
+    }
+}
+
+__device__ __forceinline__ void wf_load_x(const WfArgs& p, int g, int tid, WfRegs& R) {
+    const int lane = tid & 63, wave = tid >> 6, fq = lane >> 4;
+    const float* const xn_e = p.xn + ((long long)g * p.ipg * p.H * p.W) * p.ldi;
+    const int xo = R.nci0 + 32 * wave + 4 * fq;
+    const f32x4 zero4 = {0.f, 0.f, 0.f, 0.f};
+#pragma unroll
+    for (int nb = 0; nb < 3; ++nb) {
+        bool ok;
+        const int o = wf_pix_off(p, wf_geom(p, nb * 16 + (tid & 15)), R.nkh, R.nkw, ok);
+#pragma unroll
+        for (int j = 0; j < 2; ++j) {
+            const f32x4 v = *(const f32x4*)(xn_e + (o + xo + 16 * j));
+            R.xb[nb][j] = ok ? v : zero4;
+        }
+    }
+}
+
+__device__ __forceinline__ void wf_load_wmv(const WfArgs& p, int g, int co0, int tid, int kt, f32x4 (&M)[4], f32x4 (&V)[4], f32x4 (&W)[4]) {
+    const long long tile_base = (long long)g * p.dwgs + (long long)co0 * p.Kpad;
+    const int lo0 = (tid >> 5) * p.Kpad + 4 * (tid & 31);
+#pragma unroll
+    for (int u = 0; u < 4; ++u) {
+        const int gi = lo0 + 8 * u * p.Kpad + kt * 128;
+        M[u] = __builtin_nontemporal_load((const f32x4*)(p.m + tile_base + gi));
+        V[u] = __builtin_nontemporal_load((const f32x4*)(p.v + tile_base + gi));
+        W[u] = __builtin_nontemporal_load((const f32x4*)(p.w + tile_base + gi));
+    }
+}
+
+__device__ __forceinline__ void wf_open_rows(const WfArgs& p, int g, int tid, WfRegs& R) {
+    R.nkh = 0; R.nkw = 0; R.nci0 = 0;
+    wf_load_b(p, g, tid, R);
+}
+
+__device__ __forceinline__ void wf_load_dy(const WfArgs& p, int g, int co0, int tid, WfRegs& R) {
+    const int arow = tid >> 3, acol = (tid & 7) * 4;
+#pragma unroll
+    for (int j = 0; j < 2; ++j) {
+        const int m = arow + 32 * j;
+        f32x4 v = {0.f, 0.f, 0.f, 0.f};
+        if (m < p.rows) v = *(const f32x4*)(p.dy + ((long long)g * p.rows + m) * p.ldy + co0 + acol);
+        R.dyr[j] = v;
+    }
+}
+
+__device__ __forceinline__ void wf_store_dy(const WfRegs& R, int tid, float* As) {
+    const int arow = tid >> 3, acol = (tid & 7) * 4;
+#pragma unroll
+    for (int j = 0; j < 2; ++j) {
+        const int m = arow + 32 * j;
+        if (m < 48) *(f32x4*)(As + m * 32 + acol) = R.dyr[j];
+    }
+}
+
+__device__ __forceinline__ void wf_advance(const WfArgs& p, WfRegs& R) {
+    R.nci0 += 128;
+    if (R.nci0 == p.Cin) {
+        R.nci0 = 0;
+        if (++R.nkw == p.KW) { R.nkw = 0; ++R.nkh; }
+    }
+}
+
+template <int MODE, bool FAST, int NT>
+__device__ __forceinline__ void wf_walk(const WfArgs& p, const WfArgs& pn, const int g, const int co0, const bool has_next,
+                                        const int gn, const int con0, WfRegs& R, float* smem) {
+    constexpr int BM = 32, BN = 128, BLD = BN + 32, GLD = BN + 4, RLD = 36, TLD = 33;
+    float* As = smem;
+    float* Bs = smem + 48 * BM;
+    float* Gs = Bs + 48 * BLD;
+    const int tid = wf_tid(), lane = tid & 63, wave = tid >> 6;
+    const int r = lane & 31, h = lane >> 5;
+    const int fm = lane & 15, fq = lane >> 4;
+    const int rows = p.rows;
+    const long long row0 = (long long)g * rows;
+    const int n_kt = p.KH * p.KW * p.tiles_ci;
+    const bool fwd = p.xn != nullptr;
+    const int brow = tid >> 5, bcol = (tid & 31) * 4;
+    const int q = tid & 31, rr = tid >> 5;
+    const long long tile_base = (long long)g * p.dwgs + (long long)co0 * p.Kpad;
+    float* const wg_ = p.w + tile_base;
+    float* const mg_ = p.m + tile_base;
+    float* const vg_ = p.v + tile_base;
+    const int lo0 = rr * p.Kpad + 4 * q;
+    const f32x4 zero4 = {0.f, 0.f, 0.f, 0.f};
+    f32x4 accf[3][2];
+#pragma unroll
+    for (int nb = 0; nb < 3; ++nb)
+#pragma unroll
+        for (int cb = 0; cb < 2; ++cb) accf[nb][cb] = zero4;
+    const float step_size = p.hyper ? p.hyper[0] : p.step_size;
+    const float inv_sqrt_bc2 = p.hyper ? p.hyper[1] : p.inv_sqrt_bc2;
+    int tid_s = tid;
+    float ga = 0.f, be = 0.f, gas = 0.f, bes = 0.f, sv[6];
+
+    auto tile = [&](auto pos, int kt, f32x4 (&cm)[4], f32x4 (&cv)[4], f32x4 (&cw)[4]) {
+        constexpr int POS = decltype(pos)::value;
+        constexpr bool more = POS != 2;
+#pragma unroll
+        for (int j = 0; j < 6; ++j) *(f32x4*)(Bs + (brow + 8 * j) * BLD + bcol) = R.vb[j];
+        __syncthreads();
+        f32x16 acc;
+#pragma unroll
+        for (int e = 0; e < 16; ++e) acc[e] = 0.f;
+#pragma unroll 1
+        for (int t0 = 0; t0 < NT; t0 += 8) {
+            const float* ap = As + (2 * t0 + h) * BM + r;
+            const float* bp = Bs + (2 * t0 + h) * BLD + wave * 32 + r;
+#pragma unroll
+            for (int t = 0; t < 8; ++t) acc = __builtin_amdgcn_mfma_f32_32x32x2f32(ap[2 * t * BM], bp[2 * t * BLD], acc, 0, 0, 0);
+        }
+        if (more) wf_load_b(p, g, wf_tid(), R);
+        else if (has_next) wf_open_rows(pn, gn, tid_s, R);
+#pragma unroll
+        for (int e = 0; e < 16; ++e) Gs[((e & 3) + 8 * (e >> 2) + 4 * h) * GLD + wave * 32 + r] = acc[e];
+        __syncthreads();
+#pragma unroll
+        for (int u = 0; u < 4; ++u) {
+            const int gi = lo0 + 8 * u * p.Kpad + kt * BN;
+            float* gcell = Gs + (rr + 8 * u) * GLD + 4 * q;
+            const f32x4 ge = *(const f32x4*)gcell;
+            if (FAST) mft_adam4_fast(cm[u], cv[u], cw[u], ge, p.b1, p.b2, p.eps, step_size, inv_sqrt_bc2);
+            else mft_adam4_exact(cm[u], cv[u], cw[u], ge, p.b1, p.b2, p.eps, step_size, inv_sqrt_bc2);
+            __builtin_nontemporal_store(cm[u], (f32x4*)(mg_ + gi));
+            __builtin_nontemporal_store(cv[u], (f32x4*)(vg_ + gi));
+            __builtin_nontemporal_store(cw[u], (f32x4*)(wg_ + gi));
+            if (p.dw) *(f32x4*)(p.dw + tile_base + gi) = ge;
+            if (fwd) *(f32x4*)gcell = cw[u];
+        }
+        if (fwd) {
+            __syncthreads();
+#pragma unroll
+            for (int j = 0; j < 2; ++j) {
+                const f32x4 a0 = *(const f32x4*)(Gs + fm * GLD + 32 * wave + 16 * j + 4 * fq);
+                const f32x4 a1 = *(const f32x4*)(Gs + (16 + fm) * GLD + 32 * wave + 16 * j + 4 * fq);
+#pragma unroll
+                for (int i = 0; i < 4; ++i)
+#pragma unroll
+                    for (int nb = 0; nb < 3; ++nb) {
+                        accf[nb][0] = __builtin_amdgcn_mfma_f32_16x16x4f32(a0[i], R.xb[nb][j][i], accf[nb][0], 0, 0, 0);
+                        accf[nb][1] = __builtin_amdgcn_mfma_f32_16x16x4f32(a1[i], R.xb[nb][j][i], accf[nb][1], 0, 0, 0);
+                    }
+            }
+            if (more) wf_load_x(p, g, wf_tid(), R);
+            else {
+                if (has_next) wf_load_x(pn, gn, tid_s, R);
+                if (MODE != WF_RAW) {
+                    const int c = tid_s >> 3, pl = tid_s & 7;
+                    const int co = co0 + c;
+                    ga = p.gamma[g * p.gbs + co];
+                    be = p.beta[g * p.gbs + co];
+                    if (MODE == WF_EXIT) {
+                        gas = p.gs[g * p.gbs + co];
+                        bes = p.bs[g * p.gbs + co];
+#pragma unroll
+                        for (int i = 0; i < 6; ++i) {
+                            const int px = pl + 8 * i;
+                            sv[i] = px < rows ? p.sc[(row0 + px) * p.Cout + co] : 0.f;
+                        }
+                    }
+                }
+            }
+        }
+        if (POS == 0) wf_load_wmv(p, g, co0, tid, kt + 2, cm, cv, cw);
+        else if (has_next) wf_load_wmv(pn, gn, con0, tid_s, POS - 1, cm, cv, cw);
+        if (more) wf_advance(p, R);
+        else if (has_next) {
+            wf_load_dy(pn, gn, con0, tid_s, R);
+            wf_advance(pn, R);
+        } else {
+            R.dyr[0] = zero4;
+            R.dyr[1] = zero4;
+        }
+    };
+#pragma unroll 1
+    for (int kt = 0; kt < n_kt - 2; kt += 2) {
+        tile(std::integral_constant<int, 0>(), kt, R.am, R.av, R.aw);
+        tile(std::integral_constant<int, 0>(), kt + 1, R.bm, R.bv, R.bw);
+    }
+    tid_s = wf_tid();
+    tile(std::integral_constant<int, 1>(), n_kt - 2, R.am, R.av, R.aw);
+    tile(std::integral_constant<int, 2>(), n_kt - 1, R.bm, R.bv, R.bw);
+    __syncthreads();
+    if (!fwd) {
+        if (has_next) wf_store_dy(R, tid_s, As);
+        return;
+    }
+    float* Red = smem;
+#pragma unroll
+    for (int nb = 0; nb < 3; ++nb)
+#pragma unroll
+        for (int cb = 0; cb < 2; ++cb)
+            *(f32x4*)(Red + ((wave * 48 + nb * 16 + fm) * RLD + cb * 16 + 4 * fq)) = accf[nb][cb];
+    __syncthreads();
+    const int c = tid_s >> 3, pl = tid_s & 7;
+    float val[6];
+#pragma unroll
+    for (int i = 0; i < 6; ++i) {
+        const int px = pl + 8 * i;
+        val[i] = ((Red[(px)*RLD + c] + Red[(48 + px) * RLD + c]) + Red[(96 + px) * RLD + c]) + Red[(144 + px) * RLD + c];
+    }
+    float* T0 = Gs;
+    float* T1 = Gs + 48 * TLD;
+    const float inv_rows = 1.f / (float)rows;
+    if (MODE == WF_RAW) {
+#pragma unroll
+        for (int i = 0; i < 6; ++i) T0[(pl + 8 * i) * TLD + c] = val[i];
+    } else {
+        auto stats = [&](const float* x, float& mu, float& rs) {
+            float s = 0.f;
+#pragma unroll
+            for (int i = 0; i < 6; ++i)
+                if (pl + 8 * i < rows) s += x[i];
+            mu = lane8_sum(s) * inv_rows;
+            s = 0.f;
+#pragma unroll
+            for (int i = 0; i < 6; ++i)
+                if (pl + 8 * i < rows) {
+                    const float d = x[i] - mu;
+                    s += d * d;
+                }
+            rs = 1.0f / sqrtf(lane8_sum(s) * inv_rows + p.bn_eps);
+        };
+        const int co = co0 + c;
+        float mu, rs;
+        stats(val, mu, rs);
+        if (pl == 0) {
+            p.mean[(long long)g * p.Cout + co] = mu;
+            p.rstd[(long long)g * p.Cout + co] = rs;
+        }
+        if (MODE == WF_ENTRY) {
+#pragma unroll
+            for (int i = 0; i < 6; ++i) {
+                T0[(pl + 8 * i) * TLD + c] = val[i];
+                T1[(pl + 8 * i) * TLD + c] = fmaxf((val[i] - mu) * rs * ga + be, 0.f);
+            }
+        } else {
+            float mus, rss;
+            stats(sv, mus, rss);
+            if (pl == 0) {
+                p.means[(long long)g * p.Cout + co] = mus;
+                p.rstds[(long long)g * p.Cout + co] = rss;
+            }
+#pragma unroll
+            for (int i = 0; i < 6; ++i) {
+                float o = (val[i] - mu) * rs * ga + be;
+                o += (sv[i] - mus) * rss * gas + bes;
+                T0[(pl + 8 * i) * TLD + c] = val[i];
+                T1[(pl + 8 * i) * TLD + c] = fmaxf(o, 0.f);
+            }
+        }
+    }
+    __syncthreads();
+    if (has_next) wf_store_dy(R, tid_s, As);
+    const int c2 = tid_s & 31, p2 = tid_s >> 5;
+#pragma unroll
+    for (int i = 0; i < 6; ++i) {
+        const int px = p2 + 8 * i;
+        if (px < rows) {
+            p.raw[(row0 + px) * p.Cout + co0 + c2] = T0[px * TLD + c2];
+            if (MODE != WF_RAW) p.act[(row0 + px) * p.Cout + co0 + c2] = T1[px * TLD + c2];
+        }
+    }
+    if (MODE == WF_EXIT) {
+        const int n_img = rows / p.hw;
+        if (p2 < n_img) {
+            float sum = 0.f;
+            for (int k2 = 0; k2 < p.hw; ++k2) sum += T1[(p2 * p.hw + k2) * TLD + c2];
+            p.pooled[((long long)g * n_img + p2) * p.Cout + co0 + c2] = sum * (1.f / (float)p.hw);
+        }
+    }
+}
+
+__device__ __forceinline__ bool wf_item(const WfPersistArgs& q, int k, int& g, int& co0) {
+    const int cb = q.a.co_blocks;
+    if (q.a.xcd_groups) {
+        const int xcd = blockIdx.x & 7, i = (blockIdx.x >> 3) + k * (gridDim.x >> 3);
+        if (i >= q.per_xcd) return false;
+        g = (i / cb) * 8 + xcd;
+        co0 = (i % cb) * 32;
+    } else {
+        const int i = blockIdx.x + k * gridDim.x;
+        if (i >= q.n_items) return false;
+        g = i / cb;
+        co0 = (i % cb) * 32;
+    }
+    return true;
+}
+
+template <int M0, int M1, bool FAST, int NT>
+__global__ __launch_bounds__(256) __attribute__((amdgpu_waves_per_eu(2, 2))) void wgrad_adam_fwd_persistent_kernel(WfPersistArgs q) {
+    extern __shared__ __attribute__((aligned(16))) float smem[];
+    int g, co0;
+    if (!wf_item(q, 0, g, co0)) return;
+    WfRegs R;
+    const int tid = threadIdx.x;
+    wf_open_rows(q.a, g, tid, R);
+    wf_load_dy(q.a, g, co0, tid, R);
+    if (q.a.xn != nullptr) wf_load_x(q.a, g, tid, R);
+    wf_load_wmv(q.a, g, co0, tid, 0, R.am, R.av, R.aw);
+    wf_load_wmv(q.a, g, co0, tid, 1, R.bm, R.bv, R.bw);
+    wf_advance(q.a, R);
+    wf_store_dy(R, tid, smem);
+#pragma unroll 1
+    for (int k = 1;; ++k) {
+        int gn = 0, con0 = 0;
+        const bool nx = wf_item(q, k, gn, con0);
+        if (M1 >= 0) {
+            wf_walk<M0, FAST, NT>(q.a, q.b, g, co0, true, g, co0, R, smem);
+            wf_walk<(M1 >= 0 ? M1 : 0), FAST, NT>(q.b, q.a, g, co0, nx, gn, con0, R, smem);
+        } else {
+            wf_walk<M0, FAST, NT>(q.a, q.a, g, co0, nx, gn, con0, R, smem);
+        }
+        if (!nx) break;
+        g = gn;
+        co0 = con0;
+    }
+}
+
 int g_wf_exact = 0;
 int g_wf_xcd = 1;
 
@@ -312,14 +678,12 @@
 extern "C" void mft_wgrad_fwd_set_exact(int on) { g_wf_exact = on ? 1 : 0; }
 extern "C" void mft_wgrad_fwd_set_xcd(int on) { g_wf_xcd = on ? 1 : 0; }
 
-extern "C" int mft_wgrad_adam_next_forward(const float* x, int ldx, const float* dy, int ldy, float* w, float* m, float* v,
-                                           float* dw_or_null, int n_img, int H, int W, int Cin, int Cout, int KH, int KW,
-                                           int stride, int pad, int imgs_per_group, long long group_stride, int step,
-                                           const float* hyper, float lr, float beta1, float beta2, float eps,
-                                           const float* x_next, int mode, float* raw, float* act, const float* gamma,
-                                           const float* beta, long long gb_group_stride, float* mean, float* rstd,
-                                           const float* sc_raw, const float* gamma_s, const float* beta_s, float* mean_s,
-                                           float* rstd_s, float* pooled, float bn_eps, void* stream) {
+static int wf_make_args(WfArgs& p, const float* x, int ldx, const float* dy, int ldy, float* w, float* m, float* v, float* dw_or_null,
+                        int n_img, int H, int W, int Cin, int Cout, int KH, int KW, int stride, int pad, int imgs_per_group,
+                        long long group_stride, int step, const float* hyper, float lr, float beta1, float beta2, float eps,
+                        const float* x_next, int mode, float* raw, float* act, const float* gamma, const float* beta,
+                        long long gb_group_stride, float* mean, float* rstd, const float* sc_raw, const float* gamma_s,
+                        const float* beta_s, float* mean_s, float* rstd_s, float* pooled, float bn_eps) {
     if (n_img <= 0 || imgs_per_group <= 0 || n_img % imgs_per_group != 0) return MFT_EINVAL;
     if (Cin % 128 != 0 || Cout % 32 != 0 || ldx % 4 != 0 || ldy % 4 != 0) return MFT_EINVAL;
     if (hyper == nullptr && step < 1) return MFT_EINVAL;
@@ -333,7 +697,7 @@
         if (mode == WF_EXIT && (sc_raw == nullptr || gamma_s == nullptr || beta_s == nullptr || mean_s == nullptr || rstd_s == nullptr ||
                                 pooled == nullptr)) return MFT_EINVAL;
     }
-    WfArgs p = {};
+    p = WfArgs{};
     p.in = x; p.dy = dy; p.dw = dw_or_null; p.w = w; p.m = m; p.v = v;
     p.ldi = ldx; p.ldy = ldy;
     p.H = H; p.W = W; p.Cin = Cin; p.OH = OH; p.OW = OW; p.Cout = Cout; p.KH = KH; p.KW = KW; p.stride = stride; p.pad = pad;
@@ -355,9 +719,90 @@
     p.mean = mean; p.rstd = rstd; p.sc = sc_raw; p.gs = gamma_s; p.bs = beta_s; p.means = mean_s; p.rstds = rstd_s;
     p.pooled = pooled; p.hw = OH * OW; p.bn_eps = bn_eps;
     const int groups = n_img / imgs_per_group;
-    constexpr int lds = (48 * 32 + 48 * (128 + 32) + 32 * (128 + 4)) * 4;
     p.co_blocks = Cout / 32;
     p.xcd_groups = (g_wf_xcd && groups % 8 == 0) ? 1 : 0;
+    return 0;
+}
+
+namespace {
+
+int g_wf_grid_cap = 0;
+
+int wf_resident_workgroups() {
+    if (g_wf_grid_cap > 0) return g_wf_grid_cap;
+    static int cus = 0;
+    if (cus == 0) {
+        int dev = 0;
+        hipDeviceProp_t prop;
+        if (hipGetDevice(&dev) != hipSuccess || hipGetDeviceProperties(&prop, dev) != hipSuccess) return 0;
+        cus = prop.multiProcessorCount;
+    }
+    return 2 * cus;
+}
+
+int wf_args_of(WfArgs& p, const MftWfLayer& d, int n_img, int imgs_per_group, int step, const float* hyper, float lr, float beta1,
+               float beta2, float eps, float bn_eps) {
+    return wf_make_args(p, d.x, d.ldx, d.dy, d.ldy, d.w, d.m, d.v, d.dw_or_null, n_img, d.H, d.W, d.Cin, d.Cout, d.KH, d.KW, d.stride,
+                        d.pad, imgs_per_group, d.group_stride, step, hyper, lr, beta1, beta2, eps, d.x_next, d.mode, d.raw, d.act,
+                        d.gamma, d.beta, d.gb_group_stride, d.mean, d.rstd, d.sc_raw, d.gamma_s, d.beta_s, d.mean_s, d.rstd_s,
+                        d.pooled, bn_eps);
+}
+
+template <int M0, int M1>
+int wf_launch_persistent(const WfPersistArgs& q, hipStream_t s) {
+    const int resident = wf_resident_workgroups();
+    if (resident <= 0) return MFT_EINVAL;
+    int wgs = q.n_items < resident ? q.n_items : resident;
+    if (q.a.xcd_groups) wgs &= ~7;
+    if (wgs <= 0) return MFT_EINVAL;
+    constexpr int lds = (48 * 32 + 48 * (128 + 32) + 32 * (128 + 4)) * 4;
+    const dim3 grid((unsigned)wgs, 1, 1), block(256);
+    const bool nt16 = q.a.rows <= 32;
+    if (g_wf_exact) {
+        if (nt16) hipLaunchKernelGGL((wgrad_adam_fwd_persistent_kernel<M0, M1, false, 16>), grid, block, lds, s, q);
+        else hipLaunchKernelGGL((wgrad_adam_fwd_persistent_kernel<M0, M1, false, 24>), grid, block, lds, s, q);
+    } else {
+        if (nt16) hipLaunchKernelGGL((wgrad_adam_fwd_persistent_kernel<M0, M1, true, 16>), grid, block, lds, s, q);
+        else hipLaunchKernelGGL((wgrad_adam_fwd_persistent_kernel<M0, M1, true, 24>), grid, block, lds, s, q);
+    }
+    return mft_launch_status();
+}
+
+bool wf_even_tiles(const WfArgs& p) { return (p.KH * p.KW * p.tiles_ci) % 2 == 0; }
+
+}
+
+
+extern "C" int mft_wgrad_adam_next_forward(const float* x, int ldx, const float* dy, int ldy, float* w, float* m, float* v,
+                                           float* dw_or_null, int n_img, int H, int W, int Cin, int Cout, int KH, int KW,
+                                           int stride, int pad, int imgs_per_group, long long group_stride, int step,
+                                           const float* hyper, float lr, float beta1, float beta2, float eps,
+                                           const float* x_next, int mode, float* raw, float* act, const float* gamma,
+                                           const float* beta, long long gb_group_stride, float* mean, float* rstd,
+                                           const float* sc_raw, const float* gamma_s, const float* beta_s, float* mean_s,
+                                           float* rstd_s, float* pooled, float bn_eps, void* stream) {
+    const bool persistent = mode >= 0 && (mode & WF_PERSISTENT) != 0;
+    if (persistent) mode &= ~WF_PERSISTENT;
+    WfArgs p;
+    const int rc = wf_make_args(p, x, ldx, dy, ldy, w, m, v, dw_or_null, n_img, H, W, Cin, Cout, KH, KW, stride, pad, imgs_per_group,
+                                group_stride, step, hyper, lr, beta1, beta2, eps, x_next, mode, raw, act, gamma, beta, gb_group_stride,
+                                mean, rstd, sc_raw, gamma_s, beta_s, mean_s, rstd_s, pooled, bn_eps);
+    if (rc != 0) return rc;
+    const int rows = p.rows;
+    const int groups = n_img / imgs_per_group;
+    if (persistent) {
+        if (!wf_even_tiles(p)) return MFT_EINVAL;
+        WfPersistArgs q = {};
+        q.a = p;
+        q.b = p;
+        q.n_items = groups * p.co_blocks;
+        q.per_xcd = q.n_items / 8;
+        hipStream_t ps = (hipStream_t)stream;
+        if (mode == WF_RAW) return wf_launch_persistent<WF_RAW, -1>(q, ps);
+        if (mode == WF_ENTRY) return wf_launch_persistent<WF_ENTRY, -1>(q, ps);
+        return wf_launch_persistent<WF_EXIT, -1>(q, ps);
+    }
+    constexpr int lds = (48 * 32 + 48 * (128 + 32) + 32 * (128 + 4)) * 4;
     const dim3 grid((unsigned)(p.co_blocks * groups), 1, 1), block(256);
     hipStream_t s = (hipStream_t)stream;
     const int nt = rows <= 32 ? 16 : 24;
@@ -374,3 +819,22 @@
 #undef WF_LAUNCH2
     return mft_launch_status();
 }
+
+extern "C" void mft_wgrad_fwd_set_grid_cap(int workgroups) { g_wf_grid_cap = workgroups > 0 ? workgroups : 0; }
+
+extern "C" int mft_wgrad_adam_next_forward_pair(const MftWfLayer* raw_layer, const MftWfLayer* entry_layer, int n_img,
+                                                int imgs_per_group, int step, const float* hyper, float lr, float beta1,
+                                                float beta2, float eps, float bn_eps, void* stream) {
+    if (raw_layer == nullptr || entry_layer == nullptr) return MFT_EINVAL;
+    if (raw_layer->mode != WF_RAW || entry_layer->mode != WF_ENTRY) return MFT_EINVAL;
+    WfPersistArgs q = {};
+    int rc = wf_args_of(q.a, *raw_layer, n_img, imgs_per_group, step, hyper, lr, beta1, beta2, eps, bn_eps);
+    if (rc != 0) return rc;
+    rc = wf_args_of(q.b, *entry_layer, n_img, imgs_per_group, step, hyper, lr, beta1, beta2, eps, bn_eps);
+    if (rc != 0) return rc;
+    if (q.a.Cout != q.b.Cout || q.a.rows != q.b.rows || (q.a.xn == nullptr) != (q.b.xn == nullptr)) return MFT_EINVAL;
+    if (!wf_even_tiles(q.a) || !wf_even_tiles(q.b)) return MFT_EINVAL;
+    q.n_items = (n_img / imgs_per_group) * q.a.co_blocks;
+    q.per_xcd = q.n_items / 8;
+    return wf_launch_persistent<WF_RAW, WF_ENTRY>(q, (hipStream_t)stream);
+}
diff --git a/meta-fine-tuning_amd/functional.py b/meta-fine-tuning_amd/functional.py
--- a/meta-fine-tuning_amd/functional.py
+++ b/meta-fine-tuning_amd/functional.py
@@ -743,19 +743,24 @@
         if not hybrid:
             if fw:
                 wait_next_once()
-            ok = ops.wgrad_adam_next_forward(x, dsc, params.scw, m_.scw, v_.scw, 1, 1, 2, 0, st, ipg, x_next=x_next, mode=ops.WF_RAW,
-                                             raw=tn["sc"] if fw else None, **kw)
-            ok = ok and ops.wgrad_adam_next_forward(x, dc1, params.c1w, m_.c1w, v_.c1w, 3, 3, 2, 1, st, ipg, x_next=x_next,
-                                                    mode=ops.WF_ENTRY, raw=tn["c1"] if fw else None, act=tn["r1"] if fw else None,
-                                                    gamma=params.bn1g, beta=params.bn1b, gbs=C, mean=tn["m1"] if fw else None,
-                                                    rstd=tn["s1"] if fw else None, **kw)
-        ok = ok and ops.wgrad_adam_next_forward(r1, dc2, params.c2w, m_.c2w, v_.c2w, 3, 3, 1, 1, st, ipg,
-                                                x_next=tn["r1"] if fw else None, mode=ops.WF_EXIT, raw=tn["c2"] if fw else None,
-                                                act=tn["out"] if fw else None, gamma=params.bn2g, beta=params.bn2b, gbs=C,
-                                                mean=tn["m2"] if fw else None, rstd=tn["s2"] if fw else None,
-                                                sc_raw=tn["sc"] if fw else None, gamma_s=params.bnsg, beta_s=params.bnsb,
-                                                mean_s=tn["ms"] if fw else None, rstd_s=tn["ss"] if fw else None,
-                                                pooled=tn["feat"] if fw else None, **kw)
+            persist = settings.current().wf_persist
+            sc_kw = dict(x_next=x_next, mode=ops.WF_RAW, raw=tn["sc"] if fw else None)
+            c1_kw = dict(x_next=x_next, mode=ops.WF_ENTRY, raw=tn["c1"] if fw else None, act=tn["r1"] if fw else None,
+                         gamma=params.bn1g, beta=params.bn1b, gbs=C, mean=tn["m1"] if fw else None, rstd=tn["s1"] if fw else None)
+            ok = persist and ops.wgrad_adam_next_forward_pair(
+                ops.wf_layer(x, dsc, params.scw, m_.scw, v_.scw, 1, 1, 2, 0, **sc_kw),
+                ops.wf_layer(x, dc1, params.c1w, m_.c1w, v_.c1w, 3, 3, 2, 1, **c1_kw), st, ipg, **kw)
+            if not ok:
+                ok = ops.wgrad_adam_next_forward(x, dsc, params.scw, m_.scw, v_.scw, 1, 1, 2, 0, st, ipg, **sc_kw, **kw)
+                ok = ok and ops.wgrad_adam_next_forward(x, dc1, params.c1w, m_.c1w, v_.c1w, 3, 3, 2, 1, st, ipg, **c1_kw, **kw)
+        c2_kw = dict(x_next=tn["r1"] if fw else None, raw=tn["c2"] if fw else None, act=tn["out"] if fw else None,
+                     gamma=params.bn2g, beta=params.bn2b, gbs=C, mean=tn["m2"] if fw else None, rstd=tn["s2"] if fw else None,
+                     sc_raw=tn["sc"] if fw else None, gamma_s=params.bnsg, beta_s=params.bnsb, mean_s=tn["ms"] if fw else None,
+                     rstd_s=tn["ss"] if fw else None, pooled=tn["feat"] if fw else None)
+        c2 = (r1, dc2, params.c2w, m_.c2w, v_.c2w, 3, 3, 1, 1, st, ipg)
+        if ok and not (settings.current().wf_persist and
+                       ops.wgrad_adam_next_forward(*c2, mode=ops.WF_EXIT | ops.WF_PERSISTENT, **c2_kw, **kw)):
+            ok = ops.wgrad_adam_next_forward(*c2, mode=ops.WF_EXIT, **c2_kw, **kw)
         if not ok:
             raise RuntimeError("wgrad_adam_next_forward: shape outside the fused kernel's domain (the caller checks next_forward_ok)")
         assert waited[0] or not fw, "x_next was read without the caller's stream wait"
diff --git a/meta-fine-tuning_amd/ops.py b/meta-fine-tuning_amd/ops.py
--- a/meta-fine-tuning_amd/ops.py
+++ b/meta-fine-tuning_amd/ops.py
@@ -441,6 +441,7 @@
 
 
 WF_RAW, WF_ENTRY, WF_EXIT = 0, 1, 2
+WF_PERSISTENT = 4
 
 
 def wgrad_adam_next_forward(x, dy, w, m, v, KH, KW, stride, pad, step, imgs_per_group, x_next=None, mode=WF_RAW, raw=None, act=None,
@@ -458,6 +459,39 @@
     if rc == _lib.MFT_EINVAL:
         return False
     _lib.check(rc, "mft_wgrad_adam_next_forward")
+    return True
+
+
+class _WfLayer(ctypes.Structure):
+    _fields_ = [(n, ctypes.c_void_p) for n in ("x", "dy", "w", "m", "v", "dw", "x_next", "raw", "act", "gamma", "beta", "mean", "rstd",
+                                                "sc_raw", "gamma_s", "beta_s", "mean_s", "rstd_s", "pooled")] + \
+               [("group_stride", ctypes.c_longlong), ("gb_group_stride", ctypes.c_longlong)] + \
+               [(n, ctypes.c_int) for n in ("ldx", "ldy", "H", "W", "Cin", "Cout", "KH", "KW", "stride", "pad", "mode")]
+
+
+def wf_layer(x, dy, w, m, v, KH, KW, stride, pad, x_next=None, mode=WF_RAW, raw=None, act=None, gamma=None, beta=None, gbs=0, mean=None,
+             rstd=None, sc_raw=None, gamma_s=None, beta_s=None, mean_s=None, rstd_s=None, pooled=None, dw=None):
+    _f32c(x)
+    _f32c(dy)
+    n, H, W, Cin = x.shape
+    Cout = dy.shape[-1]
+    d = _WfLayer()
+    d.x, d.dy, d.w, d.m, d.v, d.dw = _p(x), _p(dy), _p(w), _p(m), _p(v), _p(dw)
+    d.x_next, d.raw, d.act, d.gamma, d.beta, d.mean, d.rstd = _p(x_next), _p(raw), _p(act), _p(gamma), _p(beta), _p(mean), _p(rstd)
+    d.sc_raw, d.gamma_s, d.beta_s, d.mean_s, d.rstd_s, d.pooled = _p(sc_raw), _p(gamma_s), _p(beta_s), _p(mean_s), _p(rstd_s), _p(pooled)
+    d.group_stride, d.gb_group_stride = Cout * KH * KW * Cin, gbs
+    d.ldx, d.ldy, d.H, d.W, d.Cin, d.Cout, d.KH, d.KW, d.stride, d.pad, d.mode = Cin, Cout, H, W, Cin, Cout, KH, KW, stride, pad, mode
+    d.n_img = n
+    return d
+
+
+def wgrad_adam_next_forward_pair(first, second, step, imgs_per_group, lr=0.01, beta1=0.9, beta2=0.999, eps=1e-8, hyper=None):
+    rc = _lib.lib().mft_wgrad_adam_next_forward_pair(ctypes.byref(first), ctypes.byref(second), first.n_img, imgs_per_group,
+                                                     1 if hyper is not None else step, _p(hyper), lr, beta1, beta2, eps, BN_EPS,
+                                                     _stream())
+    if rc == _lib.MFT_EINVAL:
+        return False
+    _lib.check(rc, "mft_wgrad_adam_next_forward_pair")
     return True
 
 
diff --git a/meta-fine-tuning_amd/settings.py b/meta-fine-tuning_amd/settings.py
--- a/meta-fine-tuning_amd/settings.py
+++ b/meta-fine-tuning_amd/settings.py
@@ -24,6 +24,7 @@
 KNOBS = (
     ("fuse_next", "MFT_FUSE_NEXT", _fuse, "auto", "fused weight-gradient + Adam + next-step forward launches: auto = engine.fuse_next_policy | 1 | 0"),
     ("wf_xcd", "MFT_WF_XCD", _flag, True, "fused launch: all workgroups of an episode on one XCD (A/B hook; read once per process)"),
+    ("wf_persist", "MFT_WF_PERSIST", _flag, True, "fused launches by persistent workgroups, shortcut + C1 as one pair launch (0: three one-item-per-workgroup launches; bit-identical, A/B)"),
     ("slab_candidates", "MFT_SLAB_CANDIDATES", _opt_int, None, "candidate buffers of the w/m/v placement scan (None: engine default 12; 0: off)"),
     ("slab_ballast_gb", "MFT_SLAB_BALLAST_GB", float, 12.0, "throw-away allocation between groups of placement candidates, GB"),
     ("slab_hints", "MFT_SLAB_HINTS", _flag, True, "re-use an earlier scan's placement when one probe confirms it"),
@@ -73,6 +74,7 @@
 class Settings:
     fuse_next: str = "auto"
     wf_xcd: bool = True
+    wf_persist: bool = True
     slab_candidates: "int | None" = None
     slab_ballast_gb: float = 12.0
     slab_hints: bool = True
```

After: 85.73. 0.964x the previous value.
